# willow-ahrens/ChainPartitioners.jl

Measured on AMD Instinct MI355X. Metric: partitions/sec, DynamicTotalSplitter(AffineConnectivityModel{Int64}(0,0,0,1)), K=64, higher is better.
Workload: dtype int64; 1 GPU; config 3: DynamicTotalSplitter(AffineConnectivityModel{Int64}(0,0,0,1)) on suitesparse_shaped CSR (seeded SplitMix64 generator, tests/synth.py), n=10000000 rows, nnz=100000000, K=64; one independent partition per GPU; n=10000000, nnz=100000000, K=64, includes_oracle_build=True, device_block_pool=True

## Files before the change

chainpartitioners.jl_amd/_lib.py:

```python
from __future__ import annotations

import ctypes as C
import os
from functools import partial
import weakref

import numpy as np

from . import models as M

_HERE = os.path.dirname(os.path.abspath(__file__))
LIB_PATH = os.environ.get("CP_LIB_PATH") or os.path.join(_HERE, "libchainpart.so")


class _Array:

    def __init__(self, dtype, name):
        self.dtype, self.name, self.what = np.dtype(dtype), name, np.dtype(dtype).name

    def _accepts(self, a):
        return a.dtype == self.dtype

    def from_param(self, a):
        if a is None:
            return None
        if not (isinstance(a, np.ndarray) and self._accepts(a) and a.flags.c_contiguous):
            got = f"{'' if a.flags.c_contiguous else 'non-contiguous '}{a.dtype} array" if isinstance(a, np.ndarray) else type(a).__name__
            raise TypeError(f"{self.name}: expected None or a C-contiguous {self.what} array, got {got}")
        return C.c_void_p(a.ctypes.data)


class _Words(_Array):

    def __init__(self, name):
        self.dtype, self.name, self.what = None, name, "8-byte-element"

    def _accepts(self, a):
        return a.dtype.itemsize == 8


_I64, _I32, _F64 = (partial(_Array, t) for t in (np.int64, np.int32, np.float64))
_i32, _i64, _f64, _vp, _str = C.c_int32, C.c_int64, C.c_double, C.c_void_p, C.c_char_p
_pi32, _pi64, _pf64, _pvp = C.POINTER(C.c_int32), C.POINTER(C.c_int64), C.POINTER(C.c_double), C.POINTER(C.c_void_p)
_MODEL, _ROWPART = C.POINTER(M.cp_model_t), C.POINTER(M.cp_rowpart_t)
_PACK = (_i32, [_vp, _MODEL, _ROWPART, _MODEL, _i64, _f64, _I64("spl_out"), _I64("K_out")])
_SPLIT = (_i32, [_vp, _i64, _MODEL, _ROWPART, _MODEL, _i64, _f64, _I64("spl_out")])

SIGNATURES = {
    "cp_last_error": (_str, []),
    "cp_version": (_i32, []),
    "cp_device_count": (_i32, []),
    "cp_csr_create": (_i32, [_i64, _i64, _i64, _I64("colptr"), _I64("rowval"), _i32, _pvp]),
    "cp_csr_create_device": (_i32, [_i64, _i64, _i64, _vp, _vp, _i32, _pvp]),
    "cp_csr_destroy": (_i32, [_vp]),
    "cp_adjoint": (_i32, [_vp, _pvp]),
    "cp_csr_download": (_i32, [_vp, _I64("dims_out"), _I64("colptr_out"), _I64("rowval_out")]),
    "cp_csr_reset_cache": (_i32, [_vp]),
    "cp_count_build": (_i32, [_vp, _i32, _i32, _pvp]),
    "cp_count_query": (_i32, [_vp, _i64, _I64("a"), _I64("b"), _I64("out")]),
    "cp_count_destroy": (_i32, [_vp]),
    "cp_link_array": (_i32, [_vp, _I64("out")]),
    "cp_domsum_build": (_i32, [_vp, _i32, _Words("val"), _pvp]),
    "cp_rook_build": (_i32, [_i64, _I64("idx"), _i32, _Words("val"), _i32, _pvp]),
    "cp_wsum_query": (_i32, [_vp, _i64, _I64("i"), _I64("j"), _I64("count_out"), _I64("sum_i64"), _F64("sum_f64")]),
    "cp_wsum_destroy": (_i32, [_vp]),
    "cp_partwise": (_i32, [_vp, _i64, _I64("asg"), _pi64, _I64("pios_out"), _I64("prm_out"), _I64("pos_out"), _I64("idx_out")]),
    "cp_oracle_eval": (_i32, [_vp, _MODEL, _ROWPART, _i32, _i64, _I64("j"), _I64("jp"), _I64("k"), _I64("out_i64"), _F64("out_f64")]),
    "cp_oracle_step": (_i32, [_vp, _MODEL, _ROWPART, _i64, _I32("move_j"), _I64("j"), _I32("move_jp"), _I64("jp"), _I64("k"),
                              _I64("out_i64"), _F64("out_f64")]),
    "cp_bound_stripe": (_i32, [_vp, _i64, _MODEL, _pi64, _pi64, _pf64, _pf64]),
    "cp_bound_stripe_pi": (_i32, [_vp, _i64, _ROWPART, _MODEL, _pi64, _pi64, _pf64, _pf64]),
    "cp_objective": (_i32, [_vp, _i64, _I64("spl"), _MODEL, _ROWPART, _i32, _pi64, _pf64]),
    "cp_partition_dynamic": (_i32, [_vp, _i64, _i32, _i32, _MODEL, _ROWPART, _MODEL, _i64, _f64, _I64("spl_out")]),
    "cp_pack_dynamic": _PACK,
    "cp_pack_dynamic_tables": (_i32, [_vp, _MODEL, _ROWPART, _MODEL, _i64, _f64, _I64("spl_tab"), _I64("cst_i64"), _F64("cst_f64")]),
    "cp_partition_bisect_cost": (_i32, [_vp, _i64, _MODEL, _f64, _i32, _I64("spl_out")]),
    "cp_partition_bisect_cost_batch": (_i32, [_vp, _i64, _I64("K"), _MODEL, _F64("eps"), _I32("flip"), _i64, _I64("spl_out")]),
    "cp_partition_bisect_cost_pi": (_i32, [_vp, _i64, _MODEL, _ROWPART, _f64, _i32, _I64("spl_out")]),
    "cp_partition_bisect_index_pi": (_i32, [_vp, _i64, _MODEL, _ROWPART, _i32, _I64("spl_out")]),
    "cp_pack_concave": _PACK,
    "cp_partition_concave": _SPLIT,
    "cp_partition_bisect_index": (_i32, [_vp, _i64, _MODEL, _i32, _I64("spl_out")]),
    "cp_partition_lazy_bisect_cost": (_i32, [_vp, _i64, _MODEL, _f64, _I64("spl_out")]),
    "cp_partition_lazy_bisect_cost_probes": (_i32, [_vp, _i64, _MODEL, _f64, _I64("spl_out"), _pi64]),
    "cp_partition_lazy_bisect_cost_pi": (_i32, [_vp, _i64, _MODEL, _ROWPART, _f64, _I64("spl_out"), _I64("nprobes_out")]),
    "cp_partition_lazy_flip_bisect_cost": (_i32, [_vp, _i64, _MODEL, _ROWPART, _f64, _I64("spl_out"), _I64("nprobes_out")]),
    "cp_pack_convex": _PACK,
    "cp_pack_convex_batch": (_i32, [_vp, _i64, _MODEL, _I64("wmax"), _i64, _I64("spl_out"), _I64("K_out")]),
    "cp_partition_convex": _SPLIT,
    "cp_pack_strict": (_i32, [_vp, _i64, _I64("spl_out"), _I64("K_out")]),
    "cp_pack_overlap": (_i32, [_vp, _f64, _i64, _I64("spl_out"), _I64("K_out"), _I64("n_nets_out")]),
    "cp_partition_equi": (_i32, [_i64, _i64, _I64("spl_out")]),
    "cp_pack_equi": (_i32, [_i64, _i64, _I64("spl_out"), _I64("K_out")]),
    "cp_dynamic_tables": (_i32, [_vp, _i64, _i32, _MODEL, _ROWPART, _I64("ptr_out"), _I64("cst_i64"), _F64("cst_f64")]),
    "cp_dynamic_tables_constrained": (_i32, [_vp, _i64, _MODEL, _i64, _I64("win_lo"), _I64("win_hi"), _I64("ptr_out"),
                                             _I64("cst_i64"), _F64("cst_f64")]),
    "cp_dynamic_tables_constrained_combine": (_i32, [_vp, _i64, _i32, _MODEL, _MODEL, _i64, _f64, _I64("win_lo"), _I64("win_hi"),
                                                     _I64("ptr_out"), _I64("cst_i64"), _F64("cst_f64")]),
    "cp_dp_begin": (_i32, [_vp, _i64, _i32, _i32, _MODEL, _i64, _i64, _pvp]),
    "cp_dp_layer": (_i32, [_vp, _i64, _vp, _vp]),
    "cp_dp_ptr_at": (_i32, [_vp, _i64, _i64, _pi64]),
    "cp_dp_ptr_row": (_i32, [_vp, _i64, _I64("out")]),
    "cp_dp_set_window": (_i32, [_vp, _i64]),
    "cp_dp_set_rows": (_i32, [_vp, _i64, _i64]),
    "cp_dp_block_tables": (_i32, [_vp, _pi32, _I64("opt_out"), _I64("nets_out"), _I64("selfnets_out")]),
    "cp_dp_destroy": (_i32, [_vp]),
    "cp_set_stream": (_i32, [_vp, _vp]),
    "cp_reset_stream": (_i32, [_vp]),
    "cp_get_stat": (_i32, [_str, _pi64]),
    "cp_test_round_scans": (_i32, [_I32("a"), _i64, _i64, _I32("b"), _i64, _i64, _i32, _i64, _i64, _i32, _i32,
                                   _I64("offs_out"), _I64("toffs_out"), _I64("res")]),
    "cp_test_fix_merge": (_i32, [_MODEL, _i64, _I64("toffs"), _I64("part_v"), _I32("part_p"), _I32("part_nn"), _I32("part_nl"), _I32("tile_s"),
                                 _I32("tile_s2"), _I32("anchor"), _I32("anchor2"), _I32("row"), _I32("plane"), _i64, _i32, _I32("p_out"),
                                 _I32("nn_out"), _I32("nl_out"), _I64("res")]),
    "cp_test_own_split": (_i32, [_vp, _I32("vpos_out"), _I32("vsa_out"), _I32("vnext_out"), _I64("res")]),
    "cp_test_own_pair": (_i32, [_i64, _i64, _I64("res")]),
    "cp_set_option": (_i32, [_str, _i64]),
    "cp_prof_enable": (_i32, [_i32]),
    "cp_prof_reset": (_i32, []),
    "cp_prof_get": (_i32, [_i32, C.POINTER(C.c_char_p), _pi64, _pf64, _pf64]),
}
SYMBOLS = list(SIGNATURES)

_lib = None


def _typed(name, fn, restype, argtypes):
    fn.restype, fn.argtypes = restype, argtypes

    def call(*args):
        try:
            return fn(*args)
        except C.ArgumentError as e:
            raise TypeError(f"{name}: {e}") from None
    return call


def load_library():
    global _lib
    if _lib is None:
        if not os.path.exists(LIB_PATH):
            raise RuntimeError(f"{LIB_PATH} is missing: build it with __graft_entry__.build() "
                               "(make -C chainpartitioners.jl_amd/csrc); there is no CPU fallback")
        lib = C.CDLL(LIB_PATH)
        for name, (restype, argtypes) in SIGNATURES.items():
            setattr(lib, name, _typed(name, getattr(lib, name), restype, argtypes))
        _lib = lib
    return _lib


def _cost_zeros(mm, shape):
    return np.zeros(shape, dtype=np.int64 if mm.struct.dtype == M.CP_I64 else np.float64)


def _by_type(a):
    return (None, a) if a.dtype == np.float64 else (a, None)


_COUNT_KIND = {"dom": 0, "net": 1, "selfnet": 2, "dianet": 3, "selfpin": 4}


class HipBackend:
    name = "hip"

    def __init__(self, device=0):
        self.lib = load_library()
        if self.lib.cp_device_count() <= 0:
            raise RuntimeError("libchainpart: no HIP device visible (the product path has no CPU fallback)")
        self.device = int(device)
        self._handles = {}

    def last_error(self):
        return (self.lib.cp_last_error() or b"").decode()

    def _ok(self, rc, what, exc=RuntimeError):
        if rc != 0:
            raise exc(f"{what} -> {rc}: {self.last_error()}")

    def _register(self, obj, h):
        lib, handles, key = self.lib, self._handles, id(obj)

        def _drop(_ref):
            handles.pop(key, None)
            lib.cp_csr_destroy(h)
        handles[key] = (weakref.ref(obj, _drop), h)
        return h

    def csr(self, A):
        ent = self._handles.get(id(A))
        if ent is not None and ent[0]() is A:
            return ent[1]
        h = C.c_void_p()
        rc = self.lib.cp_csr_create(A.m, A.n, A.nnz, A.colptr, A.rowval, self.device, C.byref(h))
        if rc != 0:
            raise RuntimeError(f"cp_csr_create failed ({rc}): {self.last_error()}")
        return self._register(A, h)

    def _h(self, A):
        return A if isinstance(A, C.c_void_p) else self.csr(A)

    def csr_from_device(self, m, n, N, colptr_dev_ptr, rowval_dev_ptr):
        h = C.c_void_p()
        rc = self.lib.cp_csr_create_device(m, n, N, colptr_dev_ptr, rowval_dev_ptr, self.device, C.byref(h))
        if rc != 0:
            raise RuntimeError(f"cp_csr_create_device failed ({rc}): {self.last_error()}")
        return h

    def csr_destroy(self, h):
        self.lib.cp_csr_destroy(h)

    def adjoint(self, A):
        from .types import SparseMatrixCSC
        t = C.c_void_p()
        rc = self.lib.cp_adjoint(self._h(A), C.byref(t))
        if rc != 0:
            raise RuntimeError(f"cp_adjoint failed ({rc}): {self.last_error()}")
        dims = np.zeros(3, dtype=np.int64)
        self.lib.cp_csr_download(t, dims, None, None)
        m, n, N = (int(x) for x in dims)
        colptr = np.zeros(n + 1, dtype=np.int64); rowval = np.zeros(max(N, 1), dtype=np.int64)
        rc = self.lib.cp_csr_download(t, dims, colptr, rowval)
        if rc != 0:
            self.lib.cp_csr_destroy(t)
            raise RuntimeError(f"cp_csr_download failed ({rc}): {self.last_error()}")
        T = SparseMatrixCSC(m, n, colptr, rowval[:N])
        self._register(T, t)
        return T

    def reset_cache(self, A_or_handle):
        return self.lib.cp_csr_reset_cache(self._h(A_or_handle))

    def set_stream(self, A_or_handle, stream_ptr):
        return self.lib.cp_set_stream(self._h(A_or_handle), stream_ptr)

    def reset_stream(self, A_or_handle):
        return self.lib.cp_reset_stream(self._h(A_or_handle))

    def get_stat(self, name):
        out = C.c_int64()
        rc = self.lib.cp_get_stat(name.encode(), C.byref(out))
        if rc != 0:
            raise KeyError(name)
        return out.value

    def test_round_scans(self, a, na_max, b, nb_max, two=True, cap_t=2**62, cap_nt=2**62, err_in=0, reps=1):
        a = np.ascontiguousarray(a, dtype=np.int32)
        b = np.ascontiguousarray(b, dtype=np.int32)
        offs = np.zeros(len(a) + 1, dtype=np.int64)
        toffs = np.zeros(len(b) + 1, dtype=np.int64)
        res = np.zeros(6, dtype=np.int64)
        rc = self.lib.cp_test_round_scans(a, len(a), na_max, b, len(b), nb_max, 1 if two else 0, cap_t, cap_nt, err_in, reps,
                                          offs, toffs, res)
        self._ok(rc, "cp_test_round_scans")
        return offs, toffs, dict(zip(("T", "NT", "nlong", "nown", "ntile", "err"), (int(v) for v in res)))

    def test_fix_merge(self, mm, toffs, part_v, part_p, part_nn, part_nl, tile_s, tile_s2, anchor, anchor2, row, plane, n, reps=1):
        i32 = lambda a: None if a is None else np.ascontiguousarray(a, dtype=np.int32)
        toffs = np.ascontiguousarray(toffs, dtype=np.int64)
        ntask = len(toffs) - 1
        part_v = np.ascontiguousarray(part_v, dtype=np.int64 if mm.struct.dtype == M.CP_I64 else np.float64).view(np.int64)
        p, nn, res = np.zeros(ntask, np.int32), np.zeros(ntask, np.int32), np.zeros(4, np.int64)
        nl = None if part_nl is None else np.zeros(ntask, np.int32)
        rc = self.lib.cp_test_fix_merge(mm, ntask, toffs, part_v, i32(part_p), i32(part_nn), i32(part_nl), i32(tile_s), i32(tile_s2), i32(anchor),
                                        i32(anchor2), i32(row), i32(plane), n, reps, p, nn, nl, res)
        self._ok(rc, "cp_test_fix_merge")
        return p, nn, nl, dict(zip(("items", "trips", "edges", "tickets_left"), (int(v) for v in res)))

    def test_own_split(self, A):
        nb = max(0, int(A.n).bit_length() - 8)
        vpos = np.zeros((max(nb, 1), A.n + 1), np.int32); vsa = np.zeros_like(vpos)
        vnext = np.zeros(max(A.nnz, 1), np.int32); res = np.zeros(2, np.int64)
        rc = self.lib.cp_test_own_split(self._h(A), vpos.reshape(-1), vsa.reshape(-1), vnext, res)
        self._ok(rc, "cp_test_own_split")
        assert int(res[0]) == nb
        return nb, vpos[:nb], vsa[:nb], vnext[:int(res[1])]

    def test_own_pair(self, nt, wave):
        res = np.zeros(3, np.int64)
        self._ok(self.lib.cp_test_own_pair(nt, wave, res), "cp_test_own_pair")
        return bool(res[0]), int(res[1]), int(res[2])

    def set_option(self, name, value):
        return self.lib.cp_set_option(name.encode(), value)

    def partition_dynamic(self, A, K, combine, order, mm, rp, wm, wi, wf, spl):
        return self.lib.cp_partition_dynamic(self._h(A), K, combine, order, mm, rp, wm, wi, wf, spl)

    def pack_dynamic(self, A, mm, rp, wm, wi, wf, spl, Kout):
        return self.lib.cp_pack_dynamic(self._h(A), mm, rp, wm, wi, wf, spl, Kout)

    def pack_dynamic_tables(self, A, mm, rp, wm, wi, wf):
        spl = np.zeros(A.n + 1, dtype=np.int64)
        cst = _cost_zeros(mm, A.n + 1)
        rc = self.lib.cp_pack_dynamic_tables(self._h(A), mm, rp, wm, wi, wf, spl, *_by_type(cst))
        return rc, cst, spl

    def partition_bisect_cost(self, A, K, mm, eps, flip, spl, rp=None):
        return self.lib.cp_partition_bisect_cost_pi(self._h(A), K, mm, rp, eps, flip, spl)

    def partition_bisect_cost_batch(self, A, Ks, mms, epss, flips):
        B = len(Ks)
        arr = (M.cp_model_t * B)(*[m.struct for m in mms])
        Kv = np.ascontiguousarray(Ks, dtype=np.int64)
        ev = np.ascontiguousarray(epss, dtype=np.float64)
        fv = np.ascontiguousarray(flips, dtype=np.int32)
        ld = int(Kv.max()) + 1
        out = np.zeros((B, ld), dtype=np.int64)
        rc = self.lib.cp_partition_bisect_cost_batch(self._h(A), B, Kv, arr, ev, fv, ld, out)
        return rc, [out[b, :int(Kv[b]) + 1].copy() for b in range(B)]

    def partition_bisect_index(self, A, K, mm, flip, spl, rp=None):
        return self.lib.cp_partition_bisect_index_pi(self._h(A), K, mm, rp, flip, spl)

    def partition_lazy_bisect_cost(self, A, K, mm, eps, spl):
        if getattr(mm, "rowpart", None) is not None:
            return self.lib.cp_partition_lazy_bisect_cost_pi(self._h(A), K, mm, mm.rowpart, eps, spl, None)
        return self.lib.cp_partition_lazy_bisect_cost(self._h(A), K, mm, eps, spl)

    def partition_lazy_bisect_cost_probes(self, A, K, mm, eps, rp=None):
        spl = np.zeros(K + 1, dtype=np.int64)
        if rp is not None:
            npr = np.zeros(1, dtype=np.int64)
            rc = self.lib.cp_partition_lazy_bisect_cost_pi(self._h(A), K, mm, rp, eps, spl, npr)
            return rc, spl, int(npr[0])
        npr = C.c_int64()
        rc = self.lib.cp_partition_lazy_bisect_cost_probes(self._h(A), K, mm, eps, spl, C.byref(npr))
        return rc, spl, npr.value

    def partition_lazy_flip_bisect_cost(self, A, K, mm, eps, spl, rp=None):
        return self.lib.cp_partition_lazy_flip_bisect_cost(self._h(A), K, mm, rp, eps, spl, None)

    def partition_lazy_flip_bisect_cost_probes(self, A, K, mm, eps, rp=None):
        spl, npr = np.zeros(K + 1, dtype=np.int64), np.zeros(1, dtype=np.int64)
        rc = self.lib.cp_partition_lazy_flip_bisect_cost(self._h(A), K, mm, rp, eps, spl, npr)
        return rc, spl, int(npr[0])

    def pack_convex(self, A, mm, rp, wm, wi, wf, spl, Kout):
        return self.lib.cp_pack_convex(self._h(A), mm, rp, wm, wi, wf, spl, Kout)

    def pack_convex_batch(self, A, mms, wmaxs, n):
        B = len(mms)
        arr = (M.cp_model_t * B)(*[m.struct for m in mms])
        wv = np.ascontiguousarray(wmaxs, dtype=np.int64)
        ld = int(n) + 1
        out = np.zeros((B, ld), dtype=np.int64)
        Kout = np.zeros(B, dtype=np.int64)
        rc = self.lib.cp_pack_convex_batch(self._h(A), B, arr, wv, ld, out, Kout)
        return rc, [out[b, :int(Kout[b]) + 1].copy() for b in range(B)]

    def partition_convex(self, A, K, mm, rp, wm, wi, wf, spl):
        return self.lib.cp_partition_convex(self._h(A), K, mm, rp, wm, wi, wf, spl)

    def pack_concave(self, A, mm, rp, wm, wi, wf, spl, Kout):
        return self.lib.cp_pack_concave(self._h(A), mm, rp, wm, wi, wf, spl, Kout)

    def partition_concave(self, A, K, mm, rp, wm, wi, wf, spl):
        return self.lib.cp_partition_concave(self._h(A), K, mm, rp, wm, wi, wf, spl)

    def pack_strict(self, A, w_max, spl, Kout):
        return self.lib.cp_pack_strict(self._h(A), int(w_max), spl, Kout)

    def pack_overlap(self, A, rho, w_max, spl, Kout, n_nets=None):
        return self.lib.cp_pack_overlap(self._h(A), float(rho), int(w_max), spl, Kout, n_nets)

    def oracle_eval(self, A, mm, rp, hint, j, jp, k, out):
        return self.lib.cp_oracle_eval(self._h(A), mm, rp, hint, j.size, j, jp, k, *_by_type(out))

    def oracle_step(self, A, mm, rp, mj, j, mjp, jp, k, out):
        return self.lib.cp_oracle_step(self._h(A), mm, rp, j.size, mj, j, mjp, jp, k, *_by_type(out))

    def _bounds(self, fn, mm, *args):
        li, hi, lf, hf = C.c_int64(), C.c_int64(), C.c_double(), C.c_double()
        rc = fn(*args, C.byref(li), C.byref(hi), C.byref(lf), C.byref(hf))
        if mm.struct.dtype == M.CP_I64:
            return rc, li.value, hi.value
        return rc, lf.value, hf.value

    def bound_stripe(self, A, K, mm):
        return self._bounds(self.lib.cp_bound_stripe, mm, self._h(A), K, mm)

    def bound_stripe_pi(self, A, K, rp, mm):
        return self._bounds(self.lib.cp_bound_stripe_pi, mm, self._h(A), K, rp, mm)

    def objective(self, A, K, spl, mm, rp, g):
        oi, of = C.c_int64(), C.c_double()
        rc = self.lib.cp_objective(self._h(A), K, spl, mm, rp, g, C.byref(oi), C.byref(of))
        return rc, (oi.value if mm.struct.dtype == M.CP_I64 else of.value)

    def dynamic_tables(self, A, K, combine, mm, rp):
        ptr = np.zeros((K, A.n + 1), dtype=np.int64)
        cst = _cost_zeros(mm, (K, A.n + 1))
        rc = self.lib.cp_dynamic_tables(self._h(A), K, combine, mm, rp, ptr, *_by_type(cst))
        return rc, ptr.T, cst.T

    def dynamic_tables_constrained(self, A, K, mm, wmax, combine=0, wm=None):
        ptr = np.zeros((K, A.n + 1), dtype=np.int64)
        cst = _cost_zeros(mm, (K, A.n + 1))
        lo = np.zeros(K, dtype=np.int64); hi = np.zeros(K, dtype=np.int64)
        rc = self.lib.cp_dynamic_tables_constrained_combine(self._h(A), K, combine, mm, wm, int(wmax), float(wmax), lo, hi, ptr,
                                                            *_by_type(cst))
        return rc, lo, hi, ptr.T, cst.T

    def count_build(self, kind, A, hint):
        h = C.c_void_p()
        rc = self.lib.cp_count_build(self._h(A), _COUNT_KIND[kind], hint, C.byref(h))
        if rc == M.CP_EINVAL and kind in ("dianet", "selfpin"):
            raise AssertionError(f"cp_count_build({kind}): violated precondition ({self.last_error()})")
        self._ok(rc, f"cp_count_build({kind})", NotImplementedError)
        return h

    def count_query(self, kind, h, a, b, out):
        return self.lib.cp_count_query(h, a.size, a, b, out)

    def count_free(self, kind, h):
        self.lib.cp_count_destroy(h)

    def domsum_build(self, A, val):
        val = np.ascontiguousarray(val)
        dt = M.CP_F64 if val.dtype == np.float64 else M.CP_I64
        h = C.c_void_p()
        self._ok(self.lib.cp_domsum_build(self._h(A), dt, val, C.byref(h)), "cp_domsum_build")
        return h, dt

    def rook_build(self, N, idx, val=None):
        idx = np.ascontiguousarray(idx, dtype=np.int64)
        dt = M.CP_I64
        if val is not None:
            val = np.ascontiguousarray(val)
# ... 104 lines not shown
```

chainpartitioners.jl_amd/csrc/capi.hip:

```cpp
#include "csr.hpp"
#include "model.hpp"
#include "dp.hpp"
#include "weight.hpp"
#include "sym.hpp"
#include "cut.hpp"
#include <cmath>
#include <memory>

using namespace cpk;

namespace cpk {

__global__ void __launch_bounds__(256) k_range_counts(int64_t nq, const int64_t *__restrict__ P, const int64_t *__restrict__ Rr,
                                                      const int64_t *__restrict__ pos, const int32_t *__restrict__ prev,
                                                      const int64_t *__restrict__ fpos, const int32_t *__restrict__ flast,
                                                      unsigned long long *__restrict__ nets, unsigned long long *__restrict__ selfnets)
{
    int64_t i = blockIdx.x;
    if (i >= nq) return;
    __shared__ int64_t sh[256];
    int64_t p = P[i], r = Rr[i];
    int64_t stride = (int64_t)gridDim.y * 256, start = (int64_t)blockIdx.y * 256 + threadIdx.x;
    int64_t c = 0;
    if (r > p) {
        int64_t q0 = pos[p], q1 = pos[r];
        int32_t thr = (int32_t)p;
        for (int64_t q = q0 + start; q < q1; q += stride) c += (prev[q] < thr);
    }
    sh[threadIdx.x] = c;
    __syncthreads();
    for (int o = 128; o > 0; o >>= 1) { if (threadIdx.x < (unsigned)o) sh[threadIdx.x] += sh[threadIdx.x + o]; __syncthreads(); }
    if (threadIdx.x == 0 && sh[0]) atomicAdd(&nets[i], (unsigned long long)sh[0]);
    __syncthreads();
    if (selfnets) {
        c = 0;
        if (r > p) {
            int64_t s0 = fpos[p], s1 = fpos[r];
            int32_t thr = (int32_t)r;
            for (int64_t s = s0 + start; s < s1; s += stride) c += (flast[s] < thr);
        }
        sh[threadIdx.x] = c;
        __syncthreads();
        for (int o = 128; o > 0; o >>= 1) { if (threadIdx.x < (unsigned)o) sh[threadIdx.x] += sh[threadIdx.x + o]; __syncthreads(); }
        if (threadIdx.x == 0 && sh[0]) atomicAdd(&selfnets[i], (unsigned long long)sh[0]);
    }
}

template <typename TC>
__global__ void k_apply_model(int64_t nq, const int64_t *__restrict__ P, const int64_t *__restrict__ Rr, const int64_t *__restrict__ Kk,
                              const int64_t *__restrict__ pos, const int64_t *__restrict__ nets, const int64_t *__restrict__ selfnets,
                              DevModel<TC> M, TC *__restrict__ out)
{
    int64_t i = (int64_t)blockIdx.x * blockDim.x + threadIdx.x;
    if (i >= nq) return;
    int64_t p = P[i], r = Rr[i];
    TC alpha = dm_alpha(M, Kk ? Kk[i] : (int64_t)0);
    out[i] = dm_apply(M, alpha, r - p, pos[r] - pos[p], nets ? nets[i] : (int64_t)0, selfnets ? selfnets[i] : (int64_t)0);
}

static bool model_known(const cp_model_t *m)
{
    if (!m || m->kind < CP_MODEL_FEASIBLE || m->kind > CP_MODEL_SECONDARY_EDGE_CUT) return false;
    if (m->kind == CP_MODEL_POWER_WORK) return m->dtype == CP_F64;
    return m->dtype == CP_I64 || m->dtype == CP_F64;
}

template <typename TC>
static int32_t run_oracle_eval(cp_csr_s *A, const cp_model_t *mdl, int64_t nq, const int64_t *j, const int64_t *jp,
                               const int64_t *k, TC *out)
{
    hipStream_t s = A->stream;
    if (nq <= 0) return CP_OK;
    bool has_nets = mdl->kind == CP_MODEL_CONNECTIVITY || mdl->kind == CP_MODEL_HYPEREDGE_CUT || mdl->kind == CP_MODEL_COLBLOCK;
    bool need_self = mdl->kind == CP_MODEL_HYPEREDGE_CUT;
    if (has_nets) ensure_links(A);
    if (need_self) ensure_self(A);
    std::vector<int64_t> hp((size_t)nq), hr((size_t)nq);
    for (int64_t i = 0; i < nq; i++) {
        CP_REQUIRE(j[i] >= 1 && jp[i] >= j[i] && jp[i] <= A->n + 1, CP_EINVAL, "oracle query needs 1 <= j <= j' <= n+1");
        hp[i] = j[i] - 1; hr[i] = jp[i] - 1;
    }
    DBuf<int64_t> dP((size_t)nq), dR((size_t)nq), dK, dN, dS;
    DBuf<TC> dO((size_t)nq);
    CP_HIP(hipMemcpyAsync(dP.p, hp.data(), sizeof(int64_t) * (size_t)nq, hipMemcpyHostToDevice, s));
    CP_HIP(hipMemcpyAsync(dR.p, hr.data(), sizeof(int64_t) * (size_t)nq, hipMemcpyHostToDevice, s));
    if (k) { dK.alloc((size_t)nq); CP_HIP(hipMemcpyAsync(dK.p, k, sizeof(int64_t) * (size_t)nq, hipMemcpyHostToDevice, s)); }
    if (has_nets) {
        dN.alloc((size_t)nq);
        CP_HIP(hipMemsetAsync(dN.p, 0, dN.bytes(), s));
        if (need_self) { dS.alloc((size_t)nq); CP_HIP(hipMemsetAsync(dS.p, 0, dS.bytes(), s)); }
        int64_t per = nq > 0 ? A->N / nq : 0;
        unsigned gy = (unsigned)(per / 65536 + 1);
        if (gy > 2048) gy = 2048;
        ProfScope ps(PROF_QUERY, s, 0.0);
        hipLaunchKernelGGL(k_range_counts, dim3((unsigned)nq, gy), dim3(256), 0, s, nq, dP.p, dR.p, A->pos.p, A->prev.p,
                           need_self ? A->fpos.p : nullptr, need_self ? A->flast.p : nullptr, (unsigned long long *)dN.p,
                           need_self ? (unsigned long long *)dS.p : nullptr);
    }
    HostModel<TC> HM;
    build_dev_model<TC>(mdl, HM, s);
    hipLaunchKernelGGL(HIP_KERNEL_NAME(k_apply_model<TC>), dim3((unsigned)cdiv(nq, 256)), dim3(256), 0, s, nq, dP.p, dR.p,
                       k ? dK.p : nullptr, A->pos.p, has_nets ? dN.p : nullptr, need_self ? dS.p : nullptr, HM.d, dO.p);
    CP_HIP(hipGetLastError());
    CP_HIP(hipMemcpyAsync(out, dO.p, sizeof(TC) * (size_t)nq, hipMemcpyDeviceToHost, s));
    CP_HIP(hipStreamSynchronize(s));
    prof_collect();
    return CP_OK;
}

static int64_t fld(int64_t a, int64_t b)
{
    int64_t q = a / b, r = a % b;
    if (r != 0 && ((r < 0) != (b < 0))) q -= 1;
    return q;
}
static double fld(double a, int64_t b) { return std::floor(a / (double)b); }
static int64_t max_identity(int64_t) { return INT64_MIN; }
static double max_identity(double) { return -INFINITY; }
static void also_f64(const int64_t *lo, const int64_t *hi, double *lo_f64, double *hi_f64) { *lo_f64 = (double)*lo; *hi_f64 = (double)*hi; }
static void also_f64(const double *, const double *, double *, double *) {}

template <typename TC>
static int32_t oracle_eval_into(cp_csr_t A, const cp_model_t *model, const cp_rowpart_t *Pi, int64_t nq, const int64_t *j, const int64_t *jp,
                                const int64_t *k, TC *out)
{
    const bool i64 = std::is_same<TC, int64_t>::value;
    return cp_oracle_eval(A, model, Pi, CP_HINT_STEP, nq, j, jp, k, i64 ? (int64_t *)out : nullptr, i64 ? nullptr : (double *)out);
}

static const struct { const char *name; int64_t *var; bool kept; } g_stats[] = {
    {"spec_redo", &g_spec_redo, false}, {"poison_hits", &g_poison_hits, false}, {"fix_trips", &g_fix_trips, false},
    {"fix_edges", &g_fix_edges, false}, {"fix_items", &g_fix_items, false}, {"bn_sym_layers", &g_bn_sym_layers, true},
    {"own_split_tiles", &g_own_split_tiles, false}, {"gap_split_tiles", &g_gap_split_tiles, false},
    {"own_pair_waves", &g_own_pair_waves, false}, {"own_pair_lone", &g_own_pair_lone, false},
    {"overlap_isect", &g_overlap_isect, false}, {"cut_scan_layers", &g_cut_scan_layers, false},
};
static void stats_reset(bool all) { for (const auto &c : g_stats) if (all || !c.kept) *c.var = 0; }

enum OptRule { OPT_PLAIN, OPT_BOOL, OPT_CLAMP, OPT_POW2 };
constexpr int64_t NOLIM_LO = INT64_MIN, NOLIM_HI = INT64_MAX;
static const struct Opt { const char *name; int64_t *var; OptRule rule; int64_t lo, hi; } g_options[] = {
    {"force_brute", &g_opt_force_brute, OPT_PLAIN, 0, 0}, {"brute_max_n", &g_opt_brute_max_n, OPT_PLAIN, 0, 0}, {"dbg", &g_opt_dbg, OPT_PLAIN, 0, 0},
    {"short_t", &g_opt_short_t, OPT_PLAIN, 0, 0}, {"short_e", &g_opt_short_e, OPT_PLAIN, 0, 0}, {"ra_cache", &g_opt_ra_cache, OPT_PLAIN, 0, 0},
    {"leaf", &g_opt_leaf, OPT_PLAIN, 0, 0}, {"block_tables", &g_opt_block_tables, OPT_PLAIN, 0, 0}, {"nospec", &g_opt_nospec, OPT_PLAIN, 0, 0},
    {"rpass_small_tau", &g_opt_rpass_small_tau, OPT_PLAIN, 0, 0}, {"fixed_point", &g_opt_fixed_point, OPT_PLAIN, 0, 0},
    {"bn_wave", &g_opt_bn_wave, OPT_PLAIN, 0, 0},
    {"poison", &g_opt_poison, OPT_PLAIN, 0, 0},
    {"pool", &g_opt_pool, OPT_BOOL, 0, 0},
    {"own_blk", &g_opt_own_blk, OPT_BOOL, 0, 0},
    {"own_split", &g_opt_own_split, OPT_BOOL, 0, 0},
    {"own_pair", &g_opt_own_pair, OPT_BOOL, 0, 0},
    {"gap_split", &g_opt_gap_split, OPT_BOOL, 0, 0},
    {"lws", &g_opt_lws, OPT_BOOL, 0, 0},
    {"gap_tau", &g_opt_gap_tau, OPT_CLAMP, NOLIM_LO, 20}, {"gap_min", &g_opt_gap_min, OPT_CLAMP, 8, NOLIM_HI}, {"gap_nr", &g_opt_gap_nr, OPT_CLAMP, 1, 2},
    {"force_max", &g_opt_force_max, OPT_CLAMP, 0, NOLIM_HI}, {"rpass_cap", &g_opt_rpass_cap, OPT_CLAMP, 1, NOLIM_HI},
    {"own_min", &g_opt_own_min, OPT_CLAMP, 64, NOLIM_HI}, {"bn_chunk", &g_opt_bn_chunk, OPT_CLAMP, 1, NOLIM_HI},
    {"bn_slack", &g_opt_bn_slack, OPT_CLAMP, 0, NOLIM_HI}, {"bn_run", &g_opt_bn_run, OPT_CLAMP, 2, NOLIM_HI},
    {"rpass_ch", &g_opt_rpass_ch, OPT_POW2, 16, 4096}, {"setup_bs", &g_opt_setup_bs, OPT_POW2, 64, 1024}, {"lws_leaf", &g_opt_lws_leaf, OPT_POW2, 256, 2048},
};
static int64_t opt_value(const Opt &o, int64_t value)
{
    switch (o.rule) {
    case OPT_BOOL: return value ? 1 : 0;
    case OPT_CLAMP: return value < o.lo ? o.lo : value > o.hi ? o.hi : value;
    case OPT_POW2: { int64_t v = o.lo; while (v < value && v < o.hi) v <<= 1; return v; }
    default: return value;
    }
}

}

extern "C" {

const char *cp_last_error(void) { return g_last_error.c_str(); }
int32_t cp_version(void) { return 100; }

int32_t cp_device_count(void)
{
    int c = 0;
    if (hipGetDeviceCount(&c) != hipSuccess) return 0;
    return c;
}

static int32_t csr_create_impl(int64_t m, int64_t n, int64_t N, const int64_t *colptr, const int64_t *rowval,
                               int32_t device, bool on_device, cp_csr_t *out)
{
    return guarded([&]() -> int32_t {
        CP_REQUIRE(out && colptr && (rowval || N == 0), CP_EINVAL, "null argument");
        CP_REQUIRE(m >= 0 && n >= 0 && N >= 0, CP_EINVAL, "negative dimension");
        CP_REQUIRE(n < (int64_t)1 << 30 && m < (int64_t)1 << 30 && N < ((int64_t)1 << 31) - 65536, CP_EINVAL,
                   "dimensions exceed the 32-bit link-array layout");
        CP_REQUIRE(cp_device_count() > 0, CP_EHIP, "no HIP device visible: libchainpart has no CPU fallback");
        CP_HIP(hipSetDevice(device));
        std::unique_ptr<cp_csr_s> A(new cp_csr_s());
        A->device = device; A->m = m; A->n = n; A->N = N;
        CP_HIP(hipStreamCreate(&A->stream));
        A->own_stream = true;
        csr_upload(A.get(), colptr, rowval, on_device);
        *out = A.release();
        return CP_OK;
    });
}

int32_t cp_csr_create(int64_t m, int64_t n, int64_t N, const int64_t *colptr, const int64_t *rowval, int32_t device, cp_csr_t *out)
{
    if (colptr && n >= 0 && (colptr[0] != 1 || colptr[n] != N + 1)) { set_error("colptr must be 1-based with colptr[n+1] == nnz+1"); return CP_EINVAL; }
    return csr_create_impl(m, n, N, colptr, rowval, device, false, out);
}

int32_t cp_csr_create_device(int64_t m, int64_t n, int64_t N, const int64_t *colptr_device, const int64_t *rowval_device,
                             int32_t device, cp_csr_t *out)
{
    return csr_create_impl(m, n, N, colptr_device, rowval_device, device, true, out);
}

int32_t cp_csr_destroy(cp_csr_t A)
{
    if (!A) return CP_OK;
    (void)hipSetDevice(A->device);
    if (A->stream) (void)hipStreamSynchronize(A->stream);
    delete A;
    return CP_OK;
}

int32_t cp_adjoint(cp_csr_t A, cp_csr_t *out)
{
    return guarded([&]() -> int32_t {
        CP_REQUIRE(A && out, CP_EINVAL, "null argument");
        CP_HIP(hipSetDevice(A->device));
        std::unique_ptr<cp_csr_s> T(new cp_csr_s());
        T->device = A->device;
        CP_HIP(hipStreamCreate(&T->stream));
        T->own_stream = true;
        csr_adjoint(A, T.get());
        *out = T.release();
        return CP_OK;
    });
}

int32_t cp_csr_download(cp_csr_t A, int64_t *dims_out, int64_t *colptr_out, int64_t *rowval_out)
{
    return guarded([&]() -> int32_t {
        CP_REQUIRE(A, CP_EINVAL, "null argument");
        if (dims_out) { dims_out[0] = A->m; dims_out[1] = A->n; dims_out[2] = A->N; }
        if (!colptr_out) return CP_OK;
        CP_REQUIRE(rowval_out || A->N == 0, CP_EINVAL, "rowval_out is null");
        CP_HIP(hipSetDevice(A->device));
        csr_download(A, colptr_out, rowval_out);
        return CP_OK;
    });
}

int32_t cp_csr_reset_cache(cp_csr_t A)
{
    if (!A) return CP_EINVAL;
    return guarded([&]() -> int32_t { CP_HIP(hipStreamSynchronize(A->stream)); drop_cache(A); return CP_OK; });
}

int32_t cp_set_stream(cp_csr_t A, void *hip_stream)
{
    if (!A) return CP_EINVAL;
    if (A->own_stream && A->stream) { (void)hipStreamSynchronize(A->stream); (void)hipStreamDestroy(A->stream); }
    A->stream = (hipStream_t)hip_stream;
    A->own_stream = false;
    return CP_OK;
}

int32_t cp_get_stat(const char *name, int64_t *out)
{
    if (!name || !out) return CP_EINVAL;
    for (const auto &c : g_stats) if (!strcmp(name, c.name)) { *out = *c.var; return CP_OK; }
    return CP_EINVAL;
}

int32_t cp_test_round_scans(const int32_t *a, int64_t na, int64_t na_max, const int32_t *b, int64_t nb, int64_t nb_max, int32_t two, int64_t cap_t,
                            int64_t cap_nt, int32_t err_in, int32_t reps, int64_t *offs_out, int64_t *toffs_out, int64_t *res)
{
    if (!offs_out || !toffs_out || !res || (na > 0 && !a) || (nb > 0 && !b)) return CP_EINVAL;
    return guarded([&]() -> int32_t {
        dp_round_scans_test(a, na, na_max, b, nb, nb_max, two, cap_t, cap_nt, err_in, reps, offs_out, toffs_out, res);
        return CP_OK;
    });
}

int32_t cp_test_fix_merge(const cp_model_t *model, int64_t ntask, const int64_t *toffs, const int64_t *part_v, const int32_t *part_p, const int32_t *part_nn,
                          const int32_t *part_nl, const int32_t *tile_s, const int32_t *tile_s2, const int32_t *anchor, const int32_t *anchor2,
                          const int32_t *row, const int32_t *plane, int64_t n, int32_t reps, int32_t *p_out, int32_t *nn_out, int32_t *nl_out, int64_t *res)
{
    if (!model || !toffs || !part_v || !part_p || !part_nn || !tile_s || !anchor || !row || !plane || !p_out || !nn_out || !res) return CP_EINVAL;
    return guarded([&]() -> int32_t {
        dp_fix_merge_test(model, ntask, toffs, part_v, part_p, part_nn, part_nl, tile_s, tile_s2, anchor, anchor2, row, plane, n, reps, p_out, nn_out, nl_out, res);
        return CP_OK;
    });
}

int32_t cp_test_own_pair(int64_t nt, int64_t wave, int64_t *res)
{
    if (!res) return CP_EINVAL;
    return guarded([&]() -> int32_t {
        dp_own_pair_test(nt, wave, res);
        return CP_OK;
    });
}

int32_t cp_test_own_split(cp_csr_t A, int32_t *vpos_out, int32_t *vsa_out, int32_t *vnext_out, int64_t *res)
{
    if (!A || !vpos_out || !vsa_out || !vnext_out || !res) return CP_EINVAL;
    return guarded([&]() -> int32_t {
        CP_HIP(hipSetDevice(A->device));
        dp_own_split_test(A, vpos_out, vsa_out, vnext_out, res);
        return CP_OK;
    });
}

int32_t cp_reset_stream(cp_csr_t A)
{
    if (!A) return CP_EINVAL;
    return guarded([&]() -> int32_t {
        if (A->stream || !A->own_stream) (void)hipStreamSynchronize(A->stream);
        if (A->own_stream) return CP_OK;
        CP_HIP(hipSetDevice(A->device));
        hipStream_t s = nullptr;
        CP_HIP(hipStreamCreate(&s));
        A->stream = s; A->own_stream = true;
        return CP_OK;
    });
}

int32_t cp_set_option(const char *name, int64_t value)
{
    if (!name) return CP_EINVAL;
    if (!strcmp(name, "stat_reset")) { stats_reset(true); return CP_OK; }
    if (!strcmp(name, "prof_only")) { g_prof_only = (int)value; return CP_OK; }
    for (const Opt &o : g_options) {
        if (strcmp(name, o.name)) continue;
        *o.var = opt_value(o, value);
        if (o.var == &g_opt_pool && !value) dev_pool_trim();
        if (o.var == &g_opt_poison && value) stats_reset(false);
        return CP_OK;
    }
    set_error("unknown option");
    return CP_EINVAL;
}

int32_t cp_prof_enable(int32_t on) { g_prof_on = on != 0; return CP_OK; }
int32_t cp_prof_reset(void)
{
    for (auto &p : g_prof) { p.launches = 0; p.ms = 0; p.alg_bytes = 0; }
    return CP_OK;
}
int32_t cp_prof_get(int32_t slot, const char **name, int64_t *launches, double *total_ms, double *alg_bytes)
{
    if (slot >= 0 && slot < PROF_NSLOTS) {
        if (name) *name = g_prof[slot].name;
        if (launches) *launches = g_prof[slot].launches;
        if (total_ms) *total_ms = g_prof[slot].ms;
        if (alg_bytes) *alg_bytes = g_prof[slot].alg_bytes;
    }
    return PROF_NSLOTS;
}

int32_t cp_partition_equi(int64_t n, int64_t K, int64_t *spl_out)
{
    if (K < 1 || n < 0 || !spl_out) return CP_EINVAL;
    for (int64_t k = 0; k <= K; k++) spl_out[k] = k * (n / K) + ((n % K) < k ? (n % K) : k) + 1;
    return CP_OK;
}

int32_t cp_pack_equi(int64_t n, int64_t w, int64_t *spl_out, int64_t *K_out)
{
    if (w < 1 || n < 0 || !spl_out || !K_out) return CP_EINVAL;
    int64_t K = 0;
    for (int64_t j = 1; j <= n; j += w) spl_out[K++] = j;
    spl_out[K] = n + 1;
    *K_out = K;
    return CP_OK;
}

int32_t cp_partition_dynamic(cp_csr_t A, int64_t K, int32_t combine, int32_t order, const cp_model_t *model,
                             const cp_rowpart_t *Pi, const cp_model_t *weight, int64_t wmax_i64, double wmax_f64, int64_t *spl_out)
{
    return guarded([&]() -> int32_t {
        CP_REQUIRE(A && spl_out && model_known(model) && K >= 1, CP_EINVAL, "bad argument");
        CP_REQUIRE(combine == CP_COMBINE_SUM || combine == CP_COMBINE_MAX, CP_EINVAL, "bad combine");
        CP_HIP(hipSetDevice(A->device));
        bool constrained = weight && weight->kind != CP_MODEL_FEASIBLE;
        if (model->kind == CP_MODEL_PRIMARY || model->kind == CP_MODEL_SECONDARY) {
            CP_REQUIRE(!constrained, CP_EUNSUPPORTED, "ConstrainedCost over a plaid connectivity model has no device path");
            return with_cost_type(model->dtype, [&](auto tag) { return run_plaid_dynamic<decltype(tag)>(A, K, combine, order, model, Pi, spl_out); });
        }
        if (model_is_cut(model->kind)) {
            CP_REQUIRE(!constrained, CP_EUNSUPPORTED, "ConstrainedCost over a plaid edge-cut model has no device path");
            return with_cost_type(model->dtype, [&](auto tag) {
                using TC = decltype(tag);
                return run_cut_dynamic<TC>(A, K, combine, order, model, Pi, spl_out, nullptr, (TC *)nullptr);
            });
        }
        CP_REQUIRE(!(constrained && model_is_sym(model->kind)), CP_EUNSUPPORTED, "ConstrainedCost over a symmetric cost model has no device path");
        if (constrained) {
            CP_REQUIRE(weight->kind == CP_MODEL_VERTEX_COUNT || (weight->kind == CP_MODEL_WORK && !weight->alpha_k), CP_EINVAL,
                       "weight must be VertexCount or an AffineWorkModel");
            const int64_t wv = width_of_weight(weight, A->n, wmax_i64, wmax_f64);
            if (windowed_ok(A, K, combine, model, wv))
                return run_dynamic_windowed(A, K, combine, order, model, wv, nullptr, 0, 0, spl_out, nullptr, nullptr, nullptr, nullptr, nullptr);
            if (combine == CP_COMBINE_MAX && wv == -2 && monotone_work_weight(weight) && model->dtype == CP_I64 && windowed_ok(A, K, combine, model, 1))
                return run_dynamic_windowed(A, K, combine, order, model, 0, weight, wmax_i64, wmax_f64, spl_out, nullptr, nullptr, nullptr, nullptr, nullptr);
            return with_cost_type(model->dtype, [&](auto tag) {
                return run_dyn_constrained<decltype(tag)>(A, K, combine, order, model, Pi, weight, wmax_i64, wmax_f64, spl_out);
            });
        }
        CP_REQUIRE(model->kind == CP_MODEL_WORK || model->kind == CP_MODEL_CONNECTIVITY || model->kind == CP_MODEL_HYPEREDGE_CUT ||
                       model->kind == CP_MODEL_COLBLOCK || model->kind == CP_MODEL_POWER_WORK || model_is_sym(model->kind),
                   CP_EUNSUPPORTED, "model kind has no device DP path yet");
        return run_dynamic(A, K, combine, order, model, spl_out, nullptr, nullptr, nullptr);
    });
}

int32_t cp_dynamic_tables(cp_csr_t A, int64_t K, int32_t combine, const cp_model_t *model, const cp_rowpart_t *Pi,
                          int64_t *ptr_out, int64_t *cst_i64, double *cst_f64)
{
    return guarded([&]() -> int32_t {
        CP_REQUIRE(A && ptr_out && model_known(model) && K >= 1, CP_EINVAL, "bad argument");
        CP_REQUIRE(combine == CP_COMBINE_SUM || combine == CP_COMBINE_MAX, CP_EINVAL, "bad combine");
        if (model_is_cut(model->kind)) {
            CP_HIP(hipSetDevice(A->device));
            std::vector<int64_t> spl((size_t)K + 1);
            return with_cost_type(model->dtype, [&](auto tag) {
                using TC = decltype(tag);
                return run_cut_dynamic<TC>(A, K, combine, CP_ORDER_SPLITTER, model, Pi, spl.data(), ptr_out, pick<TC>(cst_i64, cst_f64));
            });
        }
        CP_REQUIRE(model->kind == CP_MODEL_WORK || model->kind == CP_MODEL_CONNECTIVITY || model->kind == CP_MODEL_HYPEREDGE_CUT ||
                       model->kind == CP_MODEL_COLBLOCK || model->kind == CP_MODEL_POWER_WORK || model_is_sym(model->kind),
                   CP_EUNSUPPORTED, "model kind has no device DP path");
        CP_HIP(hipSetDevice(A->device));
        std::vector<int64_t> spl((size_t)K + 1);
        return run_dynamic(A, K, combine, CP_ORDER_SPLITTER, model, spl.data(), ptr_out, cst_i64, cst_f64);
    });
}

int32_t cp_dynamic_tables_constrained_combine(cp_csr_t A, int64_t K, int32_t combine, const cp_model_t *model, const cp_model_t *weight,
                                              int64_t wmax_i64, double wmax_f64, int64_t *win_lo, int64_t *win_hi, int64_t *ptr_out,
                                              int64_t *cst_i64, double *cst_f64)
{
    return guarded([&]() -> int32_t {
        CP_REQUIRE(A && ptr_out && win_lo && win_hi && model_known(model) && K >= 1, CP_EINVAL, "bad argument");
        CP_REQUIRE(combine == CP_COMBINE_SUM || combine == CP_COMBINE_MAX, CP_EINVAL, "bad combine");
        CP_REQUIRE(!weight || weight->kind == CP_MODEL_VERTEX_COUNT || (weight->kind == CP_MODEL_WORK && !weight->alpha_k), CP_EINVAL,
                   "weight must be VertexCount or an AffineWorkModel");
        const int64_t wv = weight ? width_of_weight(weight, A->n, wmax_i64, wmax_f64) : wmax_i64;
        const bool general = wv == -2 && combine == CP_COMBINE_MAX && monotone_work_weight(weight) && model->dtype == CP_I64;
        CP_REQUIRE(windowed_ok(A, K, combine, model, general ? 1 : wv), CP_EUNSUPPORTED, "outside the windowed scalable path");
        CP_HIP(hipSetDevice(A->device));
        std::vector<int64_t> spl((size_t)K + 1);
        return run_dynamic_windowed(A, K, combine, CP_ORDER_SPLITTER, model, general ? 0 : wv, general ? weight : nullptr, wmax_i64, wmax_f64,
                                    spl.data(), ptr_out, cst_i64, cst_f64, win_lo, win_hi);
    });
}

int32_t cp_dynamic_tables_constrained(cp_csr_t A, int64_t K, const cp_model_t *model, int64_t wmax, int64_t *win_lo, int64_t *win_hi,
                                      int64_t *ptr_out, int64_t *cst_i64, double *cst_f64)
{
    return cp_dynamic_tables_constrained_combine(A, K, CP_COMBINE_SUM, model, nullptr, wmax, (double)wmax, win_lo, win_hi, ptr_out, cst_i64, cst_f64);
// ... 292 lines not shown
```

chainpartitioners.jl_amd/csrc/dp.hpp:

```cpp
#pragma once
#include "csr.hpp"
#include "model.hpp"

struct cp_dp_s {
    cp_csr_s *A = nullptr;
    int64_t K = 0;
    int32_t combine = 0, order = 0;
    bool fast = false, fast_bn = false, need_self = false;
    void *work = nullptr;
    cpk::DBuf<int32_t> ptr;
    int64_t rlo = 0, rhi = 0;
    int64_t wwin = 0;
    std::vector<int64_t> lay_lo, lay_hi;
    virtual ~cp_dp_s() = default;
    virtual int32_t step_layer(int64_t k, const void *cst_prev_device, void *cst_cur_device) = 0;
    virtual int32_t block_tables(int32_t *nplanes_out, int64_t *opt_out, int64_t *nets_out, int64_t *selfnets_out) = 0;
};

namespace cpk {

using DpBase = ::cp_dp_s;

struct DpWindow {
    int64_t w = 0;
    int64_t lo = 0, hi = -1;
    const int32_t *j0 = nullptr;
};

int32_t run_dynamic(cp_csr_s *A, int64_t K, int32_t combine, int32_t order, const cp_model_t *mdl, int64_t *spl_out,
                    int64_t *ptr_tab, int64_t *cst_i64, double *cst_f64);
bool windowed_ok(cp_csr_s *A, int64_t K, int32_t combine, const cp_model_t *model, int64_t wmax);
int32_t run_dynamic_windowed(cp_csr_s *A, int64_t K, int32_t combine, int32_t order, const cp_model_t *mdl, int64_t width,
                             const cp_model_t *weight, int64_t wmax_i64, double wmax_f64, int64_t *spl_out, int64_t *ptr_tab,
                             int64_t *cst_i64, double *cst_f64, int64_t *win_lo, int64_t *win_hi);
int32_t dp_begin(cp_csr_s *A, int64_t K, int32_t combine, int32_t order, const cp_model_t *model, int64_t row_lo, int64_t row_hi,
                 cp_dp_s **out);

template <typename TC>
void dp_total_layer(cp_csr_s *A, const DevModel<TC> &M, TC alpha, const TC *W, TC *cst_out, int32_t *ptr_out, void *work,
                    int64_t rlo, int64_t rhi,
                    int64_t wwin = 0);
template <typename TC> int dp_total_block_tables(cp_csr_s *A, void *work, int64_t *opt_out, int64_t *nn_out, int64_t *nl_out);
template <typename TC> void *dp_total_work_get(cp_csr_s *A);
template <typename TC> void *dp_total_work_new();
template <typename TC> void dp_total_work_free(void *w);

template <typename TC>
void dp_brute_layer(cp_csr_s *A, const DevModel<TC> &M, TC alpha, int32_t combine, const TC *W, TC *cst_out,
                    int32_t *ptr_out, int64_t r_lo, int64_t r_hi);

struct WaveletDev;
struct BnPattern {
    const int64_t *pos; const int32_t *pos32, *pin32, *prev, *next;
    int64_t N;
    const WaveletDev *net;
};
extern int64_t g_bn_sym_layers;

template <typename TC>
void dp_bottleneck_layer(cp_csr_s *A, const DevModel<TC> &M, TC alpha, const TC *W, TC *cst_out, int32_t *ptr_out,
                         int64_t r_lo, int64_t r_hi,
                         int64_t wwin = 0, int64_t p_lo0 = 0, int64_t p_hi0 = -1, const int32_t *j0 = nullptr,
                         const BnPattern *pat = nullptr);
extern int64_t g_opt_bn_wave, g_opt_bn_run, g_opt_bn_slack;
extern int64_t g_opt_bn_chunk;

template <typename TC>
int32_t run_dyn_constrained(cp_csr_s *A, int64_t K, int32_t g, int32_t order, const cp_model_t *mdl, const cp_rowpart_t *Pi,
                            const cp_model_t *w, int64_t wi, double wf, int64_t *spl_out);
template <typename TC>
int32_t run_seq_eval(cp_csr_s *A, const cp_model_t *mdl, const cp_rowpart_t *Pi, int64_t nq, const int64_t *j, const int64_t *jp,
                     const int64_t *k, TC *out);

struct PlaidPart {
    DBuf<int32_t> owner;
    DBuf<int64_t> spl;
    std::vector<int64_t> hspl;
    int64_t K = 0;
};
void upload_part(cp_csr_s *A, const cp_rowpart_t *Pi, bool need_spl, PlaidPart &R);
template <typename TC>
int32_t run_plaid_eval(cp_csr_s *A, const cp_model_t *mdl, const cp_rowpart_t *Pi, int64_t nq, const int64_t *j, const int64_t *jp,
                       const int64_t *k, TC *out);
template <typename TC>
int32_t run_plaid_dynamic(cp_csr_s *A, int64_t K, int32_t combine, int32_t order, const cp_model_t *mdl, const cp_rowpart_t *Pi,
                          int64_t *spl_out);

template <typename TC>
bool pack_dynamic_scan(hipStream_t s, int64_t n, int64_t wmax, const TC *Ftab, TC *cst1, int64_t *spl1);

extern int64_t g_opt_lws, g_opt_lws_leaf;
bool lws_ok(const cp_csr_s *A, const cp_model_t *mdl, const cp_model_t *w, int64_t wi, double wf);
template <typename TC>
int32_t run_pack_lws(cp_csr_s *A, const DevModel<TC> &M, const WaveletDev &wnet, const WaveletDev &wself, const cp_model_t *w, int64_t wi,
                     double wf, TC *cst1, int64_t *spl1);

extern int64_t g_opt_gap_nr;
extern int64_t g_opt_gap_tau, g_opt_gap_min;
extern int64_t g_opt_poison, g_poison_hits;
void dp_round_scans_test(const int32_t *a, int64_t na, int64_t na_max, const int32_t *b, int64_t nb, int64_t nb_max, int two, int64_t capT, int64_t capNT,
                         int err_in, int reps, int64_t *offs_out, int64_t *toffs_out, int64_t *res);
void dp_fix_merge_test(const cp_model_t *model, int64_t ntask, const int64_t *toffs, const int64_t *part_v, const int32_t *part_p, const int32_t *part_nn,
                       const int32_t *part_nl, const int32_t *tile_s, const int32_t *tile_s2, const int32_t *anchor, const int32_t *anchor2, const int32_t *row,
                       const int32_t *plane, int64_t n, int reps, int32_t *p_out, int32_t *nn_out, int32_t *nl_out, int64_t *res);
extern int64_t g_fix_trips, g_fix_edges;
extern int64_t g_fix_items;
extern int64_t g_opt_leaf;
extern int64_t g_opt_block_tables;
extern int64_t g_opt_ra_cache;
extern int64_t g_opt_fixed_point;
extern int64_t g_opt_nospec;
extern int64_t g_spec_redo;
extern int64_t g_opt_rpass_small_tau;
extern int64_t g_opt_force_max;
extern int64_t g_opt_setup_bs;
extern int64_t g_opt_rpass_cap;
extern int64_t g_opt_rpass_ch;
extern int64_t g_opt_own_min;
extern int64_t g_opt_own_blk;
extern int64_t g_opt_own_split;
extern int64_t g_own_split_tiles;
extern int64_t g_opt_gap_split;
extern int64_t g_gap_split_tiles;
extern int64_t g_opt_own_pair;
extern int64_t g_own_pair_waves, g_own_pair_lone;
void dp_own_pair_test(int64_t nt, int64_t wave, int64_t *res);
extern int64_t g_overlap_isect;
void dp_own_split_test(cp_csr_s *A, int32_t *vpos_out, int32_t *vsa_out, int32_t *vnext_out, int64_t *res);
extern int64_t g_opt_short_t, g_opt_short_e;
extern int64_t g_opt_force_brute;
extern int64_t g_opt_brute_max_n;
extern int64_t g_opt_dbg;
enum DbgBit : int64_t {
    DBG_PRINT_ROUNDS = 8,
    DBG_NO_INTERIOR = 32,
    DBG_NO_OWN_TILES = 64,
    DBG_POISON = 128,
    DBG_POISON_ZERO = 256,
    DBG_GAP_ALL_SPECIAL = 512,
    DBG_MISPREDICT = 1024,
    DBG_TINY_BUFFERS = 2048,
    DBG_COUNT_NONTRIVIAL = 4096,
    DBG_COMBINE_BY_SLOT = 16384,
    DBG_RA_ROWMAJOR = 262144,
    DBG_NO_FORCE_OWN = 524288,
    DBG_WIN_NO_RA_CACHE = 1048576,
    DBG_WIN_NO_MIR_CACHE = 2097152,
    DBG_BN_NO_HINT2 = 4194304,
    DBG_MIR_ROWMAJOR = 8388608,
    DBG_RA_ALL_LEVELS = 33554432,
    DBG_BN_NO_HINT_STARTS = 33554432,
};

}
```

chainpartitioners.jl_amd/csrc/dp_brute.hip:

```cpp
#include "csr.hpp"
#include "model.hpp"
#include "dp.hpp"

namespace cpk {

int64_t g_opt_force_brute = 0;
int64_t g_opt_short_t = 8, g_opt_short_e = 64;
int64_t g_opt_own_min = 64;
int64_t g_opt_own_blk = 1;
int64_t g_opt_own_split = 1;
int64_t g_own_split_tiles = 0;
int64_t g_opt_gap_split = 1;
int64_t g_gap_split_tiles = 0;
int64_t g_opt_own_pair = 1;
int64_t g_own_pair_waves = 0, g_own_pair_lone = 0;
int64_t g_opt_rpass_ch = 256;
int64_t g_opt_rpass_small_tau = 4;
int64_t g_opt_force_max = 1024;
int64_t g_opt_setup_bs = 1024;
int64_t g_opt_rpass_cap = 200;
int64_t g_opt_nospec = 0, g_spec_redo = 0;
int64_t g_opt_gap_tau = 6, g_opt_gap_min = 64, g_opt_gap_nr = 2;
int64_t g_opt_ra_cache = 1;
int64_t g_opt_leaf = 1, g_opt_block_tables = 0;
int64_t g_opt_poison = 0, g_poison_hits = 0;
int64_t g_fix_trips = 0, g_fix_edges = 0, g_fix_items = 0;
int64_t g_opt_fixed_point = 0;
int64_t g_opt_brute_max_n = 200000;
int64_t g_opt_dbg = 0;

template <typename TC>
__global__ void __launch_bounds__(256) k_brute_layer(int64_t n, int64_t r_lo, int64_t r_hi, const int64_t *__restrict__ pos,
                                                     const int32_t *__restrict__ next, const int64_t *__restrict__ fpos,
                                                     const int32_t *__restrict__ flast, DevModel<TC> M, TC alpha,
                                                     int32_t g, const TC *__restrict__ W, TC *__restrict__ cst,
                                                     int32_t *__restrict__ ptr)
{
    int64_t wave = ((int64_t)blockIdx.x * blockDim.x + threadIdx.x) >> 6;
    int lane = threadIdx.x & 63;
    int64_t r0 = r_lo + wave * 64;
    if (r0 > r_hi) return;
    int64_t r = r0 + lane;
    bool live = r <= r_hi;
    int64_t rtop = r0 + 63 < r_hi ? r0 + 63 : r_hi;
    int64_t nn = 0, nl = 0;
    TC best = (TC)0;
    int64_t bp = -1;
    bool self = (M.kind == CP_MODEL_HYPEREDGE_CUT);
    int32_t rr = (int32_t)r;
    for (int64_t p = rtop; p >= 0; p--) {
        if (p < n) {
            bool step = live && (r > p);
            int64_t q0 = pos[p], q1 = pos[p + 1];
            for (int64_t q = q0; q < q1; q++) {
                int32_t nx = next[q];
                if (step) nn += (nx >= rr);
            }
            if (self) {
                int64_t s0 = fpos[p], s1 = fpos[p + 1];
                for (int64_t sidx = s0; sidx < s1; sidx++) {
                    int32_t la = flast[sidx];
                    if (step) nl += (la < rr);
                }
            }
        }
        if (live && r >= p) {
            TC f = dm_apply(M, alpha, r - p, pos[r] - pos[p], nn, nl);
            TC v = comb(g, W[p], f);
            if (bp < 0 || v < best) { best = v; bp = p; }
        }
    }
    if (live) { cst[r] = best; ptr[r] = (int32_t)bp; }
}

template <typename TC>
void dp_brute_layer(cp_csr_s *A, const DevModel<TC> &M, TC alpha, int32_t combine, const TC *W, TC *cst_out,
                    int32_t *ptr_out, int64_t r_lo, int64_t r_hi)
{
    hipStream_t s = A->stream;
    int64_t rows = r_hi - r_lo + 1;
    int64_t waves = cdiv(rows, 64);
    int64_t blocks = cdiv(waves, 4);
    ProfScope ps(PROF_BRUTE, s, 0.0);
    hipLaunchKernelGGL(HIP_KERNEL_NAME(k_brute_layer<TC>), dim3((unsigned)blocks), dim3(256), 0, s, A->n, r_lo, r_hi, A->pos.p,
                       A->next.p, A->fpos.p, A->flast.p, M, alpha, combine, W, cst_out, ptr_out);
    CP_HIP(hipGetLastError());
}

template void dp_brute_layer<int64_t>(cp_csr_s *, const DevModel<int64_t> &, int64_t, int32_t, const int64_t *, int64_t *, int32_t *, int64_t, int64_t);
template void dp_brute_layer<double>(cp_csr_s *, const DevModel<double> &, double, int32_t, const double *, double *, int32_t *, int64_t, int64_t);

}
```

chainpartitioners.jl_amd/csrc/dp_total.hip:

```cpp
#include "dp_total.hpp"
#include <optional>

namespace cpk {

struct RoundDesc {
    int32_t isA, tau, nbits, nextra;
    Geo G;
    int64_t aoff[32];
    int64_t n, ntask;
    int64_t tbase[36];
    int64_t tskip[36];
    int64_t a_r0, a_nmain;
    int64_t extra[64];
    int32_t nlast, last_b[31];
    int32_t skip_std, skip_mir;
    int32_t fin_stamp;
};

__device__ __forceinline__ void decode_task(const RoundDesc &R, int64_t t, int64_t &r, int &b)
{
    if (R.G.win) {
        int bb = R.isA ? 0 : R.tau + 1;
        while (t >= R.tbase[bb + 1]) bb++;
        const int64_t l = t - R.tbase[bb] + R.tskip[bb];
        r = R.isA ? ((l + 1) << bb) : (((l << 1) | 1) << R.tau);
        b = bb;
        return;
    }
    if (R.isA) {
        if (t >= R.a_nmain + R.nextra) { r = R.n; b = R.last_b[t - R.a_nmain - R.nextra]; return; }
        r = t < R.a_nmain ? R.a_r0 + t : R.extra[t - R.a_nmain]; b = __ffsll((long long)r) - 1; return;
    }
    int bb = R.tau + 1;
    while (t >= R.tbase[bb + 1]) bb++;
    int64_t l = t - R.tbase[bb] + R.tskip[bb];
    int sh = bb - R.tau - 1;
    int64_t base = l >> sh, v = l & (((int64_t)1 << sh) - 1);
    r = (base << (bb + 1)) | ((int64_t)1 << bb) | (((v << 1) | 1) << R.tau);
    b = bb;
}

template <bool ge, int NB>
__global__ void __launch_bounds__(256) k_rpass_small(int tau, int nbits, int64_t n, int64_t u0, int64_t nrows, const int64_t *__restrict__ pos,
                                                     const int32_t *__restrict__ prev, const int32_t *__restrict__ opt,
                                                     int32_t *__restrict__ cr, int allp, int cap)
{
    int64_t u = (int64_t)blockIdx.x * blockDim.x + threadIdx.x;
    bool live = u < nrows;
    u += u0;
    int64_t r = ((u << 1) | 1) << tau;
    if (r > n) live = false;
    if (!live) r = 0;
    int64_t n1 = n + 1, rL = r - ((int64_t)1 << tau);
    int32_t thr[NB], cnt[NB];
    uint32_t used = 0;
    int64_t prL = live ? prow((rL), n1 - 1) : 0;
#pragma unroll
    for (int b = 0; b < NB; b++) {
        cnt[b] = 0;
        thr[b] = ge ? INT32_MAX : INT32_MIN;
        if (b <= tau || b >= nbits) continue;
        bool on = live && (allp || ((r >> b) & 1));
        if (!__ballot(on)) continue;
        used |= 1u << b;
        int32_t v = opt[(int64_t)b * n1 + (on ? prL : 0)];
        if (on) thr[b] = v;
    }
    int64_t q0 = 0;
    int32_t len = 0;
    if (live) { q0 = pos[rL]; len = (int32_t)(pos[r] - q0); }
    const int32_t NEVER = ge ? INT32_MIN : INT32_MAX;
    const int32_t mlen = len < cap ? len : cap;
    for (int32_t o = 0; o < mlen; o += 16) {
        int32_t v[16];
        struct __attribute__((packed, aligned(4))) V4 { int32_t a, b, c, d; };
        const V4 *pv = reinterpret_cast<const V4 *>(prev + q0 + o);
        const int32_t rem = mlen - o;
#pragma unroll
        for (int j = 0; j < 4; j++) {
            V4 t = {NEVER, NEVER, NEVER, NEVER};
            if (4 * j < rem) t = pv[j];
            v[4 * j] = t.a; v[4 * j + 1] = t.b; v[4 * j + 2] = t.c; v[4 * j + 3] = t.d;
        }
#pragma unroll
        for (int j = 0; j < 16; j++) v[j] = j < rem ? v[j] : NEVER;
#pragma unroll
        for (int b = 0; b < NB; b++) {
            if (!((used >> b) & 1)) continue;
            int32_t t = thr[b];
            int32_t c = 0;
#pragma unroll
            for (int j = 0; j < 16; j++) c += ge ? (v[j] >= t) : (v[j] < t);
            cnt[b] += c;
        }
    }
    {
        const int lane = threadIdx.x & 63;
        uint32_t mypl = 0;
        if (live)
            for (int b = tau + 1; b < nbits; b++) if (allp || ((r >> b) & 1)) mypl |= 1u << b;
        uint64_t rest = __ballot(len > cap);
        const int32_t q0lo = (int32_t)(uint32_t)q0, q0hi = (int32_t)(q0 >> 32);
        while (rest) {
            const int src = __ffsll((unsigned long long)rest) - 1;
            rest &= rest - 1;
            const int64_t a = (((int64_t)__builtin_amdgcn_readlane(q0hi, src) << 32) | (uint32_t)__builtin_amdgcn_readlane(q0lo, src)) + cap;
            const int32_t ln = __builtin_amdgcn_readlane(len, src) - cap;
            const uint32_t pl = (uint32_t)__builtin_amdgcn_readlane((int32_t)mypl, src);
            for (int32_t o = 0; o < ln; o += 64) {
                const int32_t v = o + lane < ln ? prev[a + o + lane] : NEVER;
#pragma unroll
                for (int b = 0; b < NB; b++) {
                    if (!((pl >> b) & 1)) continue;
                    const int32_t t = __builtin_amdgcn_readlane(thr[b], src);
                    const int32_t c = (int32_t)__popcll(__ballot(ge ? (v >= t) : (v < t)));
                    if (lane == src) cnt[b] += c;
                }
            }
        }
    }
    if (!live) return;
#pragma unroll
    for (int b = 0; b < NB; b++)
        if (b > tau && b < nbits && (allp || ((r >> b) & 1))) cr[(int64_t)b * n1 + prow((r), n1 - 1)] = cnt[b];
}

template <bool ge, int WPB>
__global__ void __launch_bounds__(64 * WPB) k_rpass_wave(int tau, int nbits, int64_t n, int64_t u0, int64_t nrows, int chunks_per_row, int ch_cols,
                                                         const int64_t *__restrict__ pos, const int32_t *__restrict__ prev,
                                                         const int32_t *__restrict__ opt, int32_t *__restrict__ cr, int allp)
{
    int64_t w = (int64_t)blockIdx.x * WPB + (threadIdx.x >> 6);
    int lane = threadIdx.x & 63;
    int64_t u = w / chunks_per_row;
    int ck = (int)(w - u * chunks_per_row);
    if (u >= nrows) return;
    u += u0;
    int64_t r = ((u << 1) | 1) << tau;
    if (r > n) return;
    int64_t n1 = n + 1, rL = r - ((int64_t)1 << tau);
    int64_t c0 = rL + (int64_t)ck * ch_cols, c1 = c0 + ch_cols;
    if (c1 > r) c1 = r;
    int64_t prL = prow((rL), n1 - 1);
    uint32_t act = 0;
    for (int b = tau + 1; b < nbits; b++) if (allp || ((r >> b) & 1)) act |= 1u << b;
    act = __builtin_amdgcn_readfirstlane(act);
    const bool mine = lane < 32 && ((act >> lane) & 1);
    const int32_t tv = mine ? opt[(int64_t)lane * n1 + prL] : 0;
    int32_t acc = 0;
    const int64_t q0 = pos[c0], q1 = pos[c1];
    const int32_t NEVER = ge ? INT32_MIN : INT32_MAX;
    int32_t a[8], nx[8];
    struct __attribute__((packed, aligned(4))) V4 { int32_t x, y, z, w; };
#pragma unroll
    for (int k = 0; k < 2; k++) {
        const int64_t q = q0 + 4 * lane + 256 * k;
        V4 t = {NEVER, NEVER, NEVER, NEVER};
        if (q < q1) t = *reinterpret_cast<const V4 *>(prev + q);
        a[4 * k] = t.x; a[4 * k + 1] = q + 1 < q1 ? t.y : NEVER; a[4 * k + 2] = q + 2 < q1 ? t.z : NEVER; a[4 * k + 3] = q + 3 < q1 ? t.w : NEVER;
    }
    for (int64_t qb = q0; qb < q1; qb += 512) {
#pragma unroll
        for (int k = 0; k < 2; k++) {
            const int64_t q = qb + 512 + 4 * lane + 256 * k;
            V4 t = {NEVER, NEVER, NEVER, NEVER};
            if (q < q1) t = *reinterpret_cast<const V4 *>(prev + q);
            nx[4 * k] = t.x; nx[4 * k + 1] = q + 1 < q1 ? t.y : NEVER; nx[4 * k + 2] = q + 2 < q1 ? t.z : NEVER; nx[4 * k + 3] = q + 3 < q1 ? t.w : NEVER;
        }
        for (uint32_t rem = act; rem; rem &= rem - 1) {
            const int b = __ffs(rem) - 1;
            const int32_t t = __builtin_amdgcn_readlane(tv, b);
            int32_t c = 0;
#pragma unroll
            for (int k = 0; k < 8; k++) c += (int32_t)__popcll(__ballot(ge ? (a[k] >= t) : (a[k] < t)));
            acc += lane == b ? c : 0;
        }
#pragma unroll
        for (int k = 0; k < 8; k++) a[k] = nx[k];
    }
    int32_t outv = acc;
    if (WPB > 1) {
        __shared__ int32_t sacc[WPB > 1 ? WPB : 1][32];
        const int wv = threadIdx.x >> 6;
        if (lane < 32) sacc[wv][lane] = mine ? outv : 0;
        __syncthreads();
        if (wv != 0) return;
        if (mine) {
            int32_t t = 0;
#pragma unroll
            for (int k = 0; k < WPB; k++) t += sacc[k][lane];
            outv = t;
        }
    }
    if (mine) {
        if (chunks_per_row == WPB) cr[(int64_t)lane * n1 + prow((r), n1 - 1)] = outv;
        else atomicAdd(&cr[(int64_t)lane * n1 + prow((r), n1 - 1)], outv);
    }
}

__global__ void __launch_bounds__(256) k_last_row_counts(RoundDesc R, const int32_t *__restrict__ pos, const int32_t *__restrict__ prev,
                                                         const int32_t *__restrict__ lpos, const int32_t *__restrict__ lfirst, int32_t *__restrict__ out,
                                                         uint8_t *__restrict__ fin)
{
    __shared__ int32_t s_acc[64];
    if (threadIdx.x < 64) s_acc[threadIdx.x] = 0;
    __syncthreads();
    const int64_t n = R.n, n1 = n + 1;
    if (blockIdx.x == 0 && threadIdx.x < (unsigned)R.nlast) fin[(int64_t)R.last_b[threadIdx.x] * n1 + prow(n, n)] = (uint8_t)R.fin_stamp;
    for (int pass = 0; pass < (lpos ? 2 : 1); pass++) {
        const int32_t *cp = pass ? lpos : pos, *arr = pass ? lfirst : prev;
        for (int i = 0; i < R.nlast; i++) {
            const int64_t rb = (n >> R.last_b[i]) << R.last_b[i];
            int32_t c = 0;
            for (int64_t q = (int64_t)cp[rb] + (int64_t)blockIdx.x * blockDim.x + threadIdx.x, q1 = cp[n]; q < q1; q += (int64_t)gridDim.x * blockDim.x) {
                int32_t v = arr[q];
                c += pass ? (v >= rb) : (v < rb);
            }
            for (int o = 32; o > 0; o >>= 1) c += __shfl_xor(c, o);
            if ((threadIdx.x & 63) == 0 && c) atomicAdd(&s_acc[pass * 32 + i], c);
        }
    }
    __syncthreads();
    if (threadIdx.x < 64 && s_acc[threadIdx.x]) {
        int pass = threadIdx.x >> 5, i = threadIdx.x & 31;
        if (i < R.nlast) atomicAdd(&out[pass * 32 + R.last_b[i]], s_acc[threadIdx.x]);
    }
}

__global__ void __launch_bounds__(256) k_setup(RoundDesc R, const int32_t *__restrict__ opt, const int32_t *__restrict__ nnopt,
                                               int32_t *__restrict__ cr, int zero_cr_only,
                                               int4 *__restrict__ tdesc, const int32_t *__restrict__ pos32,
                                               uint8_t *__restrict__ tb, int32_t *__restrict__ len,
                                               const int32_t *__restrict__ nlopt, int32_t *__restrict__ crl, int32_t *__restrict__ tS0l)
{
    int64_t t = (int64_t)blockIdx.x * blockDim.x + threadIdx.x;
    if (t >= R.ntask) return;
    int64_t r; int b;
    decode_task(R, t, r, b);
    int64_t n1 = R.n + 1;
    if (zero_cr_only) { cr[(int64_t)b * n1 + prow((r), n1 - 1)] = 0; if (crl) crl[(int64_t)b * n1 + prow((r), n1 - 1)] = 0; return; }
    int64_t B, a, S0, S0l = 0;
    if (R.isA) {
        B = r; a = r - ((int64_t)1 << b); S0 = 0;
    } else {
        int64_t rb = (r >> b) << b;
        int64_t rL = r - ((int64_t)1 << R.tau), rR = r + ((int64_t)1 << R.tau);
        B = opt[(int64_t)b * n1 + prow((rL), n1 - 1)];
        S0 = (int64_t)nnopt[(int64_t)b * n1 + prow((rL), n1 - 1)] + cr[(int64_t)b * n1 + prow((r), n1 - 1)];
        if (tS0l) S0l = (int64_t)nlopt[(int64_t)b * n1 + prow((rL), n1 - 1)] + crl[(int64_t)b * n1 + prow((r), n1 - 1)];
        a = (rR - rb) < ((int64_t)1 << b) ? (int64_t)opt[(int64_t)b * n1 + prow((rR <= R.n ? rR : R.n), n1 - 1)] : rb - ((int64_t)1 << b);
        if (a > B) a = B;
    }
    tdesc[t] = make_int4((int32_t)B, (int32_t)S0, (int32_t)r, pos32[r]);
    tb[t] = (uint8_t)b;
    len[t] = (int32_t)(1 + (B - a));
    if (tS0l) tS0l[t] = (int32_t)S0l;
}

template <typename TC> __device__ __forceinline__ void best_clear(Best<TC, false> &b) { b.v = (TC)0; b.p = -1; b.nn = 0; }
template <typename TC> __device__ __forceinline__ void best_clear(Best<TC, true> &b) { b.v = (TC)0; b.p = -1; b.nn = 0; b.nl = 0; b._pad = 0; }
template <typename TC> __device__ __forceinline__ int32_t best_nl(const Best<TC, false> &) { return 0; }
template <typename TC> __device__ __forceinline__ int32_t best_nl(const Best<TC, true> &b) { return b.nl; }
template <typename TC> __device__ __forceinline__ void best_set_nl(Best<TC, false> &, int32_t) {}
template <typename TC> __device__ __forceinline__ void best_set_nl(Best<TC, true> &b, int32_t v) { b.nl = v; }

template <typename TC>
__device__ __forceinline__ Best<TC, false> best_sel(bool tb, const Best<TC, false> a, const Best<TC, false> b)
{
    Best<TC, false> r; r.v = tb ? b.v : a.v; r.p = tb ? b.p : a.p; r.nn = tb ? b.nn : a.nn; return r;
}
template <typename TC>
__device__ __forceinline__ Best<TC, true> best_sel(bool tb, const Best<TC, true> a, const Best<TC, true> b)
{
    Best<TC, true> r; r.v = tb ? b.v : a.v; r.p = tb ? b.p : a.p; r.nn = tb ? b.nn : a.nn; r.nl = tb ? b.nl : a.nl; r._pad = 0; return r;
}
template <typename TC, bool HYP>
__device__ __forceinline__ Best<TC, HYP> better(const Best<TC, HYP> a, const Best<TC, HYP> b)
{
    const bool tb = a.p < 0 || (b.p >= 0 && b.v < a.v);
    return best_sel<TC>(tb, a, b);
}

__device__ __forceinline__ void wave_segsum(int32_t &v, int &f, int lane)
{
#pragma unroll
    for (int o = 1; o < 64; o <<= 1) {
        int32_t pv = __shfl_up(v, o);
        int pf = __shfl_up(f, o);
        if (lane >= o) { if (!f) v += pv; f |= pf; }
    }
}

template <typename TC, bool HYP>
__device__ __forceinline__ void wave_segmin(Best<TC, HYP> &x, int &f, int lane)
{
#pragma unroll
    for (int o = 1; o < 64; o <<= 1) {
        Best<TC, HYP> p;
        best_clear(p);
        p.v = shfl_up64(x.v, o);
        p.p = __shfl_up(x.p, o);
        p.nn = __shfl_up(x.nn, o);
        if (HYP) best_set_nl(p, __shfl_up(best_nl(x), o));
        int pf = __shfl_up(f, o);
        if (lane >= o) { if (!f) x = better(p, x); f |= pf; }
    }
}

__host__ __device__ __forceinline__ int32_t own_ntiles(int blk, int64_t B, int64_t L)
{
    return blk ? (int32_t)(B / LT - (B - L + 1) / LT + 1) : (int32_t)((L + LT - 1) / LT);
}
__device__ __forceinline__ void own_tile_geo(int blk, int32_t B, int32_t L, int32_t kt, int32_t &pf, int32_t &tl)
{
    if (blk) {
        const int32_t a = B - L + 1;
        pf = kt == 0 ? B : (B / LT - kt) * LT + (LT - 1);
        const int32_t c0 = pf - pf % LT;
        tl = pf - (a > c0 ? a : c0);
    } else {
        pf = B - kt * LT;
        const int32_t rest = L - kt * LT;
        tl = (rest < LT ? rest : LT) - 1;
    }
}

template <typename TC, bool HYP>
__global__ void __launch_bounds__(1024) k_setup_short(RoundDesc R, int32_t *__restrict__ opt, int32_t *__restrict__ nnopt, int32_t *__restrict__ nlopt,
                                                      const int32_t *__restrict__ cr, const int32_t *__restrict__ crl,
                                                      const int32_t *__restrict__ pos32, const int32_t *__restrict__ next,
                                                      const int32_t *__restrict__ fpos32, const int32_t *__restrict__ flast,
                                                      const TC *__restrict__ W, DevModel<TC> M, TC alpha,
                                                      int4 *__restrict__ tdesc, uint8_t *__restrict__ tb, int32_t *__restrict__ len,
                                                      int32_t *__restrict__ tS0l, int32_t *__restrict__ nlong, int32_t SHORT_T, int32_t SHORT_E,
                                                      int4 *__restrict__ o_tdesc, uint8_t *__restrict__ o_tb, int32_t *__restrict__ o_rlen,
                                                      int32_t *__restrict__ o_ntl, int32_t *__restrict__ o_tS0l, int32_t *__restrict__ n_own,
                                                      unsigned long long *__restrict__ own_steps, int32_t OWN_MIN, int32_t o_cap,
                                                      int32_t *__restrict__ err, const uint8_t *__restrict__ fin, const int32_t *__restrict__ last_s0,
                                                      int32_t *__restrict__ dbg_ntriv, const int32_t *__restrict__ anch, const int32_t *__restrict__ anch2,
                                                      int32_t *__restrict__ pz, int OWN_BLK)
{
    int lane = threadIdx.x & 63;
    bool live;
    bool is_long = false, is_own = false, is_short = false;
    int64_t r = 0, B = 0, a = 0, S0 = 0, S0l = 0; int b = 0;
    uint8_t finb = 0;
    if (R.isA) {
        int64_t t = (int64_t)blockIdx.x * blockDim.x + threadIdx.x;
        live = t < R.ntask;
// ... 2022 lines not shown
        memcpy(&b.v, part_v + k, sizeof(TC)); b.p = part_p[k]; b.nn = part_nn[k];
        if constexpr (HYP) b.nl = part_nl[k];
        hpart[(size_t)k] = b;
    }
    std::vector<int4> htd((size_t)ntask);
    std::vector<uint8_t> htb((size_t)ntask);
    std::vector<int32_t> hrlen((size_t)ntask);
    for (int64_t t = 0; t < ntask; t++) {
        htd[(size_t)t] = make_int4(0, anchor[t], row[t], 0); htb[(size_t)t] = (uint8_t)plane[t];
        hrlen[(size_t)t] = (int32_t)std::min<int64_t>((toffs[t + 1] - toffs[t]) * LT, INT32_MAX);
    }
    HostModel<TC> HM;
    build_dev_model<TC>(model, HM, s);
    const size_t c = (size_t)NT, icap = fix_items_cap(c), pl = (size_t)np * (size_t)n1;
    DBuf<int64_t> dtoffs((size_t)ntask + 1);
    DBuf<Best<TC, HYP>> dpart(c);
    DBuf<int4> dtd((size_t)ntask), drec(c);
    DBuf<uint8_t> dtb((size_t)ntask);
    DBuf<int32_t> drlen((size_t)ntask), dS0l((size_t)ntask), dS(c), dS2(c), dtask(c), ditem_of(c), dopt(pl), dnn(pl), dnl(pl);
    DBuf<int2> ditems(icap);
    DBuf<unsigned long long> dtrec(icap * FIX_REC_W);
    DBuf<uint32_t> dtick((size_t)ntask);
    DBuf<RoundCounts> drc(1);
    auto up = [&](void *d, const void *h, size_t bytes) { CP_HIP(hipMemcpyAsync(d, h, bytes, hipMemcpyHostToDevice, s)); };
    up(dtoffs.p, toffs, dtoffs.bytes()); up(dpart.p, hpart.data(), dpart.bytes()); up(dtd.p, htd.data(), dtd.bytes()); up(dtb.p, htb.data(), dtb.bytes());
    up(drlen.p, hrlen.data(), drlen.bytes()); up(dS.p, tile_s, dS.bytes());
    if (HYP) { up(dS0l.p, anchor2, dS0l.bytes()); up(dS2.p, tile_s2, dS2.bytes()); }
    CP_HIP(hipMemsetAsync(dtick.p, 0, dtick.bytes(), s));
    RoundCounts h;
    for (int r = 0; r < reps; r++) {
        memset(&h, 0, sizeof(h));
        h.nown = (int32_t)ntask; h.NT = NT;
        up(drc.p, &h, sizeof(h));
        CP_HIP(hipMemsetAsync(dopt.p, 0xFF, dopt.bytes(), s)); CP_HIP(hipMemsetAsync(dnn.p, 0xFF, dnn.bytes(), s)); CP_HIP(hipMemsetAsync(dnl.p, 0xFF, dnl.bytes(), s));
        CP_HIP(hipMemsetAsync(ditems.p, 0x7F, ditems.bytes(), s)); CP_HIP(hipMemsetAsync(ditem_of.p, 0x7F, ditem_of.bytes(), s));
        CP_HIP(hipMemsetAsync(dtrec.p, 0x7F, dtrec.bytes(), s));
        hipLaunchKernelGGL(k_own_map, dim3((unsigned)std::min<int64_t>(cdiv(NT, (int64_t)256), 8192)), dim3(256), 0, s, drc.p, dtoffs.p, dtd.p, drlen.p, drec.p,
                           dtask.p, dtb.p, (int32_t *)nullptr, 0, n, 0, (int32_t *)nullptr, (int32_t *)nullptr, ditems.p, ditem_of.p, 0);
        launch_fix_own<TC, HYP>(s, drc.p, dtoffs.p, dpart.p, dtd.p, dtb.p, HYP ? dS0l.p : nullptr, dS.p, HYP ? dS2.p : nullptr, HM.d, dopt.p, dnn.p, HYP ? dnl.p : nullptr, n,
                                ditems.p, ditem_of.p, dtrec.p, dtick.p, NT, ntask);
        CP_HIP(hipMemcpyAsync(&h, drc.p, sizeof(h), hipMemcpyDeviceToHost, s));
        CP_HIP(hipStreamSynchronize(s));
        g_fix_items += h.n_items;
    }
    std::vector<int32_t> hopt(pl), hnn(pl), hnl(HYP ? pl : 0);
    std::vector<uint32_t> htick((size_t)ntask);
    CP_HIP(hipMemcpyAsync(hopt.data(), dopt.p, dopt.bytes(), hipMemcpyDeviceToHost, s));
    CP_HIP(hipMemcpyAsync(hnn.data(), dnn.p, dnn.bytes(), hipMemcpyDeviceToHost, s));
    if (HYP) CP_HIP(hipMemcpyAsync(hnl.data(), dnl.p, dnl.bytes(), hipMemcpyDeviceToHost, s));
    CP_HIP(hipMemcpyAsync(htick.data(), dtick.p, dtick.bytes(), hipMemcpyDeviceToHost, s));
    CP_HIP(hipStreamSynchronize(s));
    int64_t left = 0;
    for (int64_t t = 0; t < ntask; t++) {
        const int64_t r = row[t];
        const int lv = __builtin_ctzll((unsigned long long)r);
        const size_t cell = (size_t)plane[t] * (size_t)n1 + (size_t)((n - (n >> lv)) + (r >> (lv + 1)));
        p_out[t] = hopt[cell]; nn_out[t] = hnn[cell];
        if (HYP) nl_out[t] = hnl[cell];
        left += htick[(size_t)t] != 0;
    }
    res[0] = h.n_items; res[1] = h.n_trips; res[2] = h.n_edge; res[3] = left;
}

void dp_fix_merge_test(const cp_model_t *model, int64_t ntask, const int64_t *toffs, const int64_t *part_v, const int32_t *part_p, const int32_t *part_nn,
                       const int32_t *part_nl, const int32_t *tile_s, const int32_t *tile_s2, const int32_t *anchor, const int32_t *anchor2, const int32_t *row,
                       const int32_t *plane, int64_t n, int reps, int32_t *p_out, int32_t *nn_out, int32_t *nl_out, int64_t *res)
{
    const bool hyp = model->kind == CP_MODEL_HYPEREDGE_CUT;
    CP_REQUIRE(model->kind == CP_MODEL_WORK || model->kind == CP_MODEL_CONNECTIVITY || hyp, CP_EINVAL, "fix merge test: not a model of the O(n log^2 n) scheme");
    CP_REQUIRE(!hyp || (part_nl && tile_s2 && anchor2 && nl_out), CP_EINVAL, "fix merge test: a hyperedge model needs the second counts");
    CP_REQUIRE(ntask >= 1 && ntask < ((int64_t)1 << 24) && n >= 1 && n < ((int64_t)1 << 26) && reps >= 1 && reps <= 16, CP_EINVAL, "fix merge test: bad sizes");
    CP_REQUIRE(toffs[0] == 0, CP_EINVAL, "fix merge test: toffs must start at 0");
    for (int64_t t = 0; t < ntask; t++) {
        CP_REQUIRE(toffs[t + 1] > toffs[t] && toffs[t + 1] < ((int64_t)1 << 26), CP_EINVAL, "fix merge test: every task needs a tile, 2^26 tiles at most");
        CP_REQUIRE(row[t] >= 1 && row[t] <= n && plane[t] >= 0 && plane[t] < 4, CP_EINVAL, "fix merge test: rows are 1 .. n, planes 0 .. 3");
    }
    with_cost_type(model->dtype, [&](auto tag) {
        using TC = decltype(tag);
        if (hyp) fix_merge_test_run<TC, true>(model, ntask, toffs, part_v, part_p, part_nn, part_nl, tile_s, tile_s2, anchor, anchor2, row, plane, n, reps, p_out, nn_out, nl_out, res);
        else fix_merge_test_run<TC, false>(model, ntask, toffs, part_v, part_p, part_nn, part_nl, tile_s, tile_s2, anchor, anchor2, row, plane, n, reps, p_out, nn_out, nl_out, res);
    });
}

__device__ __forceinline__ int split_plane(int32_t p, int32_t x) { return 31 - __clz((int)(p ^ x)); }

__global__ void __launch_bounds__(256) k_split_count(const int32_t *__restrict__ pos, const int32_t *__restrict__ next, int64_t n, int nb,
                                                     int32_t *__restrict__ cnt)
{
    const int64_t p = (int64_t)blockIdx.x * blockDim.x + threadIdx.x;
    if (p > n) return;
    int32_t c[SPLIT_NB];
#pragma unroll
    for (int b = 0; b < SPLIT_NB; b++) c[b] = 0;
    if (p < n)
        for (int32_t q = pos[p], qe = pos[p + 1]; q < qe; q++) {
            const int h = split_plane((int32_t)p, next[q]) - SPLIT_BMIN;
#pragma unroll
            for (int b = 0; b < SPLIT_NB; b++) c[b] += (h == b);
        }
#pragma unroll
    for (int b = 0; b < SPLIT_NB; b++) if (b < nb) cnt[(int64_t)b * (n + 1) + p] = c[b];
}

__global__ void __launch_bounds__(256) k_split_scatter(const int32_t *__restrict__ pos, const int32_t *__restrict__ next, int64_t n, int nb,
                                                       const int32_t *__restrict__ vpos, int32_t *__restrict__ vnext, int32_t *__restrict__ vsa)
{
    const int64_t p = (int64_t)blockIdx.x * blockDim.x + threadIdx.x;
    if (p > n) return;
    int32_t c[SPLIT_NB];
#pragma unroll
    for (int b = 0; b < SPLIT_NB; b++) c[b] = b < nb ? vpos[(int64_t)b * (n + 1) + p] : 0;
    int32_t above = 0;
#pragma unroll
    for (int b = SPLIT_NB - 1; b >= 0; b--)
        if (b < nb) { vsa[(int64_t)b * (n + 1) + p] = above; above += c[b] - vpos[(int64_t)b * (n + 1)]; }
    if (p < n)
        for (int32_t q = pos[p], qe = pos[p + 1]; q < qe; q++) {
            const int32_t x = next[q];
            const int h = split_plane((int32_t)p, x) - SPLIT_BMIN;
            int32_t dst = -1;
#pragma unroll
            for (int b = 0; b < SPLIT_NB; b++) if (h == b) { dst = c[b]; c[b]++; }
            if (dst >= 0) vnext[dst] = x;
        }
}

static void split_build(cp_csr_s *A, SplitLinks &S, DBuf<int64_t> &scratch)
{
    hipStream_t s = A->stream;
    const int64_t n = A->n, n1 = n + 1;
    int nbits = 1;
    while (((int64_t)1 << nbits) <= n) nbits++;
    S.nb = std::max(0, nbits - SPLIT_BMIN); S.stride = n1;
    for (auto &t : S.tot) t = 0;
    if (S.nb > 0) {
        CP_REQUIRE(S.nb <= SPLIT_NB, CP_EINVAL, "n exceeds the bit-plane budget");
        const size_t cells = (size_t)S.nb * (size_t)n1;
        S.vpos.ensure(cells + 1); S.vsa.ensure(cells + 1); S.vnext.ensure((size_t)A->N + 8);
        const unsigned grid = (unsigned)cdiv(n1, 256);
        hipLaunchKernelGGL(k_split_count, dim3(grid), dim3(256), 0, s, A->pos32.p, A->next.p, n, S.nb, S.vsa.p);
        exclusive_scan_i32_i32(S.vsa.p, S.vpos.p, (int64_t)cells, scratch, s);
        hipLaunchKernelGGL(k_split_scatter, dim3(grid), dim3(256), 0, s, A->pos32.p, A->next.p, n, S.nb, S.vpos.p, S.vnext.p, S.vsa.p);
        CP_HIP(hipGetLastError());
        int32_t st[SPLIT_NB + 1];
        for (int b = 0; b <= S.nb; b++)
            CP_HIP(hipMemcpyAsync(&st[b], S.vpos.p + (size_t)b * (size_t)n1, sizeof(int32_t), hipMemcpyDeviceToHost, s));
        CP_HIP(hipStreamSynchronize(s));
        for (int b = 0; b < S.nb; b++) S.tot[b] = (int64_t)st[b + 1] - st[b];
        S.tot[S.nb] = st[S.nb];
    }
    S.built = true;
}

void dp_own_pair_test(int64_t nt, int64_t wave, int64_t *res)
{
    int64_t s0 = 0, s1 = 0;
    res[0] = own_pair_slots(wave, nt, s0, s1) ? 1 : 0;
    res[1] = s0;
    res[2] = s1;
}

void dp_own_split_test(cp_csr_s *A, int32_t *vpos_out, int32_t *vsa_out, int32_t *vnext_out, int64_t *res)
{
    ensure_links(A);
    SplitLinks S;
    DBuf<int64_t> scratch;
    split_build(A, S, scratch);
    res[0] = S.nb; res[1] = S.tot[S.nb];
    if (S.nb <= 0) return;
    const size_t cells = (size_t)S.nb * (size_t)S.stride;
    CP_HIP(hipMemcpyAsync(vpos_out, S.vpos.p, cells * sizeof(int32_t), hipMemcpyDeviceToHost, A->stream));
    CP_HIP(hipMemcpyAsync(vsa_out, S.vsa.p, cells * sizeof(int32_t), hipMemcpyDeviceToHost, A->stream));
    if (res[1] > 0) CP_HIP(hipMemcpyAsync(vnext_out, S.vnext.p, (size_t)res[1] * sizeof(int32_t), hipMemcpyDeviceToHost, A->stream));
    CP_HIP(hipStreamSynchronize(A->stream));
}

static int64_t count_rows(int b, int tau, int64_t x)
{
    if (x < 0) return 0;
    int sh = b - tau - 1;
    int64_t V = (int64_t)1 << sh;
    int64_t nfull = (x + ((int64_t)1 << tau)) >> (b + 1);
    int64_t cnt = nfull * V;
    int64_t y = x - (nfull << (b + 1)) - ((int64_t)1 << b);
    if (y >= ((int64_t)1 << tau)) cnt += ((y >> tau) + 1) >> 1;
    return cnt;
}

static void make_round(RoundDesc &R, bool isA, int tau, int nbits, int64_t n, int64_t rlo, int64_t rhi, const Geo &G = Geo{0, 0, 0},
                       const int64_t *aoff = nullptr)
{
    memset(&R, 0, sizeof(R));
    R.isA = isA; R.tau = tau; R.nbits = nbits; R.n = n; R.G = G;
    if (G.win) {
        if (aoff) for (int b = 0; b < 32; b++) R.aoff[b] = aoff[b];
        int64_t acc = 0;
        for (int b = 0; b < 36; b++) {
            R.tbase[b] = acc;
            if (b > G.s || (!isA && b <= tau)) continue;
            if (isA) {
                int64_t lo = rlo - ((int64_t)2 << b), hi = rhi + ((int64_t)1 << b);
                if (lo < ((int64_t)1 << b)) lo = (int64_t)1 << b;
                if (hi > n) hi = n;
                int64_t l0 = ((lo + ((int64_t)1 << b) - 1) >> b) - 1, l1 = (hi >> b) - 1;
                R.tskip[b] = l0;
                acc += l1 >= l0 ? l1 - l0 + 1 : 0;
            } else {
                int64_t rmin = rlo - ((int64_t)1 << tau), rmax = rhi + ((int64_t)1 << tau);
                if (rmax > n) rmax = n;
                int64_t u0 = rmin <= 0 ? 0 : (((rmin - 1) >> tau) + 1) >> 1, u1 = ((rmax >> tau) + 1) >> 1;
                R.tskip[b] = u0;
                acc += u1 > u0 ? u1 - u0 : 0;
            }
        }
        R.ntask = acc;
        return;
    }
    if (isA) {
        int64_t r0 = rlo > 1 ? rlo : 1, r1 = rhi < n ? rhi : n;
        R.a_r0 = r0; R.a_nmain = r1 >= r0 ? r1 - r0 + 1 : 0;
        R.nextra = 0;
        for (int b = 0; b < nbits; b++) {
            int64_t step = (int64_t)1 << b;
            for (int side = 0; side < 2; side++) {
                int64_t lo = side == 0 ? rlo - step : rhi + 1, hi = side == 0 ? rlo - 1 : rhi + step;
                if (lo < 1) lo = 1;
                if (hi > n) hi = n;
                for (int64_t r = ((lo + step - 1) >> b) << b; r <= hi; r += step)
                    if (r >= 1 && ((r >> b) & 1) && R.nextra < 64) R.extra[R.nextra++] = r;
            }
        }
        R.nlast = 0;
        if (n >= 1) {
            int lowest = 0;
            while (!((n >> lowest) & 1)) lowest++;
            for (int b = lowest + 1; b < nbits; b++) if ((n >> b) & 1) R.last_b[R.nlast++] = b;
        }
        R.ntask = R.a_nmain + R.nextra + R.nlast;
        return;
    }
    int64_t rmin = rlo - ((int64_t)1 << tau), rmax = rhi + ((int64_t)1 << tau);
    if (rmax > n) rmax = n;
    int64_t acc = 0;
    for (int b = 0; b <= tau; b++) R.tbase[b] = 0;
    for (int b = tau + 1; b < nbits; b++) {
        R.tbase[b] = acc;
        int64_t skip = count_rows(b, tau, rmin - 1);
        int64_t cnt = count_rows(b, tau, rmax) - skip;
        R.tskip[b] = skip;
        acc += cnt > 0 ? cnt : 0;
    }
    for (int b = nbits; b < 36; b++) R.tbase[b] = acc;
    R.ntask = acc;
}

static void launch_rpass(hipStream_t s, const RoundDesc &R, int nbits, int64_t n, int64_t rlo, int64_t rhi, const int64_t *cpos,
                         const int32_t *link, int ge, const int32_t *opt, int32_t *cr, double mean_deg)
{
    const int allp = R.G.win;
    int tau = R.tau;
    int64_t rmin = rlo - ((int64_t)1 << tau), rmax = rhi + ((int64_t)1 << tau);
    if (rmax > n) rmax = n;
    if (rmin < 0) rmin = 0;
    int64_t u0 = rmin <= 0 ? 0 : (((rmin - 1) >> tau) + 1) >> 1;
    int64_t u1 = ((rmax >> tau) + 1) >> 1;
    int64_t nrows = u1 - u0;
    if (nrows <= 0) return;
    if (tau <= g_opt_rpass_small_tau) {
        int64_t cap = (int64_t)(0.01 * (double)g_opt_rpass_cap * mean_deg * (double)((int64_t)1 << tau));
        cap = std::max<int64_t>(16, std::min<int64_t>((cap + 15) / 16 * 16, 1 << 20));
#define RPS(GE, NB) hipLaunchKernelGGL(HIP_KERNEL_NAME(k_rpass_small<GE, NB>), dim3((unsigned)cdiv(nrows, 256)), dim3(256), 0, s, tau, nbits, n, u0, nrows, cpos, link, \
                                       opt, cr, allp, (int)cap)
        if (nbits <= 24) { if (ge) RPS(true, 24); else RPS(false, 24); }
        else             { if (ge) RPS(true, NBMAX); else RPS(false, NBMAX); }
#undef RPS
    } else {
        int ch_cols = (int)g_opt_rpass_ch;
        int64_t cpr = ((int64_t)1 << tau) > ch_cols ? (((int64_t)1 << tau) / ch_cols) : 1;
        if (cpr == 1) ch_cols = 1 << tau;
        int64_t waves = nrows * cpr;
#define RPW(GE, WPB) hipLaunchKernelGGL(HIP_KERNEL_NAME(k_rpass_wave<GE, WPB>), dim3((unsigned)cdiv(waves, WPB)), dim3(64 * WPB), 0, s, tau, nbits, n, u0, \
                                        nrows, (int)cpr, ch_cols, cpos, link, opt, cr, allp)
        if (cpr % 16 == 0)     { if (ge) RPW(true, 16); else RPW(false, 16); }
        else if (cpr % 4 == 0) { if (ge) RPW(true, 4);  else RPW(false, 4); }
        else                   { if (ge) RPW(true, 1);  else RPW(false, 1); }
#undef RPW
    }
}

template <typename TC, typename Rows>
static void ra_build(cp_csr_s *A, LayerWork<TC> &Wk, RaCache<TC> &Ra, int levels, Rows rows_of, int64_t mir_w, const int32_t *anch, const int32_t *anch2)
{
    hipStream_t s = A->stream;
    const bool hyp = Wk.hyp;
    RATab &T = Ra.tab;
    memset(&T, 0, sizeof(T));
    T.nbits = levels; T.n = A->n; T.mir_w = mir_w;
    for (int b = 0; b < 33; b++) { T.tlo[b] = 0; T.thi[b] = INT64_MAX; T.aoff[b] = (mir_w && b < 32) ? Wk.win.aoff[b] : 0; }
    int64_t tb = 0, rb = 0;
    for (int b = 0; b < 33; b++) {
        T.tbase[b] = tb; T.rbase[b] = rb;
        if (b >= levels) continue;
        const int64_t nrows = rows_of(b);
        tb += cdiv(nrows << b, LT);
        if (b >= 9) rb += nrows;
    }
    Ra.ntile = tb; Ra.nrow = rb;
    const size_t total = (size_t)tb * LT;
    Ra.c.ensure(total + 8);
    if (hyp) Ra.c2.ensure(total + 8);
    Ra.part.ensure((size_t)std::max<int64_t>(1, tb - T.tbase[9]));
    if (tb > 0) {
        DBuf<int64_t> &G = Wk.sc.ra_G, &scratch = Wk.sc.scratch;
        G.ensure(total + 1);
        hipLaunchKernelGGL(k_ra_colcount, dim3((unsigned)tb), dim3(LT), 0, s, T, A->pos32.p, A->next.p, hyp ? A->fpos32.p : (const int32_t *)nullptr,
                           hyp ? A->flast.p : (const int32_t *)nullptr, Ra.c.p, hyp ? Ra.c2.p : (int32_t *)nullptr);
        exclusive_scan_i32(Ra.c.p, G.p, (int64_t)total, scratch, s);
        hipLaunchKernelGGL(k_ra_final, dim3((unsigned)tb), dim3(LT), 0, s, T, G.p, Ra.c.p, anch);
        if (hyp) {
            exclusive_scan_i32(Ra.c2.p, G.p, (int64_t)total, scratch, s);
            hipLaunchKernelGGL(k_ra_final, dim3((unsigned)tb), dim3(LT), 0, s, T, G.p, Ra.c2.p, anch2);
        }
        CP_HIP(hipGetLastError());
    }
    Ra.built = true; Ra.w = mir_w;
}
template <typename TC>
static void ra_build_std(cp_csr_s *A, LayerWork<TC> &Wk)
{
    const int64_t n = A->n;
    ra_build<TC>(A, Wk, Wk.ra, Wk.nbits, [n](int b) { return ((n >> b) + 1) >> 1; }, 0, nullptr, nullptr);
}
template <typename TC>
static void ra_build_mir(cp_csr_s *A, LayerWork<TC> &Wk)
{
    const int64_t n = A->n;
    ra_build<TC>(A, Wk, Wk.mir, Wk.G.s, [n](int b) { return n >> (b + 1); }, Wk.G.w, Wk.win.w_anch.p, Wk.win.w_anch2.p);
}

template <typename TC>
static void win_hist_scan(cp_csr_s *A, LayerWork<TC> &Wk, int64_t x, int pass)
{
    hipStream_t s = A->stream;
    const int64_t n = A->n;
    if (pass == 1 || A->N == 0) CP_HIP(hipMemsetAsync(Wk.win.w_hist.p, 0, sizeof(int32_t) * (size_t)(n + 1), s));
    if (pass == 0) { if (A->N > 0) hipLaunchKernelGGL(k_win_hist, dim3((unsigned)cdiv(n + 1, 256)), dim3(256), 0, s, n, x, A->pos32.p, A->prev.p, A->next.p, Wk.win.w_hist.p); }
    else if (A->m > 0) hipLaunchKernelGGL(k_win_hist_rows, dim3((unsigned)cdiv(A->m, 256)), dim3(256), 0, s, A->m, n, x, A->rfirst.p, A->rlast.p, Wk.win.w_hist.p);
    exclusive_scan_i32(Wk.win.w_hist.p, Wk.win.w_E.p, n + 1, Wk.sc.scratch, s);
}

template <typename TC>
static void win_build(cp_csr_s *A, LayerWork<TC> &Wk)
{
    hipStream_t s = A->stream;
    const int64_t n = A->n, w = Wk.G.w;
    const int sb = Wk.G.s;
    int64_t acc = 0;
    for (int b = 0; b < 33; b++) { Wk.win.aoff[b] = acc; if (b < sb) acc += (n >> (b + 1)) + 1; }
    Wk.win.nitems = acc;
    const size_t ni = (size_t)(acc > 0 ? acc : 1);
    Wk.win.w_anch.ensure(ni); Wk.win.w_tot.ensure(ni); Wk.win.w_hist.ensure((size_t)n + 2); Wk.win.w_E.ensure((size_t)n + 2);
    if (Wk.hyp) Wk.win.w_anch2.ensure(ni);
    Wk.win.built = false;
    if (acc > 0) {
        RoundDesc R;
        make_round(R, true, 0, sb + 1, n, 0, n, Wk.G, Wk.win.aoff);
        const unsigned wg = (unsigned)std::min<int64_t>(cdiv(acc, 4), 65536);
        for (int pass = 0; pass < (Wk.hyp ? 2 : 1); pass++) {
            win_hist_scan<TC>(A, Wk, w, pass);
            if (pass == 0) hipLaunchKernelGGL(HIP_KERNEL_NAME(k_win_block_totals<true>), dim3(wg), dim3(256), 0, s, R, acc, A->pos32.p, A->next.p, Wk.win.w_tot.p);
            else hipLaunchKernelGGL(HIP_KERNEL_NAME(k_win_block_totals<false>), dim3(wg), dim3(256), 0, s, R, acc, A->fpos32.p, A->flast.p, Wk.win.w_tot.p);
            hipLaunchKernelGGL(k_win_anchors, dim3((unsigned)cdiv(acc, 256)), dim3(256), 0, s, R, acc, pass == 0 ? A->pos.p : A->lpos.p, Wk.win.w_E.p, Wk.win.w_tot.p,
                               pass == 0 ? Wk.win.w_anch.p : Wk.win.w_anch2.p);
        }
        CP_HIP(hipGetLastError());
    }
    Wk.win.leaf_anch.release(); Wk.win.leaf_anch2.release();
    if (sb >= LEAF_T && w > 62) {
        const int64_t ng = (n >> LEAF_T) + 1;
        Wk.win.leaf_anch.alloc((size_t)ng);
        if (Wk.hyp) Wk.win.leaf_anch2.alloc((size_t)ng);
        for (int pass = 0; pass < (Wk.hyp ? 2 : 1); pass++) {
            win_hist_scan<TC>(A, Wk, w - 62, pass);
            hipLaunchKernelGGL(k_leaf_anchors, dim3((unsigned)cdiv(ng, 256)), dim3(256), 0, s, ng, n, pass == 0 ? A->pos.p : A->lpos.p, Wk.win.w_E.p,
                               pass == 0 ? Wk.win.leaf_anch.p : Wk.win.leaf_anch2.p);
        }
        CP_HIP(hipGetLastError());
    }
    Wk.win.built = true; Wk.win.w = w;
}

template <typename TC, bool HYP>
static void launch_gap(hipStream_t s, cp_csr_s *A, LayerWork<TC> &Wk, int tau, int nchunk, int gnr, RoundCounts *rc, int64_t n, const TC *W,
                       const DevModel<TC> &M, TC alpha, unsigned gg, unsigned gs_grid, unsigned gm, unsigned gslow_grid, int blk)
{
    GapCtx<TC, HYP> C{recs<HYP>(Wk.ow.o_part), recs<HYP>(Wk.ow.o_sub), Wk.ow.o_spv.p, Wk.ow.o_spec.p, Wk.ow.o_tilePS.p, if_hyp<HYP>(Wk.ow.o_tilePS2.p), A->pos32.p, A->next.p,
                      if_hyp<HYP>(A->fpos32.p), if_hyp<HYP>(A->flast.p), W, blk};
    auto *gs = reinterpret_cast<GapSegRec<TC, HYP> *>(Wk.gp.g_seg.p);
    const int32_t *lp = if_hyp<HYP>(A->lpos32.p), *lf = if_hyp<HYP>(A->lfirst.p);
    int32_t *nl = if_hyp<HYP>(Wk.pl.nlopt.p);
#define GF_ARGS tau, nchunk, rc, n, Wk.ow.o_toffs.p, C, Wk.ow.o_tdesc.p, Wk.ow.o_tb.p, Wk.ow.o_rlen.p, A->prev.p, lp, lf, M, alpha, Wk.pl.opt.p, Wk.pl.nnopt.p, nl, Wk.pl.fin.p, \
                Wk.gp.g_list.p, Wk.gp.g_slot.p, Wk.pl.fin_stamp, Wk.gp.g_slow.p
    if (gnr == 2) {
        hipLaunchKernelGGL(HIP_KERNEL_NAME(k_gap_finish<TC, HYP, 2, false>), dim3(gg), dim3(256), 0, s, GF_ARGS);
        hipLaunchKernelGGL(HIP_KERNEL_NAME(k_gap_finish<TC, HYP, 2, true>), dim3(gslow_grid), dim3(256), 0, s, GF_ARGS);
    } else {
        hipLaunchKernelGGL(HIP_KERNEL_NAME(k_gap_finish<TC, HYP, 1, false>), dim3(gg), dim3(256), 0, s, GF_ARGS);
        hipLaunchKernelGGL(HIP_KERNEL_NAME(k_gap_finish<TC, HYP, 1, true>), dim3(gslow_grid), dim3(256), 0, s, GF_ARGS);
    }
#undef GF_ARGS
#define GS_ARGS tau, nchunk, rc, n, Wk.ow.o_toffs.p, C, Wk.ow.o_tdesc.p, Wk.ow.o_tb.p, Wk.ow.o_rlen.p, M, alpha, Wk.gp.g_slot.p, gs, Wk.gp.g_sslow.p
    hipLaunchKernelGGL(HIP_KERNEL_NAME(k_gap_seg<TC, HYP, false>), dim3(gs_grid), dim3(256), 0, s, GS_ARGS);
    hipLaunchKernelGGL(HIP_KERNEL_NAME(k_gap_seg<TC, HYP, true>), dim3(gslow_grid), dim3(256), 0, s, GS_ARGS);
#undef GS_ARGS
    hipLaunchKernelGGL(HIP_KERNEL_NAME(k_gap_merge<TC, HYP>), dim3(gm), dim3(256), 0, s, tau, nchunk, rc, n, Wk.ow.o_toffs.p, Wk.ow.o_tdesc.p, Wk.ow.o_tb.p, A->pos32.p, A->prev.p,
                       lp, lf, M, Wk.gp.g_list.p, gs, Wk.pl.opt.p, Wk.pl.nnopt.p, nl, Wk.pl.fin.p, Wk.pl.fin_stamp);
}

constexpr int64_t LB_MAX = 1 << 20;

template <typename TC, bool HYP>
static void launch_round_a(const LayerCtx<TC> &C, LayerWork<TC> &Wk, const RaCache<TC> &Ra, const RATab &T, int64_t nrow_merge, int64_t tile0, int64_t tile1,
                           int bmin, bool mirrored, bool colmajor)
{
    hipStream_t s = C.s;
    cp_csr_s *A = C.A;
    int32_t *nl = if_hyp<HYP>(Wk.pl.nlopt.p);
    if (colmajor)
        hipLaunchKernelGGL(HIP_KERNEL_NAME(mirrored ? k_ra_cols<TC, HYP, true> : k_ra_cols<TC, HYP, false>), dim3((unsigned)std::max<int64_t>(1, cdiv(tile1 - tile0, 4))), dim3(256), 0, s,
                           T, Ra.c.p, if_hyp<HYP>(Ra.c2.p), A->pos32.p, C.W, C.M, C.alpha, Wk.pl.opt.p, Wk.pl.nnopt.p, nl, recs<HYP>(Ra.part), tile0, tile1, bmin);
    else
        hipLaunchKernelGGL(HIP_KERNEL_NAME(k_ra_layer<TC, HYP>), dim3((unsigned)cdiv(Ra.ntile, 4)), dim3(256), 0, s, T, Ra.ntile, Ra.c.p, if_hyp<HYP>(Ra.c2.p), A->pos32.p, C.W, C.M,
                           C.alpha, Wk.pl.opt.p, Wk.pl.nnopt.p, nl, recs<HYP>(Ra.part));
    if (nrow_merge > 0)
        hipLaunchKernelGGL(HIP_KERNEL_NAME(k_ra_merge<TC, HYP>), dim3((unsigned)cdiv(nrow_merge, 4)), dim3(256), 0, s, T, nrow_merge, recs<HYP>(Ra.part), Wk.pl.opt.p,
                           Wk.pl.nnopt.p, nl);
    CP_HIP(hipGetLastError());
}

template <typename TC, bool HYP>
static void round_a_full(const LayerCtx<TC> &C, LayerWork<TC> &Wk)
{
    hipStream_t s = C.s;
    if (!Wk.ra.built) { ProfScope ps(PROF_LINKS, s, 0.0); ra_build_std<TC>(C.A, Wk); }
    ProfScope ps(PROF_RA, s, 16.0 * (double)Wk.ra.ntile * LT);
    launch_round_a<TC, HYP>(C, Wk, Wk.ra, Wk.ra.tab, Wk.ra.nrow, 0, cdiv(C.n, LT), C.ra_bmin, false, !(g_opt_dbg & DBG_RA_ROWMAJOR));
}

template <typename TC, bool HYP>
static void round_a_win_std(const LayerCtx<TC> &C, LayerWork<TC> &Wk, std::optional<ProfScope> &scope)
{
    hipStream_t s = C.s;
    const Geo &G = C.G;
    const int64_t n = C.n, rlo = C.rlo, rhi = C.rhi;
    if (!Wk.ra.built) { ProfScope ps(PROF_LINKS, s, 0.0); ra_build_std<TC>(C.A, Wk); }
    RATab T2 = Wk.ra.tab;
    T2.nbits = std::min<int32_t>(G.s, Wk.ra.tab.nbits);
    const int64_t nrow2 = T2.nbits > 9 ? Wk.ra.tab.rbase[T2.nbits] : 0;
    const int64_t c_lo = std::max<int64_t>(0, (rlo > 0 ? rlo : 0) - ((int64_t)4 << G.s)), c_hi = std::min<int64_t>(n, rhi);
    const int64_t tile0 = c_lo / LT, tile1 = cdiv(c_hi, LT);
    scope.emplace(PROF_RA, s, 60.0 * (double)(tile1 - tile0) * LT);
    launch_round_a<TC, HYP>(C, Wk, Wk.ra, T2, nrow2, tile0, tile1, C.ra_bmin, false, true);
}

template <typename TC, bool HYP>
static bool round_a_win_mir(const LayerCtx<TC> &C, LayerWork<TC> &Wk)
{
    hipStream_t s = C.s;
    const Geo &G = C.G;
    const int64_t n = C.n, rlo = C.rlo, rhi = C.rhi;
    if (!Wk.mir.built || Wk.mir.w != G.w) { ProfScope ps2(PROF_LINKS, s, 0.0); ra_build_mir<TC>(C.A, Wk); }
    if (Wk.mir.ntile <= 0) return false;
    RATab T3 = Wk.mir.tab;
    const int64_t r_lo = std::max<int64_t>(1, (rlo > 0 ? rlo : 0) - ((int64_t)4 << G.s)), r_hi = std::min<int64_t>(n, rhi);
    double elems = 0;
    for (int b = 0; b < T3.nbits; b++) {
        const int64_t u_lo = std::max<int64_t>(0, (r_lo >> (b + 1)) - 1), u_hi = r_hi >> (b + 1);
        T3.tlo[b] = T3.tbase[b] + ((u_lo << b) / LT);
        T3.thi[b] = std::min<int64_t>(T3.tbase[b + 1], T3.tbase[b] + cdiv(std::max<int64_t>(u_hi, 0) << b, LT));
        elems += (double)std::max<int64_t>(0, T3.thi[b] - T3.tlo[b]) * LT;
    }
    const bool mcols = !(g_opt_dbg & DBG_MIR_ROWMAJOR);
    const int64_t zt0 = r_lo / LT, zt1 = cdiv(std::min<int64_t>(n + G.w + 1, r_hi + ((int64_t)1 << G.s) + 1), LT);
    ProfScope ps2(PROF_RA, s, mcols ? 80.0 * (double)(zt1 - zt0) * LT : 16.0 * elems);
    launch_round_a<TC, HYP>(C, Wk, Wk.mir, T3, Wk.mir.nrow, zt0, zt1, 0, true, mcols);
    return true;
}

static void poison_fill(hipStream_t s, std::initializer_list<std::pair<void *, size_t>> bufs)
{
    if (!(g_opt_dbg & DBG_POISON)) return;
    const int pat = (g_opt_dbg & DBG_POISON_ZERO) ? 0x00 : 0x7F;
    for (const auto &b : bufs) if (b.first) CP_HIP(hipMemsetAsync(b.first, pat, b.second, s));
}

template <typename TC, bool HYP>
static void right_pass(const LayerCtx<TC> &C, LayerWork<TC> &Wk, const RoundDesc &R)
{
    hipStream_t s = C.s;
    cp_csr_s *A = C.A;
    int64_t cols = (((C.n >> R.tau) + 1) >> 1) << R.tau;
    ProfScope ps(PROF_RPASS, s, 4.0 * (C.avg_deg + C.self_deg) * (double)cols + 8.0 * (double)R.ntask);
    if (((int64_t)1 << R.tau) > g_opt_rpass_ch)
        hipLaunchKernelGGL(k_setup, dim3((unsigned)cdiv(R.ntask, 256)), dim3(256), 0, s, R, Wk.pl.opt.p, Wk.pl.nnopt.p, Wk.pl.cr.p, 1,
                           Wk.tk.tdesc.p, A->pos32.p, Wk.tk.tb.p, Wk.tk.len.p, (const int32_t *)nullptr, if_hyp<HYP>(Wk.pl.crl.p), (int32_t *)nullptr);
    launch_rpass(s, R, C.nbits, C.n, C.rlo, C.rhi, A->pos.p, A->prev.p, 0, Wk.pl.opt.p, Wk.pl.cr.p, C.avg_deg);
    if (HYP) launch_rpass(s, R, C.nbits, C.n, C.rlo, C.rhi, A->lpos.p, A->lfirst.p, 1, Wk.pl.opt.p, Wk.pl.crl.p, C.self_deg);
}

template <typename TC, bool HYP>
static void last_row_counts(const LayerCtx<TC> &C, LayerWork<TC> &Wk, const RoundDesc &R)
{
    cp_csr_s *A = C.A;
    CP_HIP(hipMemsetAsync(Wk.pl.last_s0.p, 0, Wk.pl.last_s0.bytes(), C.s));
    hipLaunchKernelGGL(k_last_row_counts, dim3(1024), dim3(256), 0, C.s, R, A->pos32.p, A->prev.p, if_hyp<HYP>(A->lpos32.p), if_hyp<HYP>(A->lfirst.p),
                       Wk.pl.last_s0.p, Wk.pl.fin.p);
}

template <typename TC, bool HYP>
static void setup_tasks(const LayerCtx<TC> &C, LayerWork<TC> &Wk, const RoundDesc &R, RoundCounts *rc, int32_t own_min)
{
    hipStream_t s = C.s;
    cp_csr_s *A = C.A;
    ProfScope ps(PROF_SETUP, s, 29.0 * (double)R.ntask);
    const int sbs = (int)g_opt_setup_bs;
    dim3 sgrid((unsigned)cdiv(R.ntask, sbs));
    if (!R.isA) {
        int64_t mx = 1;
        for (int bb = R.tau + 1; bb < C.nbits; bb++) mx = std::max<int64_t>(mx, R.tbase[bb + 1] - R.tbase[bb]);
        sgrid = dim3((unsigned)cdiv(mx, sbs), (unsigned)std::max(1, C.nbits - R.tau - 1));
    }
    hipLaunchKernelGGL(HIP_KERNEL_NAME(k_setup_short<TC, HYP>), sgrid, dim3(sbs), 0, s, R, Wk.pl.opt.p, Wk.pl.nnopt.p, Wk.pl.nlopt.p, Wk.pl.cr.p, Wk.pl.crl.p, A->pos32.p,
                       A->next.p, if_hyp<HYP>(A->fpos32.p), if_hyp<HYP>(A->flast.p), C.W, C.M, C.alpha, Wk.tk.tdesc.p, Wk.tk.tb.p, Wk.tk.len.p, Wk.tk.tS0l.p, &rc->nlong,
                       (int32_t)g_opt_short_t, (int32_t)g_opt_short_e, C.own_tiles ? Wk.ow.o_tdesc.p : (int4 *)nullptr, Wk.ow.o_tb.p, Wk.ow.o_rlen.p, Wk.ow.o_ntl.p,
                       Wk.ow.o_tS0l.p, &rc->nown, &rc->own_steps, own_min,
                       (int32_t)std::min<size_t>(Wk.ow.o_ntl.n, (size_t)INT32_MAX), &rc->err, Wk.pl.fin.p, Wk.pl.last_s0.p,
                       (g_opt_dbg & DBG_COUNT_NONTRIVIAL) ? &rc->_pad : (int32_t *)nullptr, Wk.win.w_anch.p, Wk.win.w_anch2.p, C.pzp, C.oblk);
}

template <typename TC>
static void round_scans(const LayerCtx<TC> &C, LayerWork<TC> &Wk, const RoundDesc &R, RoundCounts *rc)
{
    hipStream_t s = C.s;
    ProfScope ps(PROF_SCAN, s, 12.0 * (double)R.ntask);
    const bool tiny = C.spec && (g_opt_dbg & DBG_TINY_BUFFERS);
    const int64_t capT = C.spec ? (tiny ? (int64_t)64 : (int64_t)Wk.fl.loc.n) : INT64_MAX, capNT = C.spec ? (tiny ? (int64_t)1 : (int64_t)Wk.ow.o_rec.n) : INT64_MAX;
    const int64_t nm = std::min<int64_t>(R.ntask, (int64_t)Wk.ow.o_ntl.n);
    if (R.ntask <= LB_MAX) {
        launch_round_scans(rc, Wk.tk.len.p, Wk.tk.offs.p, R.ntask, Wk.ow.o_ntl.p, Wk.ow.o_toffs.p, nm, C.own_tiles, capT, capNT, Wk.sc.scanws, s);
    } else {
        exclusive_scan_i32_devn(Wk.tk.len.p, Wk.tk.offs.p, &rc->nlong, R.ntask, &rc->T, Wk.sc.scratch, s);
        if (C.own_tiles) exclusive_scan_i32_devn(Wk.ow.o_ntl.p, Wk.ow.o_toffs.p, &rc->nown, nm, &rc->NT, Wk.sc.scratch, s);
        hipLaunchKernelGGL(k_round_finish, dim3(1), dim3(1), 0, s, rc, capT, capNT);
    }
}

template <bool HYP> static bool own_pairs(bool gap, bool win) { return !HYP && !gap && !win && g_opt_own_pair != 0; }

template <typename TC, bool HYP>
static void own_stream(const LayerCtx<TC> &C, LayerWork<TC> &Wk, const RoundDesc &R, RoundCounts *rc, const RoundCounts &P, bool gap, int split)
{
    hipStream_t s = C.s;
    cp_csr_s *A = C.A;
    const int64_t n = C.n;
    const int oblk = C.oblk;
    const int64_t gNT = C.spec ? (int64_t)Wk.ow.o_rec.n : P.NT;
    poison_fill(s, {{Wk.ow.o_part.p, Wk.ow.o_part.bytes()}, {Wk.ow.o_tileS.p, Wk.ow.o_tileS.bytes()}, {Wk.ow.o_rec.p, Wk.ow.o_rec.bytes()}, {Wk.ow.o_srec.p, Wk.ow.o_srec.bytes()},
                    {if_hyp<HYP>(Wk.ow.o_tileS2.p), Wk.ow.o_tileS2.bytes()}, {Wk.ow.o_items.p, Wk.ow.o_items.bytes()}, {Wk.ow.o_item_of.p, Wk.ow.o_item_of.bytes()},
                    {Wk.ow.o_trec.p, Wk.ow.o_trec.bytes()}});
    const unsigned mgrid = (unsigned)std::min<int64_t>(cdiv(gNT, 256), 8192);
    if (split && !Wk.ow.split.built) {
        ProfScope ps(PROF_LINKS, s, 8.0 * (double)A->N + 16.0 * (double)(C.nbits - SPLIT_BMIN) * (double)(n + 1));
        split_build(A, Wk.ow.split, Wk.sc.scratch);
    }
    hipLaunchKernelGGL(k_own_map, dim3(mgrid), dim3(256), 0, s, rc, Wk.ow.o_toffs.p, Wk.ow.o_tdesc.p, Wk.ow.o_rlen.p, Wk.ow.o_rec.p, Wk.ow.o_task.p,
                       Wk.ow.o_tb.p, gap ? Wk.ow.o_hi.p : (int32_t *)nullptr, R.tau, n, oblk, oblk ? Wk.ow.b_cnt.p : (int32_t *)nullptr, Wk.ow.o_brank.p,
                       gap ? (int2 *)nullptr : Wk.ow.o_items.p, Wk.ow.o_item_of.p, split);
    ProfScope ps(gap ? PROF_GAPSTREAM : PROF_OWN, s, C.own_bytes(Wk.ow.split, R.tau, split != 0, (double)P.own_steps));
    if (oblk) {
        exclusive_scan_i32_lb(Wk.ow.b_cnt.p, Wk.ow.b_start.p, Wk.ow.b_n.p, Wk.ow.b_nblk, nullptr, Wk.sc.scanws, s);
        hipLaunchKernelGGL(k_blk_order, dim3(mgrid), dim3(256), 0, s, rc, Wk.ow.o_rec.p, Wk.ow.o_brank.p, Wk.ow.b_start.p, Wk.ow.o_border.p, Wk.ow.o_srec.p, Wk.ow.b_cnt.p);
    }
    const bool pair = own_pairs<HYP>(gap, C.G.win != 0);
    hipLaunchKernelGGL(HIP_KERNEL_NAME(gap ? k_lpass_own<TC, HYP, true> : pair ? k_lpass_own<TC, HYP, false, !HYP> : k_lpass_own<TC, HYP, false>),
                       dim3((unsigned)cdiv(pair ? cdiv(gNT, 2) : gNT, 4)), dim3(256), 0, s, R.isA, rc,
                       oblk ? Wk.ow.o_border.p : (const int32_t *)nullptr, A->pos32.p, A->next.p, if_hyp<HYP>(A->fpos32.p), if_hyp<HYP>(A->flast.p),
                       Wk.ow.o_tileS.p, Wk.ow.o_tileS2.p, Wk.ow.o_rec.p, Wk.ow.o_srec.p, C.W, C.M, C.alpha, recs<HYP>(Wk.ow.o_part), R.tau, Wk.ow.o_hi.p, Wk.ow.o_spec.p,
                       (int)((g_opt_dbg & DBG_GAP_ALL_SPECIAL) != 0), recs<HYP>(Wk.ow.o_sub), Wk.ow.o_spv.p, A->col.p, if_hyp<HYP>(A->ffirst.p),
                       split ? Wk.ow.split.vnext.p : (const int32_t *)nullptr, Wk.ow.split.vpos.p, Wk.ow.split.vsa.p, (int64_t)(n + 1));
}

template <typename TC, bool HYP>
static void own_merge(const LayerCtx<TC> &C, LayerWork<TC> &Wk, RoundCounts *rc, const RoundCounts &P)
{
    ProfScope ps(PROF_FIX, C.s, 24.0 * (double)P.NT);
    launch_fix_own<TC, HYP>(C.s, rc, Wk.ow.o_toffs.p, recs<HYP>(Wk.ow.o_part), Wk.ow.o_tdesc.p, Wk.ow.o_tb.p, if_hyp<HYP>(Wk.ow.o_tS0l.p), Wk.ow.o_tileS.p,
                            if_hyp<HYP>(Wk.ow.o_tileS2.p), C.M, Wk.pl.opt.p, Wk.pl.nnopt.p, if_hyp<HYP>(Wk.pl.nlopt.p), C.n, Wk.ow.o_items.p, Wk.ow.o_item_of.p, Wk.ow.o_trec.p,
                            Wk.ow.o_tick.p, C.spec ? grow_pred(P.NT) : P.NT, C.spec ? grow_pred(P.nown) : P.nown);
}

template <typename TC, bool HYP>
static void gap_finish(const LayerCtx<TC> &C, LayerWork<TC> &Wk, const RoundDesc &R, RoundCounts *rc, const RoundCounts &P)
{
    hipStream_t s = C.s;
    const int64_t gown = C.spec ? grow_pred(P.nown) : P.nown;
    {
        ProfScope ps(PROF_CARRY, s, 12.0 * (double)P.NT);
        const int32_t *ntp = reinterpret_cast<const int32_t *>(&rc->NT);
        exclusive_scan_i32_lb(Wk.ow.o_tileS.p, Wk.ow.o_tilePS.p, ntp, (int64_t)Wk.ow.o_tileS.n, nullptr, Wk.sc.scanws, s);
        if (HYP) exclusive_scan_i32_lb(Wk.ow.o_tileS2.p, Wk.ow.o_tilePS2.p, ntp, (int64_t)Wk.ow.o_tileS.n, nullptr, Wk.sc.scanws, s);
    }
    ProfScope ps(PROF_GAP, s, 24.0 * (double)P.NT);
    const int nchunk = (int)std::max<int64_t>(1, ((int64_t)2 << R.tau) / 64);
    const size_t ncap = Wk.ow.o_rec.n / GAPSEG + 2;
    Wk.gp.g_list.ensure(ncap); Wk.gp.g_slot.ensure(2 * ncap);
    Wk.gp.g_seg.ensure((2 * ncap) * (size_t)nchunk * 64 * sizeof(GapSegRec<TC, true>));
    Wk.gp.g_slow.ensure((size_t)gown * (size_t)nchunk + 64); Wk.gp.g_sslow.ensure((2 * ncap) * (size_t)nchunk + 64);
    CP_REQUIRE((int64_t)gown * nchunk < INT32_MAX && (int64_t)(2 * ncap) * nchunk < INT32_MAX, CP_EINTERNAL, "gap work index beyond 32 bits");
    const int gnr = (g_opt_gap_nr >= 2 && nchunk >= 2) ? 2 : 1;
    unsigned gg = (unsigned)std::min<int64_t>(cdiv(gown * cdiv((int64_t)nchunk, gnr), 4), 16384);
    unsigned gs_grid = (unsigned)std::min<int64_t>(cdiv((int64_t)(2 * ncap) * nchunk, 4), 8192);
    unsigned gm = (unsigned)std::min<int64_t>(cdiv((int64_t)ncap * nchunk, 4), 4096);
    const unsigned gslow_grid = 2048;
    launch_gap<TC, HYP>(s, C.A, Wk, R.tau, nchunk, gnr, rc, C.n, C.W, C.M, C.alpha, gg, gs_grid, gm, gslow_grid, C.oblk);
}

template <typename TC>
static int64_t flat_gtile(const LayerCtx<TC> &C, const LayerWork<TC> &Wk, const RoundCounts &P) { return C.spec ? (int64_t)Wk.fl.tileS.n : cdiv(P.T, LT); }

template <typename TC, bool HYP>
static void flat_stream(const LayerCtx<TC> &C, LayerWork<TC> &Wk, const RoundDesc &R, RoundCounts *rc, const RoundCounts &P)
{
    hipStream_t s = C.s;
    cp_csr_s *A = C.A;
    const int64_t gtile = flat_gtile(C, Wk, P);
    poison_fill(s, {{Wk.fl.loc.p, Wk.fl.loc.bytes()}, {if_hyp<HYP>(Wk.fl.loc2.p), Wk.fl.loc2.bytes()}, {Wk.fl.partL.p, Wk.fl.partL.bytes()}, {Wk.fl.partR.p, Wk.fl.partR.bytes()},
                    {Wk.fl.tileS.p, Wk.fl.tileS.bytes()}, {if_hyp<HYP>(Wk.fl.tileS2.p), Wk.fl.tileS2.bytes()}});
    hipLaunchKernelGGL(k_tile_t0, dim3((unsigned)cdiv(gtile, 256)), dim3(256), 0, s, rc, Wk.tk.offs.p, Wk.tk.tdesc.p, Wk.fl.tile_t0.p,
                       Wk.fl.tile_rec.p, (int)((g_opt_dbg & DBG_NO_INTERIOR) != 0), Wk.fl.taskR.p);
    ProfScope ps(PROF_EXPAND, s, (double)P.T * C.step_bytes);
    hipLaunchKernelGGL(HIP_KERNEL_NAME(k_lpass<TC, HYP>), dim3((unsigned)cdiv(gtile, 4)), dim3(256), 0, s, R, rc, Wk.tk.offs.p, Wk.tk.tdesc.p, Wk.tk.tS0l.p, Wk.tk.tb.p,
                       A->pos32.p, A->next.p, if_hyp<HYP>(A->fpos32.p), if_hyp<HYP>(A->flast.p), Wk.pl.opt.p, Wk.pl.nnopt.p, Wk.pl.nlopt.p, Wk.fl.loc.p, Wk.fl.loc2.p,
                       Wk.fl.tileS.p, Wk.fl.tileS2.p, Wk.fl.taskR.p, Wk.fl.tile_t0.p, Wk.fl.tile_rec.p, C.W, C.M, C.alpha, recs<HYP>(Wk.fl.partR), recs<HYP>(Wk.fl.partL));
}

template <typename TC, bool HYP>
static void flat_finish(const LayerCtx<TC> &C, LayerWork<TC> &Wk, const RoundDesc &R, RoundCounts *rc, const RoundCounts &P)
{
    hipStream_t s = C.s;
    cp_csr_s *A = C.A;
    const int64_t gtile = flat_gtile(C, Wk, P);
    {
        ProfScope ps(PROF_CARRY, s, 12.0 * (double)cdiv(P.T, LT));
        exclusive_scan_i32_lb(Wk.fl.tileS.p, Wk.fl.tilePS.p, &rc->ntile, (int64_t)Wk.fl.tileS.n, nullptr, Wk.sc.scanws, s);
        if (HYP) exclusive_scan_i32_lb(Wk.fl.tileS2.p, Wk.fl.tilePS2.p, &rc->ntile, (int64_t)Wk.fl.tileS.n, nullptr, Wk.sc.scanws, s);
    }
    unsigned wgrid = (unsigned)std::min<int64_t>(cdiv(gtile, 4), 8192);
    {
        ProfScope ps(PROF_EVAL, s, 0.0);
        hipLaunchKernelGGL(HIP_KERNEL_NAME(k_span_short<TC, HYP>), dim3((unsigned)cdiv(gtile, 256)), dim3(256), 0, s, R, rc, Wk.tk.offs.p, Wk.tk.tdesc.p, Wk.tk.tS0l.p,
                           Wk.tk.tb.p, A->pos32.p, Wk.fl.loc.p, Wk.fl.loc2.p, Wk.fl.tile_t0.p, Wk.fl.taskR.p, Wk.fl.tileS.p, Wk.fl.tileS2.p, recs<HYP>(Wk.fl.partR), C.W, C.M, C.alpha,
                           Wk.pl.opt.p, Wk.pl.nnopt.p, if_hyp<HYP>(Wk.pl.nlopt.p), Wk.fl.open_list.p, Wk.fl.fix_list.p, Wk.fl.tile_rec.p);
        hipLaunchKernelGGL(HIP_KERNEL_NAME(k_open<TC, HYP>), dim3(wgrid), dim3(256), 0, s, R, rc, Wk.tk.offs.p, Wk.tk.tdesc.p, Wk.tk.tS0l.p, A->pos32.p, Wk.fl.loc.p,
                           Wk.fl.loc2.p, Wk.fl.tile_t0.p, Wk.fl.tilePS.p, if_hyp<HYP>(Wk.fl.tilePS2.p), C.W, C.M, C.alpha, recs<HYP>(Wk.fl.partL), Wk.fl.open_list.p);
    }
    {
        ProfScope ps(PROF_FIX, s, 8.0 * (double)cdiv(P.T, LT));
        hipLaunchKernelGGL(HIP_KERNEL_NAME(k_fix<TC, HYP>), dim3(wgrid), dim3(256), 0, s, rc, Wk.tk.offs.p, Wk.fl.taskR.p, recs<HYP>(Wk.fl.partL), recs<HYP>(Wk.fl.partR),
                           Wk.tk.tdesc.p, Wk.tk.tb.p, Wk.pl.opt.p, Wk.pl.nnopt.p, if_hyp<HYP>(Wk.pl.nlopt.p), C.n + 1, Wk.fl.fix_list.p, Wk.fl.tile_rec.p, Wk.fl.tilePS.p,
                           if_hyp<HYP>(Wk.fl.tilePS2.p), if_hyp<HYP>(Wk.tk.tS0l.p), C.M);
    }
    CP_HIP(hipGetLastError());
}

template <typename TC, bool HYP>
static LayerCtx<TC> begin_layer(cp_csr_s *A, const DevModel<TC> &M, TC alpha, const TC *W, TC *cst_out, int32_t *ptr_out, LayerWork<TC> &Wk,
                                int64_t rlo, int64_t rhi, bool spec)
{
    hipStream_t s = A->stream;
    const int64_t n = A->n;
    const Geo G = Wk.G;
    const int nbits = G.win ? G.s + 1 : Wk.nbits;
    const double avg_deg = n > 0 ? (double)A->N / (double)n : 0.0;
    const double self_deg = (HYP && n > 0) ? (double)A->nrows_nonempty / (double)n : 0.0;
    const double step_bytes = 4.0 * (avg_deg + self_deg) + 12.0 + 32.0 / (double)LT;
    const bool own_tiles = !(g_opt_dbg & DBG_NO_OWN_TILES);
    const bool split_layer = !HYP && !G.win && g_opt_own_split && nbits > SPLIT_BMIN;
    CP_HIP(hipMemsetAsync(Wk.sp.rc.p, 0, sizeof(RoundCounts) * (size_t)(nbits + 1), s));
    const bool gaps = own_tiles && g_opt_gap_tau >= 0;
    const int oblk = g_opt_own_blk ? 1 : 0;
    if (oblk) {
        const int64_t nblk = n / LT + 1;
        if (Wk.ow.b_nblk != nblk || !Wk.ow.b_cnt.p) {
            Wk.ow.b_cnt.ensure((size_t)nblk); Wk.ow.b_start.ensure((size_t)nblk + 1); Wk.ow.b_n.ensure(1);
            CP_HIP(hipMemsetD32Async(reinterpret_cast<hipDeviceptr_t>(Wk.ow.b_n.p), (int)nblk, 1, s));
            Wk.ow.b_nblk = nblk;
            Wk.ow.b_dirty = true;
        }
        if (Wk.ow.b_dirty) CP_HIP(hipMemsetAsync(Wk.ow.b_cnt.p, 0, Wk.ow.b_cnt.bytes(), s));
        Wk.ow.b_dirty = true;
    }
    if (Wk.ow.t_dirty) CP_HIP(hipMemsetAsync(Wk.ow.o_tick.p, 0, Wk.ow.o_tick.bytes(), s));
    Wk.ow.t_dirty = true;
    int32_t *pzp = nullptr;
    if (g_opt_poison) {
        Wk.pl.pz.ensure(2);
        pzp = Wk.pl.pz.p;
        CP_HIP(hipMemsetAsync(Wk.pl.pz.p, 0, sizeof(int32_t) * 2, s));
        CP_HIP(hipMemsetAsync(Wk.pl.opt.p, 0x7F, Wk.pl.opt.bytes(), s));
        CP_HIP(hipMemsetAsync(Wk.pl.nnopt.p, 0x7F, Wk.pl.nnopt.bytes(), s));
        if (HYP) CP_HIP(hipMemsetAsync(Wk.pl.nlopt.p, 0x7F, Wk.pl.nlopt.bytes(), s));
    }
    const bool leaf = g_opt_leaf && (!G.win || (G.s >= LEAF_T && !g_opt_block_tables && Wk.win.leaf_anch.p));
    Wk.pl.planes_full = !leaf || g_opt_block_tables;
    const int ra_bmin = (leaf && !Wk.pl.planes_full && !(g_opt_dbg & DBG_RA_ALL_LEVELS)) ? LEAF_T : 0;
    if (++Wk.pl.fin_stamp > 255 || Wk.pl.fin_stamp <= 0) { CP_HIP(hipMemsetAsync(Wk.pl.fin.p, 0, Wk.pl.fin.bytes(), s)); Wk.pl.fin_stamp = 1; }
    return LayerCtx<TC>{A, s, M, alpha, W, cst_out, ptr_out, n, rlo, rhi, G, nbits, spec, own_tiles, gaps, split_layer, leaf, oblk, ra_bmin, pzp,
                        avg_deg, self_deg, step_bytes};
}

template <typename TC, bool HYP>
static bool run_layer(cp_csr_s *A, const DevModel<TC> &M, TC alpha, const TC *W, TC *cst_out, int32_t *ptr_out, LayerWork<TC> &Wk,
                      int64_t rlo, int64_t rhi, bool spec, bool allow_force)
{
    const LayerCtx<TC> C = begin_layer<TC, HYP>(A, M, alpha, W, cst_out, ptr_out, Wk, rlo, rhi, spec);
    hipStream_t s = C.s;
    const int64_t n = C.n;
    const Geo G = C.G;
    const int nbits = C.nbits;
    int32_t *pzp = C.pzp;
    const int NR = nbits + 1;
    std::vector<RoundCounts> used((size_t)NR);
    memset(used.data(), 0, sizeof(RoundCounts) * (size_t)NR);
    struct Patch { size_t idx; int rd; int kind; int tau; bool split; };
    std::vector<Patch> patches;
    auto note = [&](int rd, int kind, int slot, int tau = 0, bool sp = false) {
        if (prof_active(slot)) patches.push_back({g_prof_pending.size() - 1, rd, kind, tau, sp});
    };
    bool any_forced = false;
    std::vector<int8_t> split_mode((size_t)NR, 0);
    std::vector<int8_t> pair_mode((size_t)NR, 0);

    for (int rd = 0; rd <= nbits; rd++) {
        RoundDesc R;
        if (rd == 0) make_round(R, true, 0, nbits, n, rlo, rhi, G, Wk.win.aoff);
        else make_round(R, false, nbits - rd, nbits, n, rlo, rhi, G, Wk.win.aoff);
        R.fin_stamp = Wk.pl.fin_stamp;
        if (C.leaf && !R.isA && R.tau < LEAF_T) continue;
        if (rd == 0 && g_opt_ra_cache && rlo <= 1 && rhi >= n && n >= 1 && !G.win) {
            round_a_full<TC, HYP>(C, Wk);
            R.a_nmain = 0; R.ntask = R.nextra + R.nlast;
        }
        if (rd == 0 && g_opt_ra_cache && G.win && G.s >= 1 && n >= 1 && !(g_opt_dbg & DBG_WIN_NO_RA_CACHE)) {
            std::optional<ProfScope> scope;
            round_a_win_std<TC, HYP>(C, Wk, scope);
            R.skip_std = 1;
            if (!(g_opt_dbg & DBG_WIN_NO_MIR_CACHE) && round_a_win_mir<TC, HYP>(C, Wk)) R.skip_mir = 1;
        }
        if (R.ntask <= 0) continue;
        CP_REQUIRE(R.ntask <= Wk.max_tasks, CP_EINTERNAL, "a DP round has more tasks than the task buffers hold");
        RoundCounts *rc = Wk.sp.rc.p + rd;
        const bool gap = C.gaps && !R.isA && R.tau <= g_opt_gap_tau;
        const bool forced = allow_force && C.own_tiles && !gap && !R.isA && (size_t)rd < Wk.sp.force_own.size() && Wk.sp.force_own[(size_t)rd] &&
                            (rhi - rlo + 1) <= 2 * Wk.sp.force_rows && !(g_opt_dbg & DBG_NO_FORCE_OWN);
        any_forced |= forced;
        if (!R.isA) right_pass<TC, HYP>(C, Wk, R);
        if (R.isA && R.nlast > 0) last_row_counts<TC, HYP>(C, Wk, R);
        setup_tasks<TC, HYP>(C, Wk, R, rc, (int32_t)(forced ? 2 : gap ? g_opt_gap_min : g_opt_own_min));
        RoundCounts P;
        if (spec) {
            P = Wk.sp.pred[(size_t)rd];
            if (Wk.sp.pred_scale != 1.0) {
                auto sc = [&](int64_t v) { return (int64_t)((double)v * Wk.sp.pred_scale) + (v > 0 ? 1 : 0); };
                P.nlong = (int32_t)sc(P.nlong); P.nown = (int32_t)sc(P.nown); P.T = sc(P.T); P.NT = sc(P.NT);
                P.own_steps = (unsigned long long)sc((int64_t)P.own_steps);
            }
            if ((g_opt_dbg & DBG_MISPREDICT) && (rd & 1)) { P.nown = 0; P.NT = 0; P.nlong = 0; P.T = 0; }
            Wk.ow.ensure_own(Wk.hyp, (size_t)grow_pred(P.NT));
            Wk.fl.ensure_flat(Wk.hyp, (size_t)grow_pred(P.T));
        }
        round_scans<TC>(C, Wk, R, rc);
        if (!spec) {
            CP_HIP(hipMemcpyAsync(&P, rc, sizeof(P), hipMemcpyDeviceToHost, s));
            CP_HIP(hipStreamSynchronize(s));
            Wk.ow.ensure_own(Wk.hyp, (size_t)P.NT);
            Wk.fl.ensure_flat(Wk.hyp, (size_t)P.T);
        }
        used[(size_t)rd] = P;
        if (g_opt_dbg & DBG_PRINT_ROUNDS) fprintf(stderr, "round isA=%d tau=%d ntask=%lld %s long=%d own=%d T=%lld NT=%lld nontrivial=%d\n", R.isA, R.tau, (long long)R.ntask,
                                   spec ? "predicted" : "exact", P.nlong, P.nown, (long long)P.T, (long long)P.NT, P._pad);
        if (P.nown > 0 && P.NT > 0) {
            const int split = !(C.split_layer && !R.isA && (!gap || g_opt_gap_split)) ? 0 : R.tau + 1 >= SPLIT_BMIN ? 1 : 2;
            split_mode[(size_t)rd] = (int8_t)(gap ? -split : split);
            pair_mode[(size_t)rd] = own_pairs<HYP>(gap, G.win != 0);
            own_stream<TC, HYP>(C, Wk, R, rc, P, gap, split);
            note(rd, 0, gap ? PROF_GAPSTREAM : PROF_OWN, R.tau, split != 0);
            if (gap) gap_finish<TC, HYP>(C, Wk, R, rc, P);
            else own_merge<TC, HYP>(C, Wk, rc, P);
            CP_HIP(hipGetLastError());
        }
        if (P.nlong <= 0 || P.T <= 0) continue;
        flat_stream<TC, HYP>(C, Wk, R, rc, P);
        note(rd, 1, PROF_EXPAND);
        flat_finish<TC, HYP>(C, Wk, R, rc, P);
    }
    if (C.leaf) leaf_pass<TC, HYP>(C, Wk);
    combine_rows<TC, HYP>(C, Wk);
    CP_HIP(hipGetLastError());
    std::vector<RoundCounts> got((size_t)NR);
    int32_t pz_hits[2] = {0, 0};
    CP_HIP(hipMemcpyAsync(got.data(), Wk.sp.rc.p, sizeof(RoundCounts) * (size_t)NR, hipMemcpyDeviceToHost, s));
    if (pzp) CP_HIP(hipMemcpyAsync(pz_hits, pzp, sizeof(pz_hits), hipMemcpyDeviceToHost, s));
    CP_HIP(hipStreamSynchronize(s));
    bool ok = true;
    for (int rd = 0; rd < NR; rd++) {
        const RoundCounts &g = got[(size_t)rd], &u = used[(size_t)rd];
        CP_REQUIRE(!(g.err && !spec && !any_forced), CP_EINTERNAL, "DP work list overflow");
        if (g.err) ok = false;
        if (g.nown > 0 && g.NT > 0 && !(u.nown > 0 && u.NT > 0)) ok = false;
        if (g.nlong > 0 && g.T > 0 && !(u.nlong > 0 && u.T > 0)) ok = false;
    }
    if (pzp) {
        g_poison_hits += pz_hits[0];
        CP_REQUIRE(!(ok && pz_hits[0] > 0), CP_EINTERNAL, "a DP layer that is not redone read plane cells nobody wrote (poison mode)");
    }
    if (ok) Wk.ow.b_dirty = false;
    Wk.ow.t_dirty = false;
    if (ok) for (int rd = 0; rd < NR; rd++) { g_fix_trips += got[(size_t)rd].n_trips; g_fix_edges |= got[(size_t)rd].n_edge; }
    if (ok) for (int rd = 0; rd < NR; rd++) {
        const RoundCounts &g = got[(size_t)rd];
        if (g.nown > 0 && g.NT > 0) {
            const int sm = split_mode[(size_t)rd];
            (sm < 0 ? g_gap_split_tiles : g_own_split_tiles) += std::abs(sm) == 1 ? g.NT : std::abs(sm) == 2 ? g.n_split : 0;
            if (pair_mode[(size_t)rd]) { g_own_pair_waves += g.NT / 2; g_own_pair_lone += g.NT & 1; }
        }
    }
    for (int rd = 0; rd < NR; rd++) g_fix_items += got[(size_t)rd].n_items;
    if (ok) {
        for (auto &pt : patches) {
            const RoundCounts &g = got[(size_t)pt.rd];
            if (pt.idx < g_prof_pending.size())
                g_prof_pending[pt.idx].bytes = pt.kind == 0 ? C.own_bytes(Wk.ow.split, pt.tau, pt.split, (double)g.own_steps) : (double)g.T * C.step_bytes;
        }
        Wk.sp.pred = got; Wk.sp.pred_ok = true; Wk.sp.pred_rlo = rlo; Wk.sp.pred_rhi = rhi; Wk.sp.pred_win = G.win; Wk.sp.pred_w = G.w;
        if (allow_force && 2 * (rhi - rlo + 1) >= Wk.sp.force_rows) {
            Wk.sp.force_own.resize((size_t)NR, 0);
            Wk.sp.force_rows = rhi - rlo + 1;
            for (int rd = 1; rd < NR; rd++) {
                const RoundCounts &g = got[(size_t)rd];
                if (g.nlong > 0) Wk.sp.force_own[(size_t)rd] = g.nlong <= g_opt_force_max;
            }
        }
    }
    return ok;
}

template <typename TC>
void dp_total_layer(cp_csr_s *A, const DevModel<TC> &M, TC alpha, const TC *W, TC *cst_out, int32_t *ptr_out, void *work_,
                    int64_t rlo, int64_t rhi, int64_t wwin)
{
    auto &Wk = *reinterpret_cast<LayerWork<TC> *>(work_);
    int64_t n = A->n;
    bool hyp = M.kind == CP_MODEL_HYPEREDGE_CUT;
    int nbits = 1;
    while (((int64_t)1 << nbits) <= n) nbits++;
    CP_REQUIRE(nbits <= NBMAX, CP_EINVAL, "n exceeds the bit-plane budget");
    if (Wk.n != n || Wk.hyp != hyp) {
        Wk.n = -1; Wk.nbits = nbits; Wk.hyp = hyp;
        Wk.forget();
        Wk.ow.o_rec.release(); Wk.fl.loc.release();
        size_t plane = (size_t)nbits * (size_t)(n + 1);
        Wk.pl.opt.alloc(plane); Wk.pl.nnopt.alloc(plane); Wk.pl.cr.alloc(plane);
        if (hyp) { Wk.pl.nlopt.alloc(plane); Wk.pl.crl.alloc(plane); }
        CP_HIP(hipMemsetAsync(Wk.pl.opt.p, 0, Wk.pl.opt.bytes(), A->stream));
        CP_HIP(hipMemsetAsync(Wk.pl.nnopt.p, 0, Wk.pl.nnopt.bytes(), A->stream));
        CP_HIP(hipMemsetAsync(Wk.pl.cr.p, 0, Wk.pl.cr.bytes(), A->stream));
        if (hyp) { CP_HIP(hipMemsetAsync(Wk.pl.nlopt.p, 0, Wk.pl.nlopt.bytes(), A->stream)); CP_HIP(hipMemsetAsync(Wk.pl.crl.p, 0, Wk.pl.crl.bytes(), A->stream)); }
        int64_t mx = n;
        for (int tau = 0; tau < nbits; tau++) { RoundDesc R; make_round(R, false, tau, nbits, n, 0, n); if (R.ntask > mx) mx = R.ntask; }
        for (int tau = 0; tau < nbits; tau++) mx = std::max<int64_t>(mx, ((n >> (tau + 1)) + 1) * (int64_t)(nbits - 1 - tau));
        mx = std::max<int64_t>(mx, 2 * n + nbits);
        Wk.max_tasks = mx > 0 ? mx : 1;
        size_t mt = (size_t)Wk.max_tasks;
        Wk.tk.tdesc.alloc(mt); Wk.tk.len.alloc(mt); Wk.tk.tb.alloc(mt); Wk.tk.offs.alloc(mt + 1);
        if (hyp) Wk.tk.tS0l.alloc(mt);
        int64_t mmin = std::max<int64_t>(2, std::min(g_opt_own_min, g_opt_gap_tau >= 0 ? g_opt_gap_min : g_opt_own_min));
        size_t mo = (size_t)(2 * n / mmin + 64) * (size_t)nbits + 1024;
        if (mo > mt) mo = mt;
        Wk.ow.o_tdesc.alloc(mo); Wk.ow.o_tb.alloc(mo); Wk.ow.o_rlen.alloc(mo); Wk.ow.o_ntl.alloc(mo); Wk.ow.o_toffs.alloc(mo + 1); Wk.ow.o_tick.alloc(mo);
        Wk.ow.t_dirty = true;
        if (hyp) Wk.ow.o_tS0l.alloc(mo);
        Wk.sp.rc.alloc((size_t)NBMAX + 2);
        Wk.pl.fin.alloc(plane); Wk.pl.last_s0.alloc(64); Wk.pl.fin_stamp = 255;
        Wk.n = n;
    }
    Geo G{0, 0, 0};
    if (wwin > 0) { G.win = 1; G.w = wwin; G.s = 0; while (((int64_t)2 << G.s) <= wwin) G.s++; if (G.s > nbits - 1) G.s = nbits - 1; }
    Wk.G = G;
    if (G.win && (!Wk.win.built || Wk.win.w != wwin)) win_build<TC>(A, Wk);
    bool spec = Wk.sp.pred_ok && !g_opt_nospec && Wk.sp.pred_win == G.win && Wk.sp.pred_w == G.w;
    Wk.sp.pred_scale = 1.0;
    if (spec && (Wk.sp.pred_rlo != rlo || Wk.sp.pred_rhi != rhi)) {
        const double a = (double)(Wk.sp.pred_rhi - Wk.sp.pred_rlo + 1), b = (double)(rhi - rlo + 1);
        if (!G.win || a < 1 || b < 1 || b > 2.0 * a) spec = false;
        else Wk.sp.pred_scale = b / a;
    }
    if (Wk.sp.pred_win != G.win || Wk.sp.pred_w != G.w || (int)Wk.sp.force_own.size() != (G.win ? G.s + 1 : Wk.nbits) + 1) { Wk.sp.force_own.clear(); Wk.sp.force_rows = 0; }
    auto run = [&](bool sp, bool allow_force) {
        return hyp ? run_layer<TC, true>(A, M, alpha, W, cst_out, ptr_out, Wk, rlo, rhi, sp, allow_force)
                   : run_layer<TC, false>(A, M, alpha, W, cst_out, ptr_out, Wk, rlo, rhi, sp, allow_force);
    };
    if (run(spec, true)) return;
    g_spec_redo++;
    Wk.sp.force_own.clear(); Wk.sp.force_rows = 0;
    bool ok = run(false, false);
    CP_REQUIRE(ok, CP_EINTERNAL, "DP layer failed with exact counts");
}

template <typename TC>
int dp_total_block_tables(cp_csr_s *A, void *work_, int64_t *opt_out, int64_t *nn_out, int64_t *nl_out)
{
    auto &Wk = *reinterpret_cast<LayerWork<TC> *>(work_);
    const int64_t n = A->n, n1 = n + 1;
    CP_REQUIRE(Wk.n == n && Wk.pl.opt.p, CP_EINVAL, "no layer has been computed by the O(n log^2 n) scheme on this handle");
    CP_REQUIRE(Wk.pl.planes_full, CP_EINVAL, "the last layer kept no per-block winners for its leaf rows: cp_set_option(\"block_tables\", 1) before the layer");
    const size_t plane = (size_t)Wk.nbits * (size_t)n1;
    std::vector<int32_t> ho(plane), hn(plane), hl;
    CP_HIP(hipMemcpyAsync(ho.data(), Wk.pl.opt.p, plane * sizeof(int32_t), hipMemcpyDeviceToHost, A->stream));
    CP_HIP(hipMemcpyAsync(hn.data(), Wk.pl.nnopt.p, plane * sizeof(int32_t), hipMemcpyDeviceToHost, A->stream));
    if (Wk.hyp && nl_out) { hl.resize(plane); CP_HIP(hipMemcpyAsync(hl.data(), Wk.pl.nlopt.p, plane * sizeof(int32_t), hipMemcpyDeviceToHost, A->stream)); }
    CP_HIP(hipStreamSynchronize(A->stream));
    for (int b = 0; b < Wk.nbits; b++)
        for (int64_t r = 0; r <= n; r++) {
            const size_t o = (size_t)b * (size_t)n1 + (size_t)r;
            opt_out[o] = 0; nn_out[o] = 0; if (nl_out) nl_out[o] = 0;
            if (r == 0 || !((r >> b) & 1)) continue;
            int t = 0; while (!((r >> t) & 1)) t++;
            const size_t slot = (size_t)b * (size_t)n1 + (size_t)((n - (n >> t)) + (r >> (t + 1)));
            opt_out[o] = (int64_t)ho[slot] + 1; nn_out[o] = hn[slot];
            if (nl_out && !hl.empty()) nl_out[o] = hl[slot];
        }
    return Wk.nbits;
}
template int dp_total_block_tables<int64_t>(cp_csr_s *, void *, int64_t *, int64_t *, int64_t *);
template int dp_total_block_tables<double>(cp_csr_s *, void *, int64_t *, int64_t *, int64_t *);

template <typename TC> void *dp_total_work_new() { return new LayerWork<TC>(); }
template <typename TC> void dp_total_work_free(void *w) { delete reinterpret_cast<LayerWork<TC> *>(w); }
template <typename TC> static void work_reset_fn(void *w) { reinterpret_cast<LayerWork<TC> *>(w)->forget(); }
template <typename TC> void *dp_total_work_get(cp_csr_s *A)
{
    const int i = sizeof(TC) == sizeof(double) && ((TC)0.5 != (TC)0) ? 1 : 0;
    if (!A->dp_work[i]) { A->dp_work[i] = new LayerWork<TC>(); A->dp_work_free_fn[i] = dp_total_work_free<TC>; A->dp_work_reset_fn[i] = work_reset_fn<TC>; }
    return A->dp_work[i];
}
template void *dp_total_work_get<int64_t>(cp_csr_s *);
template void *dp_total_work_get<double>(cp_csr_s *);

template void dp_total_layer<int64_t>(cp_csr_s *, const DevModel<int64_t> &, int64_t, const int64_t *, int64_t *, int32_t *, void *, int64_t, int64_t, int64_t);
template void dp_total_layer<double>(cp_csr_s *, const DevModel<double> &, double, const double *, double *, int32_t *, void *, int64_t, int64_t, int64_t);
template void *dp_total_work_new<int64_t>();
template void *dp_total_work_new<double>();
template void dp_total_work_free<int64_t>(void *);
template void dp_total_work_free<double>(void *);

}
```

chainpartitioners.jl_amd/csrc/dp_total.hpp:

```cpp
#pragma once
#include "csr.hpp"
#include "model.hpp"
#include "dp.hpp"
#include <algorithm>

namespace cpk {

template <typename TC>
__device__ __forceinline__ TC dm_apply_affine(const DevModel<TC> &m, TC alpha, int64_t nv, int64_t np, int64_t nn, int64_t nl)
{
    TC v = cadd(cadd(alpha, cmulc(nv, m.p[CP_P_VERTEX])), cmulc(np, m.p[CP_P_PIN]));
    if (m.kind == CP_MODEL_CONNECTIVITY) return cadd(v, cmulc(nn, m.p[CP_P_NET]));
    if (m.kind == CP_MODEL_HYPEREDGE_CUT) return cadd(cadd(v, cmulc(nl, m.p[CP_P_SELF_NET])), cmulc(nn - nl, m.p[CP_P_CUT_NET]));
    return v;
}

constexpr int LT = 256;
constexpr int NBMAX = 31;
constexpr int SPLIT_BMIN = 8;
constexpr int SPLIT_NB = NBMAX - SPLIT_BMIN;
constexpr int SMAX = 31;
constexpr int FIX_SERIAL = 16;
constexpr int FIX_U = 8;
constexpr int FIX_TRIP = 256 * FIX_U;
constexpr int FIX_REC_W = 5;
constexpr int GAPSEG = 16;
constexpr int LEAF_T = 6;
constexpr int LEAF_G = 1 << LEAF_T;
constexpr int LEAF_FEW = 12;
constexpr int LEAF_LIST = 1024;

__device__ __forceinline__ int64_t prow(int64_t r, int64_t n)
{
    int t = __ffsll((long long)r) - 1;
    return (n - (n >> t)) + (r >> (t + 1));
}

struct Geo { int32_t win, s; int64_t w; };

__host__ __device__ __forceinline__ bool geo_block(const Geo &G, int64_t r, int b, int64_t &cs, int64_t &ce)
{
    const int64_t lo = (r >> b) << b;
    if (!G.win) { cs = lo - ((int64_t)1 << b); ce = lo; return (r >> b) & 1; }
    if (b > G.s) return false;
    if (b == G.s) { cs = lo - G.w + ((int64_t)1 << b) - 1; ce = lo; }
    else if ((r >> b) & 1) { cs = lo - ((int64_t)1 << b); ce = lo; }
    else { cs = lo + ((int64_t)1 << b) - 1 - G.w; ce = cs + ((int64_t)1 << b); }
    if (cs < 0) cs = 0;
    if (ce < 0) ce = 0;
    return ce > cs;
}

struct RoundCounts {
    int32_t n_open, n_fix;
    int32_t nlong, nown;
    unsigned long long own_steps;
    int64_t T, NT;
    int32_t ntile, err;
    int32_t n_items, _pad;
    int32_t n_glong, n_gslots;
    int32_t n_gslow, n_sslow;
    int32_t n_split, _pad2;
    int32_t n_trips, n_edge;
};

template <typename TC, bool HYP> struct Best;
template <typename TC> struct Best<TC, false> { TC v; int32_t p; int32_t nn; };
template <typename TC> struct Best<TC, true> { TC v; int32_t p; int32_t nn; int32_t nl; int32_t _pad; };

__device__ __forceinline__ int64_t shfl_up64(int64_t v, int o)
{
    int lo = __shfl_up((int)(v & 0xffffffffll), o), hi = __shfl_up((int)(v >> 32), o);
    return ((int64_t)hi << 32) | (uint32_t)lo;
}
__device__ __forceinline__ double shfl_up64(double v, int o) { return __longlong_as_double((long long)shfl_up64((int64_t)__double_as_longlong(v), o)); }
__device__ __forceinline__ int64_t shfl64(int64_t v, int src)
{
    int lo = __shfl((int)(v & 0xffffffffll), src), hi = __shfl((int)(v >> 32), src);
    return ((int64_t)hi << 32) | (uint32_t)lo;
}
__device__ __forceinline__ double shfl64(double v, int src) { return __longlong_as_double((long long)shfl64((int64_t)__double_as_longlong(v), src)); }


__device__ __forceinline__ int32_t rdl(int32_t v, int src) { return __builtin_amdgcn_readlane(v, src); }
__device__ __forceinline__ int64_t rdl64(int64_t v, int src)
{
    return ((int64_t)__builtin_amdgcn_readlane((int)(v >> 32), src) << 32) | (uint32_t)__builtin_amdgcn_readlane((int)(v & 0xffffffffll), src);
}
__device__ __forceinline__ double rdl64(double v, int src) { return __longlong_as_double((long long)rdl64((int64_t)__double_as_longlong(v), src)); }

struct RATab { int32_t nbits, _pad; int64_t n; int64_t tbase[33]; int64_t rbase[33]; int64_t mir_w; int64_t aoff[33]; int64_t tlo[33], thi[33]; };


struct SplitLinks {
    bool built = false;
    int nb = 0;
    int64_t stride = 0;
    int64_t tot[SPLIT_NB + 1] = {0};
    DBuf<int32_t> vnext, vpos, vsa;
};

inline size_t fix_items_cap(size_t nt) { return nt / FIX_TRIP + nt / (FIX_SERIAL + 1) + 2; }


struct Planes {
    DBuf<int32_t> opt, nnopt, cr;
    DBuf<int32_t> nlopt, crl;
    DBuf<uint8_t> fin;
    int fin_stamp = 255;
    DBuf<int32_t> last_s0;
    DBuf<int32_t> pz;
    bool planes_full = false;
};

struct SetupTasks {
    DBuf<int4> tdesc;
    DBuf<uint8_t> tb;
    DBuf<int32_t> len, tS0l;
    DBuf<int64_t> offs;
};

struct ScanScratch {
    DBuf<int64_t> scratch;
    DBuf<int64_t> ra_G;
    ScanWS scanws;
};

template <typename TC>
struct FlatStage {
    DBuf<int32_t> loc, tileS;
    DBuf<int32_t> loc2, tileS2;
    DBuf<int64_t> taskR, tilePS, tilePS2, tile_t0;
    DBuf<Best<TC, true>> partL, partR;
    DBuf<int32_t> open_list, fix_list;
    DBuf<int4> tile_rec;
    void ensure_flat(bool hyp, size_t T) {
        if (loc.n >= T && loc.n > 0) return;
        size_t c = T > 0 ? T : 1, nt = (c + LT - 1) / LT;
        loc.release();
        if (hyp) loc2.alloc(c);
        tileS.alloc(nt); tilePS.alloc(nt + 1); tile_t0.alloc(nt); partL.alloc(nt); partR.alloc(nt); taskR.alloc(nt);
        open_list.alloc(nt); fix_list.alloc(nt); tile_rec.alloc(nt);
        if (hyp) { tileS2.alloc(nt); tilePS2.alloc(nt + 1); }
        loc.alloc(c);
    }
};

template <typename TC>
struct OwnTiles {
    DBuf<int4> o_tdesc, o_rec;
    DBuf<uint8_t> o_tb;
    DBuf<int32_t> o_rlen, o_ntl, o_tS0l, o_task, o_tileS, o_tileS2, o_hi;
    DBuf<int64_t> o_toffs, o_tilePS, o_tilePS2;
    DBuf<Best<TC, true>> o_part;
    DBuf<int2> o_items; DBuf<int32_t> o_item_of; DBuf<unsigned long long> o_trec; DBuf<uint32_t> o_tick;
    bool t_dirty = true;
    DBuf<Best<TC, true>> o_sub;
    DBuf<int32_t> o_spv;
    DBuf<uint8_t> o_spec;
    DBuf<int32_t> b_cnt, b_n, o_brank, o_border;
    DBuf<int4> o_srec;
    DBuf<int64_t> b_start;
    int64_t b_nblk = 0;
    bool b_dirty = true;
    SplitLinks split;
    void ensure_own(bool hyp, size_t NT) {
        if (o_rec.n >= NT && o_rec.n > 0) return;
        size_t c = NT > 0 ? NT : 1;
        o_rec.release();
        o_task.alloc(c); o_tileS.alloc(c); o_tilePS.alloc(c + 1); o_part.alloc(c); o_hi.alloc(c); o_spec.alloc(c); o_brank.alloc(c); o_border.alloc(c); o_srec.alloc(c);
        o_item_of.alloc(c); o_items.alloc(fix_items_cap(c)); o_trec.alloc(fix_items_cap(c) * FIX_REC_W);
        o_sub.alloc(c * (SMAX + 1)); o_spv.alloc(c * (SMAX + 1));
        if (hyp) { o_tileS2.alloc(c); o_tilePS2.alloc(c + 1); }
        o_rec.alloc(c);
    }
};

struct GapPass {
    DBuf<int2> g_slot;
    DBuf<int2> g_list;
    DBuf<char> g_seg;
    DBuf<int32_t> g_slow, g_sslow;
};

struct WinAnchors {
    bool built = false; int64_t w = -1, nitems = 0, aoff[33];
    DBuf<int32_t> w_anch, w_anch2, w_tot, w_hist;
    DBuf<int32_t> leaf_anch, leaf_anch2;
    DBuf<int64_t> w_E;
};

template <typename TC>
struct RaCache {
    bool built = false; RATab tab; int64_t ntile = 0, nrow = 0, w = 0;
    DBuf<int32_t> c, c2;
    DBuf<Best<TC, true>> part;
};

struct SpecState {
    DBuf<RoundCounts> rc;
    std::vector<RoundCounts> pred;
    bool pred_ok = false; int64_t pred_rlo = 0, pred_rhi = 0; double pred_scale = 1.0; int pred_win = 0; int64_t pred_w = 0;
    std::vector<uint8_t> force_own;
    int64_t force_rows = 0;
};

template <typename TC>
struct LayerWork {
    int64_t n = -1; int nbits = 0; bool hyp = false;
    Geo G{0, 0, 0};
    int64_t max_tasks = 0;
    Planes pl;
    SetupTasks tk;
    ScanScratch sc;
    FlatStage<TC> fl;
    OwnTiles<TC> ow;
    GapPass gp;
    WinAnchors win;
    RaCache<TC> ra, mir;
    SpecState sp;
    void forget() { ra.built = false; ow.split.built = false; sp.pred_ok = false; win.built = false; mir.built = false; sp.force_own.clear(); sp.force_rows = 0; }
};

template <typename TC>
struct LayerCtx {
    cp_csr_s *A; hipStream_t s;
    DevModel<TC> M; TC alpha; const TC *W;
    TC *cst_out; int32_t *ptr_out;
    int64_t n, rlo, rhi;
    Geo G; int nbits;
    bool spec;
    bool own_tiles, gaps, split_layer, leaf;
    int oblk;
    int ra_bmin;
    int32_t *pzp;
    double avg_deg, self_deg, step_bytes;
    double own_bytes(const SplitLinks &S, int tau, bool sp, double steps) const {
        if (!sp) return steps * step_bytes;
        double var = 0;
        for (int b = std::max(tau + 1, SPLIT_BMIN); b < nbits && b - SPLIT_BMIN < S.nb; b++) var += (double)S.tot[b - SPLIT_BMIN];
        return steps * (20.0 + 32.0 / (double)LT) + 4.0 * std::min(var, avg_deg * steps);
    }
};

inline int64_t grow_pred(int64_t v) { return v + (v >> 2) + 1024; }

template <bool HYP, typename TC> inline Best<TC, HYP> *recs(const DBuf<Best<TC, true>> &b) { return reinterpret_cast<Best<TC, HYP> *>(b.p); }
template <bool HYP, typename T> inline T *if_hyp(T *p) { return HYP ? p : nullptr; }

template <typename TC, bool HYP> void leaf_pass(const LayerCtx<TC> &C, LayerWork<TC> &Wk);
template <typename TC, bool HYP> void combine_rows(const LayerCtx<TC> &C, LayerWork<TC> &Wk);

}
```

include/chainpart.h:

```cpp
#ifndef CHAINPART_H
#define CHAINPART_H

#include "chainpart_types.h"

#ifdef __cplusplus
extern "C" {
#endif

typedef struct cp_csr_s *cp_csr_t;
typedef struct cp_count_s *cp_count_t;

const char *cp_last_error(void);
int32_t cp_version(void);
int32_t cp_device_count(void);

int32_t cp_csr_create(int64_t m, int64_t n, int64_t N, const int64_t *colptr, const int64_t *rowval,
                      int32_t device, cp_csr_t *out);
int32_t cp_csr_create_device(int64_t m, int64_t n, int64_t N, const int64_t *colptr_device,
                             const int64_t *rowval_device, int32_t device, cp_csr_t *out);
int32_t cp_csr_destroy(cp_csr_t csr);
int32_t cp_adjoint(cp_csr_t csr, cp_csr_t *out);
int32_t cp_csr_download(cp_csr_t csr, int64_t *dims_out, int64_t *colptr_out, int64_t *rowval_out);
int32_t cp_csr_reset_cache(cp_csr_t csr);

#define CP_COUNT_DOM     0
#define CP_COUNT_NET     1
#define CP_COUNT_SELFNET 2
#define CP_COUNT_DIANET  3
#define CP_COUNT_SELFPIN 4
int32_t cp_count_build(cp_csr_t csr, int32_t kind, int32_t hint, cp_count_t *out);
int32_t cp_count_query(cp_count_t h, int64_t nq, const int64_t *a, const int64_t *b, int64_t *out);
int32_t cp_count_destroy(cp_count_t h);
int32_t cp_link_array(cp_csr_t csr, int64_t *out );

typedef struct cp_wsum_s *cp_wsum_t;
int32_t cp_domsum_build(cp_csr_t csr, int32_t dtype, const void *val, cp_wsum_t *out);
int32_t cp_rook_build(int64_t N, const int64_t *idx, int32_t dtype, const void *val , int32_t device, cp_wsum_t *out);
int32_t cp_wsum_query(cp_wsum_t h, int64_t nq, const int64_t *i, const int64_t *j, int64_t *count_out ,
                      int64_t *sum_i64, double *sum_f64);
int32_t cp_wsum_destroy(cp_wsum_t h);

int32_t cp_partwise(cp_csr_t csr, int64_t K, const int64_t *asg, int64_t *nprime_out,
                    int64_t *pios_out , int64_t *prm_out ,
                    int64_t *pos_out , int64_t *idx_out );

int32_t cp_oracle_eval(cp_csr_t csr, const cp_model_t *model, const cp_rowpart_t *Pi, int32_t hint,
                       int64_t nq, const int64_t *j, const int64_t *jp, const int64_t *k,
                       int64_t *out_i64, double *out_f64);
int32_t cp_oracle_step(cp_csr_t csr, const cp_model_t *model, const cp_rowpart_t *Pi, int64_t nq,
                       const int32_t *move_j, const int64_t *j, const int32_t *move_jp, const int64_t *jp,
                       const int64_t *k, int64_t *out_i64, double *out_f64);
int32_t cp_bound_stripe(cp_csr_t csr, int64_t K, const cp_model_t *model,
                        int64_t *lo_i64, int64_t *hi_i64, double *lo_f64, double *hi_f64);
int32_t cp_bound_stripe_pi(cp_csr_t csr, int64_t K, const cp_rowpart_t *Pi, const cp_model_t *model,
                           int64_t *lo_i64, int64_t *hi_i64, double *lo_f64, double *hi_f64);
int32_t cp_objective(cp_csr_t csr, int64_t K, const int64_t *spl, const cp_model_t *model,
                     const cp_rowpart_t *Pi, int32_t combine, int64_t *out_i64, double *out_f64);

int32_t cp_partition_dynamic(cp_csr_t csr, int64_t K, int32_t combine, int32_t order,
                             const cp_model_t *model, const cp_rowpart_t *Pi,
                             const cp_model_t *weight, int64_t wmax_i64, double wmax_f64,
                             int64_t *spl_out );
int32_t cp_pack_dynamic(cp_csr_t csr, const cp_model_t *model, const cp_rowpart_t *Pi,
                        const cp_model_t *weight, int64_t wmax_i64, double wmax_f64,
                        int64_t *spl_out , int64_t *K_out);
int32_t cp_pack_dynamic_tables(cp_csr_t csr, const cp_model_t *model, const cp_rowpart_t *Pi,
                               const cp_model_t *weight, int64_t wmax_i64, double wmax_f64,
                               int64_t *spl_tab , int64_t *cst_i64 , double *cst_f64 );
int32_t cp_partition_bisect_cost(cp_csr_t csr, int64_t K, const cp_model_t *model, double eps,
                                 int32_t flip, int64_t *spl_out );
int32_t cp_partition_bisect_cost_batch(cp_csr_t csr, int64_t B, const int64_t *K, const cp_model_t *models, const double *eps,
                                       const int32_t *flip, int64_t ld, int64_t *spl_out);
int32_t cp_partition_bisect_cost_pi(cp_csr_t csr, int64_t K, const cp_model_t *model, const cp_rowpart_t *Pi, double eps,
                                    int32_t flip, int64_t *spl_out );
int32_t cp_partition_bisect_index_pi(cp_csr_t csr, int64_t K, const cp_model_t *model, const cp_rowpart_t *Pi, int32_t flip,
                                     int64_t *spl_out );
int32_t cp_pack_concave(cp_csr_t csr, const cp_model_t *model, const cp_rowpart_t *Pi,
                        const cp_model_t *weight, int64_t wmax_i64, double wmax_f64,
                        int64_t *spl_out , int64_t *K_out);
int32_t cp_partition_concave(cp_csr_t csr, int64_t K, const cp_model_t *model, const cp_rowpart_t *Pi,
                             const cp_model_t *weight, int64_t wmax_i64, double wmax_f64,
                             int64_t *spl_out );
int32_t cp_partition_bisect_index(cp_csr_t csr, int64_t K, const cp_model_t *model, int32_t flip,
                                  int64_t *spl_out );
int32_t cp_partition_lazy_bisect_cost(cp_csr_t csr, int64_t K, const cp_model_t *model, double eps,
                                      int64_t *spl_out );
int32_t cp_partition_lazy_bisect_cost_probes(cp_csr_t csr, int64_t K, const cp_model_t *model, double eps,
                                             int64_t *spl_out , int64_t *nprobes_out);
int32_t cp_partition_lazy_bisect_cost_pi(cp_csr_t csr, int64_t K, const cp_model_t *model, const cp_rowpart_t *Pi, double eps,
                                         int64_t *spl_out , int64_t *nprobes_out);
int32_t cp_partition_lazy_flip_bisect_cost(cp_csr_t csr, int64_t K, const cp_model_t *model, const cp_rowpart_t *Pi, double eps,
                                           int64_t *spl_out , int64_t *nprobes_out);
int32_t cp_pack_convex(cp_csr_t csr, const cp_model_t *model, const cp_rowpart_t *Pi,
                       const cp_model_t *weight, int64_t wmax_i64, double wmax_f64,
                       int64_t *spl_out , int64_t *K_out);
int32_t cp_pack_convex_batch(cp_csr_t csr, int64_t B, const cp_model_t *models, const int64_t *wmax, int64_t ld, int64_t *spl_out, int64_t *K_out);
int32_t cp_partition_convex(cp_csr_t csr, int64_t K, const cp_model_t *model, const cp_rowpart_t *Pi,
                            const cp_model_t *weight, int64_t wmax_i64, double wmax_f64,
                            int64_t *spl_out );
int32_t cp_pack_strict(cp_csr_t csr, int64_t w_max, int64_t *spl_out , int64_t *K_out);
int32_t cp_pack_overlap(cp_csr_t csr, double rho, int64_t w_max, int64_t *spl_out , int64_t *K_out, int64_t *n_nets_out );
int32_t cp_partition_equi(int64_t n, int64_t K, int64_t *spl_out );
int32_t cp_pack_equi(int64_t n, int64_t w, int64_t *spl_out , int64_t *K_out);

int32_t cp_dynamic_tables(cp_csr_t csr, int64_t K, int32_t combine, const cp_model_t *model,
                          const cp_rowpart_t *Pi, int64_t *ptr_out, int64_t *cst_i64, double *cst_f64);

int32_t cp_dynamic_tables_constrained(cp_csr_t csr, int64_t K, const cp_model_t *model, int64_t wmax,
                                      int64_t *win_lo , int64_t *win_hi ,
                                      int64_t *ptr_out, int64_t *cst_i64, double *cst_f64);
int32_t cp_dynamic_tables_constrained_combine(cp_csr_t csr, int64_t K, int32_t combine, const cp_model_t *model, const cp_model_t *weight,
                                              int64_t wmax_i64, double wmax_f64, int64_t *win_lo , int64_t *win_hi ,
                                              int64_t *ptr_out, int64_t *cst_i64, double *cst_f64);

typedef struct cp_dp_s *cp_dp_t;
int32_t cp_dp_begin(cp_csr_t csr, int64_t K, int32_t combine, int32_t order, const cp_model_t *model,
                    int64_t row_lo, int64_t row_hi, cp_dp_t *out);
int32_t cp_dp_layer(cp_dp_t dp, int64_t k, const void *cst_prev_device, void *cst_cur_device);
int32_t cp_dp_ptr_at(cp_dp_t dp, int64_t k, int64_t jp, int64_t *out);
int32_t cp_dp_ptr_row(cp_dp_t dp, int64_t k, int64_t *out );
int32_t cp_dp_set_window(cp_dp_t dp, int64_t wmax);
int32_t cp_dp_set_rows(cp_dp_t dp, int64_t row_lo, int64_t row_hi);
int32_t cp_dp_block_tables(cp_dp_t dp, int32_t *nplanes_out, int64_t *opt_out, int64_t *nets_out, int64_t *selfnets_out);
int32_t cp_dp_destroy(cp_dp_t dp);

int32_t cp_set_stream(cp_csr_t csr, void *hip_stream);
int32_t cp_reset_stream(cp_csr_t csr);
int32_t cp_get_stat(const char *name, int64_t *out);
int32_t cp_test_round_scans(const int32_t *a, int64_t na, int64_t na_max, const int32_t *b, int64_t nb, int64_t nb_max, int32_t two,
                            int64_t cap_t, int64_t cap_nt, int32_t err_in, int32_t reps, int64_t *offs_out, int64_t *toffs_out, int64_t *res);
int32_t cp_test_fix_merge(const cp_model_t *model, int64_t ntask, const int64_t *toffs, const int64_t *part_v, const int32_t *part_p,
                          const int32_t *part_nn, const int32_t *part_nl, const int32_t *tile_s, const int32_t *tile_s2, const int32_t *anchor,
                          const int32_t *anchor2, const int32_t *row, const int32_t *plane, int64_t n, int32_t reps, int32_t *p_out,
                          int32_t *nn_out, int32_t *nl_out, int64_t *res);
int32_t cp_test_own_split(cp_csr_t csr, int32_t *vpos_out, int32_t *vsa_out, int32_t *vnext_out, int64_t *res);
int32_t cp_test_own_pair(int64_t nt, int64_t wave, int64_t *res);
int32_t cp_set_option(const char *name, int64_t value);
int32_t cp_prof_enable(int32_t on);
int32_t cp_prof_reset(void);
int32_t cp_prof_get(int32_t slot, const char **name, int64_t *launches, double *total_ms, double *alg_bytes);

#ifdef __cplusplus
}
#endif
#endif
```

Before: 2.701 partitions/s.

## Bucket prev-links by bit plane for a split right pass on high rounds

```diff
diff --git a/chainpartitioners.jl_amd/_lib.py b/chainpartitioners.jl_amd/_lib.py
--- a/chainpartitioners.jl_amd/_lib.py
+++ b/chainpartitioners.jl_amd/_lib.py
@@ -115,6 +115,8 @@
                                  _I32("nn_out"), _I32("nl_out"), _I64("res")]),
     "cp_test_own_split": (_i32, [_vp, _I32("vpos_out"), _I32("vsa_out"), _I32("vnext_out"), _I64("res")]),
     "cp_test_own_pair": (_i32, [_i64, _i64, _I64("res")]),
+    "cp_test_rpass_split": (_i32, [_vp, _i32, _I32("thr"), _I32("vprev_out"), _I32("wpos_out"), _I32("wsa_out"), _I32("cr_split"),
+                                   _I32("cr_whole"), _I64("res")]),
     "cp_set_option": (_i32, [_str, _i64]),
     "cp_prof_enable": (_i32, [_i32]),
     "cp_prof_reset": (_i32, []),
@@ -274,6 +276,25 @@
         self._ok(rc, "cp_test_own_split")
         assert int(res[0]) == nb
         return nb, vpos[:nb], vsa[:nb], vnext[:int(res[1])]
+
+    def test_rpass_split(self, A, tau=-1, thr=None):
+        nbits = max(1, int(A.n).bit_length())
+        nb, ng = max(0, nbits - 7), A.n // 64 + 1
+        wpos = np.zeros((nb + 1, ng), np.int32); wsa = np.zeros((max(nb, 1), ng), np.int32)
+        vprev = np.zeros(max(A.nnz, 1), np.int32); res = np.zeros(6, np.int64)
+        crs = crw = None
+        if tau >= 0:
+            thr = np.ascontiguousarray(thr, dtype=np.int32)
+            assert thr.shape == (nbits, A.n + 1)
+            crs = np.zeros((nbits, A.n + 1), np.int32); crw = np.zeros_like(crs)
+        flat = lambda a: None if a is None else a.reshape(-1)
+        rc = self.lib.cp_test_rpass_split(self._h(A), tau, flat(thr) if tau >= 0 else None, vprev, wpos.reshape(-1), wsa.reshape(-1), flat(crs), flat(crw), res)
+        self._ok(rc, "cp_test_rpass_split")
+        assert int(res[0]) == nb and int(res[1]) == ng
+        out = (nb, ng, wpos, wsa[:nb], vprev[:int(res[2])])
+        if tau >= 0:
+            out += (crs, crw, dict(zip(("items", "adds", "wpi"), (int(v) for v in res[3:6]))))
+        return out
 
     def test_own_pair(self, nt, wave):
         res = np.zeros(3, np.int64)
diff --git a/chainpartitioners.jl_amd/csrc/capi.hip b/chainpartitioners.jl_amd/csrc/capi.hip
--- a/chainpartitioners.jl_amd/csrc/capi.hip
+++ b/chainpartitioners.jl_amd/csrc/capi.hip
@@ -134,6 +134,7 @@
     {"own_split_tiles", &g_own_split_tiles, false}, {"gap_split_tiles", &g_gap_split_tiles, false},
     {"own_pair_waves", &g_own_pair_waves, false}, {"own_pair_lone", &g_own_pair_lone, false},
     {"overlap_isect", &g_overlap_isect, false}, {"cut_scan_layers", &g_cut_scan_layers, false},
+    {"rpass_split_items", &g_rpass_split_items, false},
 };
 static void stats_reset(bool all) { for (const auto &c : g_stats) if (all || !c.kept) *c.var = 0; }
 
@@ -151,11 +152,13 @@
     {"own_split", &g_opt_own_split, OPT_BOOL, 0, 0},
     {"own_pair", &g_opt_own_pair, OPT_BOOL, 0, 0},
     {"gap_split", &g_opt_gap_split, OPT_BOOL, 0, 0},
+    {"rpass_split", &g_opt_rpass_split, OPT_BOOL, 0, 0},
     {"lws", &g_opt_lws, OPT_BOOL, 0, 0},
     {"gap_tau", &g_opt_gap_tau, OPT_CLAMP, NOLIM_LO, 20}, {"gap_min", &g_opt_gap_min, OPT_CLAMP, 8, NOLIM_HI}, {"gap_nr", &g_opt_gap_nr, OPT_CLAMP, 1, 2},
     {"force_max", &g_opt_force_max, OPT_CLAMP, 0, NOLIM_HI}, {"rpass_cap", &g_opt_rpass_cap, OPT_CLAMP, 1, NOLIM_HI},
     {"own_min", &g_opt_own_min, OPT_CLAMP, 64, NOLIM_HI}, {"bn_chunk", &g_opt_bn_chunk, OPT_CLAMP, 1, NOLIM_HI},
     {"bn_slack", &g_opt_bn_slack, OPT_CLAMP, 0, NOLIM_HI}, {"bn_run", &g_opt_bn_run, OPT_CLAMP, 2, NOLIM_HI},
+    {"rpass_split_tau", &g_opt_rpass_split_tau, OPT_CLAMP, 6, 31}, {"rpass_split_ch", &g_opt_rpass_split_ch, OPT_POW2, 64, 65536},
     {"rpass_ch", &g_opt_rpass_ch, OPT_POW2, 16, 4096}, {"setup_bs", &g_opt_setup_bs, OPT_POW2, 64, 1024}, {"lws_leaf", &g_opt_lws_leaf, OPT_POW2, 256, 2048},
 };
 static int64_t opt_value(const Opt &o, int64_t value)
@@ -309,6 +312,17 @@
     return guarded([&]() -> int32_t {
         CP_HIP(hipSetDevice(A->device));
         dp_own_split_test(A, vpos_out, vsa_out, vnext_out, res);
+        return CP_OK;
+    });
+}
+
+int32_t cp_test_rpass_split(cp_csr_t A, int32_t tau, const int32_t *thr, int32_t *vprev_out, int32_t *wpos_out, int32_t *wsa_out, int32_t *cr_split,
+                            int32_t *cr_whole, int64_t *res)
+{
+    if (!A || !vprev_out || !wpos_out || !wsa_out || !res) return CP_EINVAL;
+    return guarded([&]() -> int32_t {
+        CP_HIP(hipSetDevice(A->device));
+        dp_rpass_split_test(A, tau, thr, vprev_out, wpos_out, wsa_out, cr_split, cr_whole, res);
         return CP_OK;
     });
 }
diff --git a/chainpartitioners.jl_amd/csrc/dp.hpp b/chainpartitioners.jl_amd/csrc/dp.hpp
--- a/chainpartitioners.jl_amd/csrc/dp.hpp
+++ b/chainpartitioners.jl_amd/csrc/dp.hpp
@@ -116,6 +116,12 @@
 extern int64_t g_opt_setup_bs;
 extern int64_t g_opt_rpass_cap;
 extern int64_t g_opt_rpass_ch;
+extern int64_t g_opt_rpass_split;
+extern int64_t g_opt_rpass_split_tau;
+extern int64_t g_opt_rpass_split_ch;
+extern int64_t g_rpass_split_items;
+void dp_rpass_split_test(cp_csr_s *A, int tau, const int32_t *thr, int32_t *vprev_out, int32_t *wpos_out, int32_t *wsa_out, int32_t *cr_split,
+                         int32_t *cr_whole, int64_t *res);
 extern int64_t g_opt_own_min;
 extern int64_t g_opt_own_blk;
 extern int64_t g_opt_own_split;
diff --git a/chainpartitioners.jl_amd/csrc/dp_brute.hip b/chainpartitioners.jl_amd/csrc/dp_brute.hip
--- a/chainpartitioners.jl_amd/csrc/dp_brute.hip
+++ b/chainpartitioners.jl_amd/csrc/dp_brute.hip
@@ -15,6 +15,10 @@
 int64_t g_opt_own_pair = 1;
 int64_t g_own_pair_waves = 0, g_own_pair_lone = 0;
 int64_t g_opt_rpass_ch = 256;
+int64_t g_opt_rpass_split = 1;
+int64_t g_opt_rpass_split_tau = 12;
+int64_t g_opt_rpass_split_ch = 2048;
+int64_t g_rpass_split_items = 0;
 int64_t g_opt_rpass_small_tau = 4;
 int64_t g_opt_force_max = 1024;
 int64_t g_opt_setup_bs = 1024;
diff --git a/chainpartitioners.jl_amd/csrc/dp_total.hip b/chainpartitioners.jl_amd/csrc/dp_total.hip
--- a/chainpartitioners.jl_amd/csrc/dp_total.hip
+++ b/chainpartitioners.jl_amd/csrc/dp_total.hip
@@ -125,7 +125,7 @@
         if (b > tau && b < nbits && (allp || ((r >> b) & 1))) cr[(int64_t)b * n1 + prow((r), n1 - 1)] = cnt[b];
 }
 
-template <bool ge, int WPB>
+template <bool ge, int WPB, bool SKIP0 = false>
 __global__ void __launch_bounds__(64 * WPB) k_rpass_wave(int tau, int nbits, int64_t n, int64_t u0, int64_t nrows, int chunks_per_row, int ch_cols,
                                                          const int64_t *__restrict__ pos, const int32_t *__restrict__ prev,
                                                          const int32_t *__restrict__ opt, int32_t *__restrict__ cr, int allp)
@@ -145,6 +145,7 @@
     uint32_t act = 0;
     for (int b = tau + 1; b < nbits; b++) if (allp || ((r >> b) & 1)) act |= 1u << b;
     act = __builtin_amdgcn_readfirstlane(act);
+    if (SKIP0 && act == 0) return;
     const bool mine = lane < 32 && ((act >> lane) & 1);
     const int32_t tv = mine ? opt[(int64_t)lane * n1 + prL] : 0;
     int32_t acc = 0;
@@ -195,6 +196,71 @@
     if (mine) {
         if (chunks_per_row == WPB) cr[(int64_t)lane * n1 + prow((r), n1 - 1)] = outv;
         else atomicAdd(&cr[(int64_t)lane * n1 + prow((r), n1 - 1)], outv);
+    }
+}
+
+struct RsGrid { int32_t gpi[32]; };
+
+template <int WPI>
+__global__ void __launch_bounds__(64 * WPI) k_rpass_split(RoundDesc R, RsGrid Gd, int64_t ng, uint32_t ch, const int32_t *__restrict__ wpos,
+                                                          const int32_t *__restrict__ wsa, const int32_t *__restrict__ vprev,
+                                                          const int32_t *__restrict__ opt, int32_t *__restrict__ cr)
+{
+    const int tau = R.tau, b = tau + 1 + (int)blockIdx.y;
+    const uint32_t gpi = (uint32_t)Gd.gpi[b];
+    const uint32_t item = blockIdx.x / gpi, grp = blockIdx.x - item * gpi;
+    if ((int64_t)item >= R.tbase[b + 1] - R.tbase[b]) return;
+    const int64_t l = (int64_t)item + R.tskip[b];
+    const int sh = b - tau - 1;
+    const int64_t r = ((l >> sh) << (b + 1)) | ((int64_t)1 << b) | ((((l & (((int64_t)1 << sh) - 1)) << 1) | 1) << tau);
+    const int64_t rL = r - ((int64_t)1 << tau), n1 = R.n + 1;
+    const int32_t *__restrict__ wp = wpos + (int64_t)(b - RSPLIT_BMIN) * ng, *__restrict__ wa = wsa + (int64_t)(b - RSPLIT_BMIN) * ng;
+    const uint32_t q0 = (uint32_t)wp[rL >> 6], len = (uint32_t)wp[r >> 6] - q0;
+    const int32_t thr = opt[(int64_t)b * n1 + prow(rL, R.n)];
+    const uint32_t lane = threadIdx.x & 63;
+    const uint32_t wv = (uint32_t)__builtin_amdgcn_readfirstlane((int)(threadIdx.x >> 6));
+    const uint32_t slot = grp * WPI + wv, stride = gpi * WPI * ch;
+    int32_t acc = 0;
+    struct __attribute__((packed, aligned(4))) V4 { int32_t x, y, z, w; };
+    for (uint32_t cs = slot * ch; cs < len; cs += stride) {
+        const uint32_t el = len - cs < ch ? len - cs : ch;
+        const int32_t *__restrict__ src = vprev + q0 + cs;
+        int32_t a[8], nx[8];
+#pragma unroll
+        for (int k = 0; k < 2; k++) {
+            const uint32_t o = 4 * lane + 256 * k, oc = o < el ? o : el;
+            const V4 t = *reinterpret_cast<const V4 *>(src + oc);
+            a[4 * k] = o < el ? t.x : INT32_MAX; a[4 * k + 1] = o + 1 < el ? t.y : INT32_MAX;
+            a[4 * k + 2] = o + 2 < el ? t.z : INT32_MAX; a[4 * k + 3] = o + 3 < el ? t.w : INT32_MAX;
+        }
+        for (uint32_t tb = 0; tb < el; tb += 512) {
+#pragma unroll
+            for (int k = 0; k < 2; k++) {
+                const uint32_t o = tb + 512 + 4 * lane + 256 * k, oc = o < el ? o : el;
+                const V4 t = *reinterpret_cast<const V4 *>(src + oc);
+                nx[4 * k] = o < el ? t.x : INT32_MAX; nx[4 * k + 1] = o + 1 < el ? t.y : INT32_MAX;
+                nx[4 * k + 2] = o + 2 < el ? t.z : INT32_MAX; nx[4 * k + 3] = o + 3 < el ? t.w : INT32_MAX;
+            }
+#pragma unroll
+            for (int k = 0; k < 8; k++) acc += (int32_t)__popcll(__ballot(a[k] < thr));
+#pragma unroll
+            for (int k = 0; k < 8; k++) a[k] = nx[k];
+        }
+    }
+    if (slot == 0) acc += wa[r >> 6] - wa[rL >> 6];
+    if (WPI > 1) {
+        __shared__ int32_t sacc[WPI];
+        if (lane == 0) sacc[wv] = acc;
+        __syncthreads();
+        if (wv != 0) return;
+        acc = 0;
+#pragma unroll
+        for (int k = 0; k < WPI; k++) acc += sacc[k];
+    }
+    if (lane == 0) {
+        int32_t *cell = &cr[(int64_t)b * n1 + prow(r, R.n)];
+        if (gpi == 1) *cell = acc;
+        else if (acc) atomicAdd(cell, acc);
     }
 }
 
@@ -2523,6 +2589,118 @@
     S.built = true;
 }
 
+__device__ __forceinline__ int rsplit_slot(int32_t p, int32_t x, int nb)
+{
+    const int h = split_plane(p, x);
+    return h == 31 ? nb : h - RSPLIT_BMIN;
+}
+
+__global__ void __launch_bounds__(256) k_rsplit_count(const int32_t *__restrict__ pos, const int32_t *__restrict__ prev, int64_t n, int nb, int64_t ng,
+                                                      int32_t *__restrict__ cnt)
+{
+    const int64_t p = (int64_t)blockIdx.x * blockDim.x + threadIdx.x, g = p >> 6;
+    int32_t c[RSPLIT_NB + 1];
+#pragma unroll
+    for (int b = 0; b <= RSPLIT_NB; b++) c[b] = 0;
+    if (p < n)
+        for (int32_t q = pos[p], qe = pos[p + 1]; q < qe; q++) {
+            const int h = rsplit_slot((int32_t)p, prev[q], nb);
+#pragma unroll
+            for (int b = 0; b <= RSPLIT_NB; b++) c[b] += (h == b);
+        }
+#pragma unroll
+    for (int b = 0; b <= RSPLIT_NB; b++) {
+        if (b > nb) continue;
+        int32_t v = c[b];
+        for (int o = 32; o > 0; o >>= 1) v += __shfl_xor(v, o);
+        if ((threadIdx.x & 63) == 0 && g < ng) cnt[(int64_t)b * ng + g] = v;
+    }
+}
+
+__global__ void __launch_bounds__(256) k_rsplit_scatter(const int32_t *__restrict__ pos, const int32_t *__restrict__ prev, int64_t n, int nb, int64_t ng,
+                                                        const int32_t *__restrict__ wpos, int32_t *__restrict__ vprev)
+{
+    const int64_t p = (int64_t)blockIdx.x * blockDim.x + threadIdx.x, g = p >> 6;
+    const int lane = threadIdx.x & 63;
+    int32_t c[RSPLIT_NB];
+#pragma unroll
+    for (int b = 0; b < RSPLIT_NB; b++) c[b] = 0;
+    if (p < n)
+        for (int32_t q = pos[p], qe = pos[p + 1]; q < qe; q++) {
+            const int h = rsplit_slot((int32_t)p, prev[q], nb);
+#pragma unroll
+            for (int b = 0; b < RSPLIT_NB; b++) c[b] += (h == b);
+        }
+#pragma unroll
+    for (int b = 0; b < RSPLIT_NB; b++) {
+        if (b >= nb) continue;
+        int32_t v = c[b];
+        for (int o = 1; o < 64; o <<= 1) { const int32_t t = __shfl_up(v, o); if (lane >= o) v += t; }
+        c[b] = (g < ng ? wpos[(int64_t)b * ng + g] : 0) + v - c[b];
+    }
+    if (p < n)
+        for (int32_t q = pos[p], qe = pos[p + 1]; q < qe; q++) {
+            const int32_t x = prev[q];
+            const int h = rsplit_slot((int32_t)p, x, nb);
+            int32_t dst = -1;
+#pragma unroll
+            for (int b = 0; b < RSPLIT_NB; b++) if (h == b) { dst = c[b]; c[b]++; }
+            if (dst >= 0 && h < nb) vprev[dst] = x;
+        }
+}
+
+__global__ void __launch_bounds__(256) k_rsplit_sums(const int32_t *__restrict__ wpos, int64_t n, int nb, int64_t ng, int32_t *__restrict__ wsa,
+                                                     unsigned long long *__restrict__ sum)
+{
+    const int64_t g = (int64_t)blockIdx.x * blockDim.x + threadIdx.x;
+    const bool live = g < ng;
+    if (g == 0) for (int b = 0; b <= nb + 1; b++) sum[32 + b] = (unsigned long long)wpos[(int64_t)b * ng];
+    int32_t above = 0, stored = 0;
+    for (int b = nb; b >= 0; b--) {
+        const int64_t i = (int64_t)b * ng + (live ? g : 0);
+        if (b < nb) {
+            if (live) wsa[i] = above;
+            stored += wpos[i + 1] - wpos[i];
+            const int tau = b + RSPLIT_BMIN - 1;
+            const int64_t c = g << 6, r = ((c >> tau) | 1) << tau;
+            int64_t v = (live && !((c >> tau) & 1) && r <= n) ? stored : 0;
+            for (int o = 32; o > 0; o >>= 1) v += __shfl_xor(v, o);
+            if ((threadIdx.x & 63) == 0 && v) atomicAdd(&sum[tau], (unsigned long long)v);
+        }
+        above += wpos[i] - wpos[(int64_t)b * ng];
+    }
+}
+
+static void rsplit_build(cp_csr_s *A, RightSplit &S, DBuf<int64_t> &scratch)
+{
+    hipStream_t s = A->stream;
+    const int64_t n = A->n;
+    int nbits = 1;
+    while (((int64_t)1 << nbits) <= n) nbits++;
+    S.nb = std::max(0, nbits - RSPLIT_BMIN); S.ng = (n >> 6) + 1;
+    for (auto &t : S.tot) t = 0;
+    for (auto &t : S.round_tot) t = 0;
+    if (S.nb > 0) {
+        CP_REQUIRE(S.nb <= RSPLIT_NB, CP_EINVAL, "n exceeds the bit-plane budget");
+        const size_t cells = (size_t)(S.nb + 1) * (size_t)S.ng;
+        S.wpos.ensure(cells + 1); S.wsa.ensure(cells + 1); S.vprev.ensure((size_t)A->N + 16); S.sum.ensure(96);
+        const unsigned grid = (unsigned)cdiv(S.ng * 64, 256);
+        hipLaunchKernelGGL(k_rsplit_count, dim3(grid), dim3(256), 0, s, A->pos32.p, A->prev.p, n, S.nb, S.ng, S.wsa.p);
+        exclusive_scan_i32_i32(S.wsa.p, S.wpos.p, (int64_t)cells, scratch, s);
+        hipLaunchKernelGGL(k_rsplit_scatter, dim3(grid), dim3(256), 0, s, A->pos32.p, A->prev.p, n, S.nb, S.ng, S.wpos.p, S.vprev.p);
+        CP_HIP(hipMemsetAsync(S.sum.p, 0, S.sum.bytes(), s));
+        hipLaunchKernelGGL(k_rsplit_sums, dim3((unsigned)cdiv(S.ng, 256)), dim3(256), 0, s, S.wpos.p, n, S.nb, S.ng, S.wsa.p, S.sum.p);
+        CP_HIP(hipGetLastError());
+        unsigned long long h[96];
+        CP_HIP(hipMemcpyAsync(h, S.sum.p, sizeof(h), hipMemcpyDeviceToHost, s));
+        CP_HIP(hipStreamSynchronize(s));
+        for (int b = 0; b < S.nb; b++) S.tot[b] = (int64_t)h[32 + b + 1] - (int64_t)h[32 + b];
+        S.tot[S.nb] = (int64_t)h[32 + S.nb];
+        for (int tau = 0; tau < 32; tau++) S.round_tot[tau] = (int64_t)h[tau];
+    }
+    S.built = true;
+}
+
 void dp_own_pair_test(int64_t nt, int64_t wave, int64_t *res)
 {
     int64_t s0 = 0, s1 = 0;
@@ -2625,8 +2803,14 @@
     R.ntask = acc;
 }
 
+static void clear_cr(hipStream_t s, const RoundDesc &R, int32_t *cr, int32_t *crl)
+{
+    hipLaunchKernelGGL(k_setup, dim3((unsigned)cdiv(R.ntask, 256)), dim3(256), 0, s, R, (const int32_t *)nullptr, (const int32_t *)nullptr, cr, 1,
+                       (int4 *)nullptr, (const int32_t *)nullptr, (uint8_t *)nullptr, (int32_t *)nullptr, (const int32_t *)nullptr, crl, (int32_t *)nullptr);
+}
+
 static void launch_rpass(hipStream_t s, const RoundDesc &R, int nbits, int64_t n, int64_t rlo, int64_t rhi, const int64_t *cpos,
-                         const int32_t *link, int ge, const int32_t *opt, int32_t *cr, double mean_deg)
+                         const int32_t *link, int ge, const int32_t *opt, int32_t *cr, double mean_deg, bool skip0 = false)
 {
     const int allp = R.G.win;
     int tau = R.tau;
@@ -2652,10 +2836,100 @@
         int64_t waves = nrows * cpr;
 #define RPW(GE, WPB) hipLaunchKernelGGL(HIP_KERNEL_NAME(k_rpass_wave<GE, WPB>), dim3((unsigned)cdiv(waves, WPB)), dim3(64 * WPB), 0, s, tau, nbits, n, u0, \
                                         nrows, (int)cpr, ch_cols, cpos, link, opt, cr, allp)
-        if (cpr % 16 == 0)     { if (ge) RPW(true, 16); else RPW(false, 16); }
-        else if (cpr % 4 == 0) { if (ge) RPW(true, 4);  else RPW(false, 4); }
-        else                   { if (ge) RPW(true, 1);  else RPW(false, 1); }
+        if (skip0 && !ge) {
+#define RPW0(WPB) hipLaunchKernelGGL(HIP_KERNEL_NAME(k_rpass_wave<false, WPB, true>), dim3((unsigned)cdiv(waves, WPB)), dim3(64 * WPB), 0, s, tau, nbits, n, u0, \
+                                     nrows, (int)cpr, ch_cols, cpos, link, opt, cr, allp)
+            if (cpr % 16 == 0) RPW0(16); else if (cpr % 4 == 0) RPW0(4); else RPW0(1);
+#undef RPW0
+        }
+        else if (cpr % 16 == 0) { if (ge) RPW(true, 16); else RPW(false, 16); }
+        else if (cpr % 4 == 0)  { if (ge) RPW(true, 4);  else RPW(false, 4); }
+        else                    { if (ge) RPW(true, 1);  else RPW(false, 1); }
 #undef RPW
+    }
+}
+
+static int rsplit_grid(const RoundDesc &R, const RightSplit &S, int nbits, RsGrid &Gd, unsigned &gx, bool &adds)
+{
+    const int tau = R.tau;
+    int64_t slots[32], mx = 1;
+    for (int b = 0; b < 32; b++) { slots[b] = 1; Gd.gpi[b] = 1; }
+    for (int b = tau + 1; b < nbits; b++) {
+        const int64_t rows = std::max<int64_t>(1, count_rows(b, tau, R.n));
+        const int64_t chunks = cdiv(cdiv(S.tot[b - RSPLIT_BMIN], 2 * rows), g_opt_rpass_split_ch);
+        while (slots[b] < chunks && slots[b] < 4096) slots[b] <<= 1;
+        mx = std::max(mx, slots[b]);
+    }
+    const int wpi = mx >= 64 ? 16 : mx >= 4 ? 4 : 1;
+    int64_t x = 1;
+    adds = false;
+    for (int b = tau + 1; b < nbits; b++) {
+        Gd.gpi[b] = (int32_t)std::max<int64_t>(1, slots[b] / wpi);
+        adds |= Gd.gpi[b] > 1;
+        x = std::max(x, (R.tbase[b + 1] - R.tbase[b]) * Gd.gpi[b]);
+    }
+    CP_REQUIRE(x < ((int64_t)1 << 31), CP_EINTERNAL, "the split right pass has too many workgroups");
+    gx = (unsigned)x;
+    return wpi;
+}
+
+static void launch_rpass_split(hipStream_t s, const RoundDesc &R, const RightSplit &S, int nbits, const RsGrid &Gd, unsigned gx, int wpi,
+                               const int32_t *opt, int32_t *cr)
+{
+    const dim3 grid(gx, (unsigned)(nbits - R.tau - 1));
+#define RPS(WPI) hipLaunchKernelGGL(HIP_KERNEL_NAME(k_rpass_split<WPI>), grid, dim3(64 * WPI), 0, s, R, Gd, S.ng, (uint32_t)g_opt_rpass_split_ch, S.wpos.p, S.wsa.p, \
+                                    S.vprev.p, opt, cr)
+    if (wpi == 16) RPS(16); else if (wpi == 4) RPS(4); else RPS(1);
+#undef RPS
+}
+
+void dp_rpass_split_test(cp_csr_s *A, int tau, const int32_t *thr, int32_t *vprev_out, int32_t *wpos_out, int32_t *wsa_out, int32_t *cr_split,
+                         int32_t *cr_whole, int64_t *res)
+{
+    ensure_links(A);
+    hipStream_t s = A->stream;
+    RightSplit S;
+    DBuf<int64_t> scratch;
+    rsplit_build(A, S, scratch);
+    res[0] = S.nb; res[1] = S.ng; res[2] = S.tot[S.nb]; res[3] = 0; res[4] = 0; res[5] = 0;
+    if (S.nb <= 0) return;
+    CP_HIP(hipMemcpyAsync(wpos_out, S.wpos.p, (size_t)(S.nb + 1) * (size_t)S.ng * sizeof(int32_t), hipMemcpyDeviceToHost, s));
+    CP_HIP(hipMemcpyAsync(wsa_out, S.wsa.p, (size_t)S.nb * (size_t)S.ng * sizeof(int32_t), hipMemcpyDeviceToHost, s));
+    if (res[2] > 0) CP_HIP(hipMemcpyAsync(vprev_out, S.vprev.p, (size_t)res[2] * sizeof(int32_t), hipMemcpyDeviceToHost, s));
+    CP_HIP(hipStreamSynchronize(s));
+    if (tau < 0) return;
+    const int64_t n = A->n, n1 = n + 1;
+    const int nbits = S.nb + RSPLIT_BMIN;
+    CP_REQUIRE(tau >= LEAF_T && tau < nbits - 1 && thr && cr_split && cr_whole, CP_EINVAL, "cp_test_rpass_split: no such round");
+    const size_t plane = (size_t)nbits * (size_t)n1;
+    auto slot = [&](int64_t r) { int t = 0; while (!((r >> t) & 1)) t++; return (n - (n >> t)) + (r >> (t + 1)); };
+    std::vector<int32_t> h(plane, 0);
+    for (int b = 0; b < nbits; b++)
+        for (int64_t r = 1; r <= n; r++) h[(size_t)b * n1 + slot(r)] = thr[(size_t)b * n1 + r];
+    DBuf<int32_t> opt(plane), cr(plane);
+    CP_HIP(hipMemcpyAsync(opt.p, h.data(), plane * sizeof(int32_t), hipMemcpyHostToDevice, s));
+    RoundDesc R;
+    make_round(R, false, tau, nbits, n, 0, n);
+    res[3] = R.ntask;
+    for (int form = 0; form < 2; form++) {
+        CP_HIP(hipMemsetAsync(cr.p, 0, cr.bytes(), s));
+        if (R.ntask <= 0) {
+        } else if (form == 0) {
+            RsGrid Gd; unsigned gx = 1; bool adds = false;
+            const int wpi = rsplit_grid(R, S, nbits, Gd, gx, adds);
+            res[4] = adds; res[5] = wpi;
+            if (adds) clear_cr(s, R, cr.p, (int32_t *)nullptr);
+            launch_rpass_split(s, R, S, nbits, Gd, gx, wpi, opt.p, cr.p);
+        } else {
+            if (((int64_t)1 << tau) > g_opt_rpass_ch) clear_cr(s, R, cr.p, (int32_t *)nullptr);
+            launch_rpass(s, R, nbits, n, 0, n, A->pos.p, A->prev.p, 0, opt.p, cr.p, n > 0 ? (double)A->N / (double)n : 0.0);
+        }
+        CP_HIP(hipGetLastError());
+        CP_HIP(hipMemcpyAsync(h.data(), cr.p, plane * sizeof(int32_t), hipMemcpyDeviceToHost, s));
+        CP_HIP(hipStreamSynchronize(s));
+        int32_t *out = form == 0 ? cr_split : cr_whole;
+        out[0] = 0;
+        for (int b = 0; b < nbits; b++) { out[(size_t)b * n1] = 0; for (int64_t r = 1; r <= n; r++) out[(size_t)b * n1 + r] = h[(size_t)b * n1 + slot(r)]; }
     }
 }
 
@@ -2865,17 +3139,34 @@
     for (const auto &b : bufs) if (b.first) CP_HIP(hipMemsetAsync(b.first, pat, b.second, s));
 }
 
+static bool rsplit_round(bool rsplit_layer, int tau) { return rsplit_layer && tau >= std::max<int64_t>(LEAF_T, g_opt_rpass_split_tau); }
+
 template <typename TC, bool HYP>
 static void right_pass(const LayerCtx<TC> &C, LayerWork<TC> &Wk, const RoundDesc &R)
 {
     hipStream_t s = C.s;
     cp_csr_s *A = C.A;
     int64_t cols = (((C.n >> R.tau) + 1) >> 1) << R.tau;
+    if (!HYP && rsplit_round(C.rsplit_layer, R.tau)) {
+        RightSplit &S = Wk.rs;
+        if (!S.built) {
+            ProfScope pb(PROF_LINKS, s, 12.0 * (double)A->N + 8.0 * (double)A->n + 16.0 * (double)(C.nbits - RSPLIT_BMIN + 1) * (double)(C.n / 64 + 1));
+            rsplit_build(A, S, Wk.sc.scratch);
+        }
+        RsGrid Gd; unsigned gx = 1; bool adds = false;
+        const int wpi = rsplit_grid(R, S, C.nbits, Gd, gx, adds);
+        const int64_t rows_all = ((C.n >> R.tau) + 1) >> 1, rmax = std::min(C.n, C.rhi + ((int64_t)1 << R.tau)), rmin = std::max<int64_t>(0, C.rlo - ((int64_t)1 << R.tau));
+        const int64_t rows = (((rmax >> R.tau) + 1) >> 1) - (rmin <= 0 ? 0 : (((rmin - 1) >> R.tau) + 1) >> 1);
+        ProfScope ps(PROF_RPASS, s, 4.0 * (double)S.round_tot[R.tau] * (rows_all > 0 ? (double)rows / (double)rows_all : 0.0) + 16.0 * (double)R.ntask);
+        if (adds) clear_cr(s, R, Wk.pl.cr.p, (int32_t *)nullptr);
+        launch_rpass_split(s, R, S, C.nbits, Gd, gx, wpi, Wk.pl.opt.p, Wk.pl.cr.p);
+        return;
+    }
     ProfScope ps(PROF_RPASS, s, 4.0 * (C.avg_deg + C.self_deg) * (double)cols + 8.0 * (double)R.ntask);
     if (((int64_t)1 << R.tau) > g_opt_rpass_ch)
         hipLaunchKernelGGL(k_setup, dim3((unsigned)cdiv(R.ntask, 256)), dim3(256), 0, s, R, Wk.pl.opt.p, Wk.pl.nnopt.p, Wk.pl.cr.p, 1,
                            Wk.tk.tdesc.p, A->pos32.p, Wk.tk.tb.p, Wk.tk.len.p, (const int32_t *)nullptr, if_hyp<HYP>(Wk.pl.crl.p), (int32_t *)nullptr);
-    launch_rpass(s, R, C.nbits, C.n, C.rlo, C.rhi, A->pos.p, A->prev.p, 0, Wk.pl.opt.p, Wk.pl.cr.p, C.avg_deg);
+    launch_rpass(s, R, C.nbits, C.n, C.rlo, C.rhi, A->pos.p, A->prev.p, 0, Wk.pl.opt.p, Wk.pl.cr.p, C.avg_deg, C.rsplit_layer);
     if (HYP) launch_rpass(s, R, C.nbits, C.n, C.rlo, C.rhi, A->lpos.p, A->lfirst.p, 1, Wk.pl.opt.p, Wk.pl.crl.p, C.self_deg);
 }
 
@@ -3057,6 +3348,7 @@
     const double step_bytes = 4.0 * (avg_deg + self_deg) + 12.0 + 32.0 / (double)LT;
     const bool own_tiles = !(g_opt_dbg & DBG_NO_OWN_TILES);
     const bool split_layer = !HYP && !G.win && g_opt_own_split && nbits > SPLIT_BMIN;
+    const bool rsplit_layer = !HYP && !G.win && g_opt_rpass_split && nbits > RSPLIT_BMIN;
     CP_HIP(hipMemsetAsync(Wk.sp.rc.p, 0, sizeof(RoundCounts) * (size_t)(nbits + 1), s));
     const bool gaps = own_tiles && g_opt_gap_tau >= 0;
     const int oblk = g_opt_own_blk ? 1 : 0;
@@ -3086,7 +3378,7 @@
     Wk.pl.planes_full = !leaf || g_opt_block_tables;
     const int ra_bmin = (leaf && !Wk.pl.planes_full && !(g_opt_dbg & DBG_RA_ALL_LEVELS)) ? LEAF_T : 0;
     if (++Wk.pl.fin_stamp > 255 || Wk.pl.fin_stamp <= 0) { CP_HIP(hipMemsetAsync(Wk.pl.fin.p, 0, Wk.pl.fin.bytes(), s)); Wk.pl.fin_stamp = 1; }
-    return LayerCtx<TC>{A, s, M, alpha, W, cst_out, ptr_out, n, rlo, rhi, G, nbits, spec, own_tiles, gaps, split_layer, leaf, oblk, ra_bmin, pzp,
+    return LayerCtx<TC>{A, s, M, alpha, W, cst_out, ptr_out, n, rlo, rhi, G, nbits, spec, own_tiles, gaps, split_layer, leaf, rsplit_layer, oblk, ra_bmin, pzp,
                         avg_deg, self_deg, step_bytes};
 }
 
@@ -3111,6 +3403,7 @@
     bool any_forced = false;
     std::vector<int8_t> split_mode((size_t)NR, 0);
     std::vector<int8_t> pair_mode((size_t)NR, 0);
+    int64_t rsplit_items = 0;
 
     for (int rd = 0; rd <= nbits; rd++) {
         RoundDesc R;
@@ -3136,6 +3429,7 @@
                             (rhi - rlo + 1) <= 2 * Wk.sp.force_rows && !(g_opt_dbg & DBG_NO_FORCE_OWN);
         any_forced |= forced;
         if (!R.isA) right_pass<TC, HYP>(C, Wk, R);
+        if (!R.isA && !HYP && rsplit_round(C.rsplit_layer, R.tau)) rsplit_items += R.ntask;
         if (R.isA && R.nlast > 0) last_row_counts<TC, HYP>(C, Wk, R);
         setup_tasks<TC, HYP>(C, Wk, R, rc, (int32_t)(forced ? 2 : gap ? g_opt_gap_min : g_opt_own_min));
         RoundCounts P;
@@ -3197,6 +3491,7 @@
     }
     if (ok) Wk.ow.b_dirty = false;
     Wk.ow.t_dirty = false;
+    if (ok) g_rpass_split_items += rsplit_items;
     if (ok) for (int rd = 0; rd < NR; rd++) { g_fix_trips += got[(size_t)rd].n_trips; g_fix_edges |= got[(size_t)rd].n_edge; }
     if (ok) for (int rd = 0; rd < NR; rd++) {
         const RoundCounts &g = got[(size_t)rd];
diff --git a/chainpartitioners.jl_amd/csrc/dp_total.hpp b/chainpartitioners.jl_amd/csrc/dp_total.hpp
--- a/chainpartitioners.jl_amd/csrc/dp_total.hpp
+++ b/chainpartitioners.jl_amd/csrc/dp_total.hpp
@@ -27,6 +27,8 @@
 constexpr int GAPSEG = 16;
 constexpr int LEAF_T = 6;
 constexpr int LEAF_G = 1 << LEAF_T;
+constexpr int RSPLIT_BMIN = LEAF_T + 1;
+constexpr int RSPLIT_NB = NBMAX - RSPLIT_BMIN;
 constexpr int LEAF_FEW = 12;
 constexpr int LEAF_LIST = 1024;
 
@@ -98,6 +100,16 @@
     int64_t stride = 0;
     int64_t tot[SPLIT_NB + 1] = {0};
     DBuf<int32_t> vnext, vpos, vsa;
+};
+
+struct RightSplit {
+    bool built = false;
+    int nb = 0;
+    int64_t ng = 0;
+    int64_t tot[RSPLIT_NB + 1] = {0};
+    int64_t round_tot[NBMAX + 1] = {0};
+    DBuf<int32_t> vprev, wpos, wsa;
+    DBuf<unsigned long long> sum;
 };
 
 inline size_t fix_items_cap(size_t nt) { return nt / FIX_TRIP + nt / (FIX_SERIAL + 1) + 2; }
@@ -219,7 +231,8 @@
     WinAnchors win;
     RaCache<TC> ra, mir;
     SpecState sp;
-    void forget() { ra.built = false; ow.split.built = false; sp.pred_ok = false; win.built = false; mir.built = false; sp.force_own.clear(); sp.force_rows = 0; }
+    RightSplit rs;
+    void forget() { ra.built = false; ow.split.built = false; rs.built = false; sp.pred_ok = false; win.built = false; mir.built = false; sp.force_own.clear(); sp.force_rows = 0; }
 };
 
 template <typename TC>
@@ -231,6 +244,7 @@
     Geo G; int nbits;
     bool spec;
     bool own_tiles, gaps, split_layer, leaf;
+    bool rsplit_layer;
     int oblk;
     int ra_bmin;
     int32_t *pzp;
diff --git a/include/chainpart.h b/include/chainpart.h
--- a/include/chainpart.h
+++ b/include/chainpart.h
@@ -134,6 +134,8 @@
                           const int32_t *anchor2, const int32_t *row, const int32_t *plane, int64_t n, int32_t reps, int32_t *p_out,
                           int32_t *nn_out, int32_t *nl_out, int64_t *res);
 int32_t cp_test_own_split(cp_csr_t csr, int32_t *vpos_out, int32_t *vsa_out, int32_t *vnext_out, int64_t *res);
+int32_t cp_test_rpass_split(cp_csr_t csr, int32_t tau, const int32_t *thr, int32_t *vprev_out, int32_t *wpos_out, int32_t *wsa_out,
+                            int32_t *cr_split, int32_t *cr_whole, int64_t *res);
 int32_t cp_test_own_pair(int64_t nt, int64_t wave, int64_t *res);
 int32_t cp_set_option(const char *name, int64_t value);
 int32_t cp_prof_enable(int32_t on);
```

After: 2.716 partitions/s, median of 6. About the same (+0.5%).
